# RRZE-HPC/Ultimate-SpMV

Hardware: AMD Instinct MI355X
Metric: SpMV GFLOP/s (SELL-32-512 dp; achieved HBM GB/s in roofline) (higher is better)
Workload: dtype f64; 1 GPU; nlpkkt200-class synthetic (27-pt stencil 253x253x253, n=16194277, nnz=433798093) scs -c 32 -s 512 -dp; C=32, sigma=512, n_rows=16194277, nnz=433798093, x=5.0 (DefaultValues), partition=none, halo_overlap=False, kernel=tile-local-column (LDS-staged x lines, 12-bit local indices)

## Files before the change

### include/uspmv.h

```cpp
#ifndef USPMV_H
#define USPMV_H

#include <stddef.h>
#include <stdint.h>

#ifdef __cplusplus
extern "C" {
#endif

typedef enum {
    USPMV_OK = 0,
    USPMV_ERR_INVALID = 1,
    USPMV_ERR_IO = 2,
    USPMV_ERR_UNSUPPORTED = 3,
    USPMV_ERR_OVERFLOW = 4,
    USPMV_ERR_NO_DEVICE = 5,
    USPMV_ERR_HIP = 6,
    USPMV_ERR_ALLOC = 7,
    USPMV_ERR_COMM = 8
} uspmv_status;

typedef enum { USPMV_F64 = 0, USPMV_F32 = 1, USPMV_F16 = 2 } uspmv_dtype;
typedef enum { USPMV_COLWISE = 0, USPMV_ROWWISE = 1 } uspmv_layout;
typedef enum { USPMV_SEG_ROWS = 0, USPMV_SEG_NNZ = 1 } uspmv_seg;
// ... 21 lines not shown

int uspmv_gen_stencil27(int64_t nx, int64_t ny, int64_t nz, int dof, uint64_t seed, double magnitude_decades,
                        int64_t row_begin, int64_t row_end, uspmv_coo_t **out);
int uspmv_gen_stencil27_row_counts(int64_t nx, int64_t ny, int64_t nz, int dof, int64_t row_begin, int64_t row_end, int32_t *out);
int uspmv_gen_banded_random(int64_t n, int nnz_per_row, int64_t band, uint64_t seed, double magnitude_decades,
                            int64_t row_begin, int64_t row_end, uspmv_coo_t **out);
int uspmv_gen_kkt(int64_t N, uint64_t seed, int64_t row_begin, int64_t row_end, uspmv_coo_t **out);
int uspmv_gen_kkt_row_counts(int64_t N, int64_t row_begin, int64_t row_end, int32_t *out);

int uspmv_convert_to_scs(const uspmv_coo_t *m, int64_t C, int64_t sigma, int dtype,
                         const int32_t *fixed_permutation, uspmv_scs_t **out);
int uspmv_scs_meta(const uspmv_scs_t *s, int64_t meta[8]);
int uspmv_scs_dtype(const uspmv_scs_t *s, int *dtype);
int uspmv_scs_arrays(const uspmv_scs_t *s, const int32_t **chunk_ptrs, const int32_t **chunk_lengths,
                     const int32_t **col_idxs, const void **values, const int32_t **old_to_new_idx,
                     const int32_t **new_to_old_idx);
int uspmv_scs_col_idxs_mut(uspmv_scs_t *s, int32_t **col_idxs);
int uspmv_permute_scs_cols(uspmv_scs_t *s, const int32_t *perm);
void uspmv_scs_free(uspmv_scs_t *s);
int uspmv_apply_permutation(void *out, const void *in, const int32_t *perm, int64_t n, int dtype);
int uspmv_partition_precisions(const uspmv_coo_t *m, double threshold_1, uspmv_coo_t **dp, uspmv_coo_t **sp);
enum { USPMV_AP_DP_HP = 0, USPMV_AP_SP_HP = 1, USPMV_AP_DP_SP_HP = 2 };
int uspmv_partition_precisions_hp(const uspmv_coo_t *m, int kind, double threshold_1, double threshold_2, uspmv_coo_t **hi,
                                  uspmv_coo_t **mid, uspmv_coo_t **hp);

int uspmv_device_count(int *count);
int uspmv_set_device(int device);
int uspmv_stream_synchronize(void *stream);

int uspmv_dmat_upload(const uspmv_scs_t *s, uspmv_dmat_t **out);
int uspmv_convert_to_scs_device(const uspmv_coo_t *m, int64_t C, int64_t sigma, int dtype, const int32_t *fixed_permutation,
                                int permute_cols, uspmv_scs_t **layout, uspmv_dmat_t **out);
int uspmv_dmat_plan_addresses(const uspmv_dmat_t *m, uint64_t addr[8]);
int uspmv_dmat_meta(const uspmv_dmat_t *m, int64_t meta[4]);
enum { USPMV_SORT_HOST = 0, USPMV_SORT_DEVICE_STABLE = 1 };
int uspmv_convert_to_scs_device_from_arrays(const int32_t *d_I, const int32_t *d_J, const double *d_V, int64_t n_rows, int64_t n_cols, int64_t nnz,
                                            int64_t C, int64_t sigma, int dtype, const int32_t *d_fixed_permutation, int permute_cols,
                                            int sort_mode, void *stream, uspmv_scs_t **layout, int32_t *d_old_to_new, int32_t *d_new_to_old,
                                            uspmv_dmat_t **out);
int uspmv_dmat_download(const uspmv_dmat_t *m, int32_t *chunk_ptrs, int32_t *chunk_lengths, int32_t *col_idxs, void *values);
int uspmv_dmat_wrap(int64_t C, int64_t n_chunks, int64_t n_elements, int dtype, const int32_t *d_chunk_ptrs,
                    const int32_t *d_chunk_lengths, const int32_t *d_col_idxs, const void *d_values,
                    uspmv_dmat_t **out);
void uspmv_dmat_free(uspmv_dmat_t *m);
int uspmv_dmat_optimize(uspmv_dmat_t *m, const uspmv_scs_t *s, int max_lines, int64_t *n_tiles, int64_t *n_staged);
int uspmv_dmat_optimize_ap(uspmv_dmat_t *dp, uspmv_dmat_t *sp, const uspmv_scs_t *s_dp, const uspmv_scs_t *s_sp,
                           int max_lines, int64_t *n_tiles, int64_t *n_staged);
int uspmv_dmat_optimize_ap_hp(uspmv_dmat_t *hi, uspmv_dmat_t *mid, uspmv_dmat_t *hp, const uspmv_scs_t *s_hi, const uspmv_scs_t *s_mid,
                              const uspmv_scs_t *s_hp, int max_lines, int64_t *n_tiles, int64_t *n_staged);
int uspmv_dmat_optimize_block(uspmv_dmat_t *m, const uspmv_scs_t *s, int block_vec_size, int64_t *n_tiles, int64_t *n_staged);

int uspmv_dmat_optimize_sweep(uspmv_dmat_t *m, const uspmv_scs_t *s, int wlog, int tile_rows, int64_t *n_tiles, int64_t *n_sweep);
int uspmv_dmat_optimize_sweep_ap(uspmv_dmat_t *dp, uspmv_dmat_t *sp, const uspmv_scs_t *s_dp, const uspmv_scs_t *s_sp, int wlog,
                                 int tile_rows, int64_t *n_tiles, int64_t *n_sweep);
int uspmv_dmat_optimize_sweep_ap_hp(uspmv_dmat_t *hi, uspmv_dmat_t *mid, uspmv_dmat_t *hp, const uspmv_scs_t *s_hi, const uspmv_scs_t *s_mid,
                                    const uspmv_scs_t *s_hp, int wlog, int tile_rows, int64_t *n_tiles, int64_t *n_sweep);
int uspmv_dmat_optimize_sweep_device_ap_hp(uspmv_dmat_t *hi, uspmv_dmat_t *mid, uspmv_dmat_t *hp, int wlog, int tile_rows, int64_t *n_tiles,
                                           int64_t *n_sweep);
int uspmv_dmat_optimize_sweep_device(uspmv_dmat_t *m, uspmv_dmat_t *sp, int wlog, int tile_rows, int64_t *n_tiles, int64_t *n_sweep);
int uspmv_dmat_sweep_plan_digest(const uspmv_dmat_t *m, uint64_t digest[16], int64_t meta[8]);
int uspmv_dmat_sweep_plan_digest_part(const uspmv_dmat_t *m, int part, uint64_t digest[5], int64_t *n_vals);
int uspmv_dmat_plan_info(const uspmv_dmat_t *m, int *kind, int64_t *n_tiles, int64_t *n_planned);
int uspmv_dmat_block_plan_info(const uspmv_dmat_t *m, int64_t meta[10]);
int uspmv_dmat_block_plan_staged(const uspmv_dmat_t *m, int64_t *rows_staged);
int uspmv_dmat_plan_granularity(const uspmv_dmat_t *m, int *elements_per_list_entry);
int uspmv_dmat_plan_rows_dealt(const uspmv_dmat_t *m, int *dealt);
int uspmv_dmat_stream_info(const uspmv_dmat_t *m, int64_t meta[2]);
int uspmv_dmat_block_plan_digest(const uspmv_dmat_t *m, uint64_t digest[8]);

int uspmv_dmat_optimize_block_sweep(uspmv_dmat_t *m, const uspmv_scs_t *s, int block_vec_size, int wlog, int tile_rows, int64_t *n_tiles, int64_t *n_sweep);

int uspmv_dmat_optimize_block_device(uspmv_dmat_t *m, int block_vec_size, int64_t *n_tiles, int64_t *n_staged);

int uspmv_dmat_optimize_device(uspmv_dmat_t *m, int max_lines, int64_t *n_tiles, int64_t *n_staged);
int uspmv_dmat_optimize_device_ap(uspmv_dmat_t *dp, uspmv_dmat_t *sp, int max_lines, int64_t *n_tiles, int64_t *n_staged);
int uspmv_dmat_optimize_device_ap_hp(uspmv_dmat_t *hi, uspmv_dmat_t *mid, uspmv_dmat_t *hp, int max_lines, int64_t *n_tiles, int64_t *n_staged);
int uspmv_dmat_plan_download(const uspmv_dmat_t *m, int64_t meta[4], int32_t *tile_line_ptr, int32_t *tile_lines,
                             uint32_t *c16_ptrs, uint16_t *col16);

int uspmv_dmat_tile_rows(const uspmv_dmat_t *m, int *tile_rows);
int uspmv_dmat_index_bits(const uspmv_dmat_t *m, int *bits);
int uspmv_dmat_additive_chunks(const uspmv_dmat_t *m, int64_t *n_additive, int64_t *n_chunks);
int uspmv_additive_plan_probe(const uspmv_scs_t *s, int64_t stats[8], int32_t *cols);
int uspmv_spmv_tiles(const uspmv_dmat_t *A, const int32_t *d_tile_ids, int64_t n_ids, const void *d_x, void *d_y,
                     void *stream);
int uspmv_dmat_set_crs(uspmv_dmat_t *m, int on);

int uspmv_spmv(const uspmv_dmat_t *A, const void *d_x, void *d_y, void *stream);
int uspmv_spmv_chunks(const uspmv_dmat_t *A, const int32_t *d_chunk_ids, int64_t n_ids, const void *d_x,
                      void *d_y, void *stream);
int uspmv_spmmv(const uspmv_dmat_t *A, const void *d_X, void *d_Y, int b, int64_t ld, int layout, void *stream);
int uspmv_spmmv_x_prepared(const uspmv_dmat_t *m, const void *d_X, int block_vec_size, int64_t ld, void *stream);
int uspmv_spmmv_x_release(const uspmv_dmat_t *m);
int uspmv_spmv_ap(const uspmv_dmat_t *dp, const uspmv_dmat_t *sp, const double *d_x, double *d_y, void *stream);
int uspmv_spmmv_ap(const uspmv_dmat_t *dp, const uspmv_dmat_t *sp, const void *d_X, void *d_Y, int b, int64_t ld, int layout,
                   void *stream);
int uspmv_spmmv_ap_plan_lines(int b, int *max_lines);
int uspmv_spmmv_ap_path(const uspmv_dmat_t *dp, const uspmv_dmat_t *sp, int b, int64_t ld, int layout, int *path, int *vectors_per_pass);
int uspmv_spmmv_ap_sweep_vectors(int b, int wlog, int *vectors);
int uspmv_spmv_ap_generic(const uspmv_dmat_t *dp, const uspmv_dmat_t *sp, const double *d_x, const float *d_x_sp,
                          double *d_y, void *stream);
int uspmv_spmv_ap_hp(const uspmv_dmat_t *hi, const uspmv_dmat_t *mid, const uspmv_dmat_t *hp, const void *d_x, void *d_y, void *stream);
int uspmv_spmmv_ap_hp(const uspmv_dmat_t *hi, const uspmv_dmat_t *mid, const uspmv_dmat_t *hp, const void *d_X, void *d_Y, int b, int64_t ld,
                      int layout, void *stream);
int uspmv_spmmv_ap_hp_path(const uspmv_dmat_t *hi, const uspmv_dmat_t *mid, const uspmv_dmat_t *hp, int b, int64_t ld, int layout, int *path,
                           int *vectors_per_pass);
int uspmv_spmmv_ap_hp_plan_lines(int b, int x_dtype, int *max_lines);
int uspmv_spmmv_ap_hp_sweep_vectors(int b, int wlog, int x_dtype, int *vectors);

int uspmv_scs_gpu_f64(int64_t C, int64_t n_chunks, const int32_t *d_chunk_ptrs, const int32_t *d_chunk_lengths,
                      const int32_t *d_col_idxs, const double *d_values, const double *d_x, double *d_y,
                      void *stream);
int uspmv_scs_gpu_f32(int64_t C, int64_t n_chunks, const int32_t *d_chunk_ptrs, const int32_t *d_chunk_lengths,
                      const int32_t *d_col_idxs, const float *d_values, const float *d_x, float *d_y,
                      void *stream);
int uspmv_csr_gpu_f64(int64_t n_rows, const int32_t *d_row_ptrs, const int32_t *d_col_idxs,
                      const double *d_values, const double *d_x, double *d_y, void *stream);
int uspmv_csr_gpu_f32(int64_t n_rows, const int32_t *d_row_ptrs, const int32_t *d_col_idxs,
                      const float *d_values, const float *d_x, float *d_y, void *stream);

int uspmv_peek_i64(const void *p, int64_t *out);
int uspmv_peek_i32(const void *p, int32_t *out);

int uspmv_apply_permutation_dev(void *d_out, const void *d_in, const int32_t *d_perm, int64_t n, int dtype,
                                void *stream);

void uspmv_raw_plan_cache_clear(void);
int uspmv_set_tuning(const char *key, int value);
int uspmv_get_tuning(const char *key, int *value);

int uspmv_seg_work_sharing_arr(const uspmv_coo_t *total, int seg_method, int P, int32_t *wsa);
int uspmv_graph_partition(const uspmv_coo_t *total, int P, int32_t *part );
int uspmv_read_partition(const char *path, int64_t n_rows, int P, int32_t *part);
int uspmv_coo_apply_partition(const uspmv_coo_t *total, int P, const int32_t *part, uspmv_coo_t **permuted, int32_t *wsa, int32_t *perm);
int uspmv_seg_from_row_counts(const int32_t *row_nnz, int64_t n_rows, int seg_method, int P, int32_t *wsa);
int uspmv_seg_local_coo(const uspmv_coo_t *total, const int32_t *wsa, int rank, uspmv_coo_t **out);
int uspmv_halo_discover(uspmv_scs_t *local_scs, const int32_t *wsa, int rank, int P, uspmv_halo_t **out);
int uspmv_halo_meta(const uspmv_halo_t *h, int64_t *n_halo, const int32_t **recv_counts_cumsum,
                    const int32_t **recv_idxs, const int32_t **recv_counts);
void uspmv_halo_free(uspmv_halo_t *h);
int uspmv_scs_split_chunks(const uspmv_scs_t *s, int64_t n_local, int32_t **interior, int64_t *n_interior,
                           int32_t **boundary, int64_t *n_boundary);
int uspmv_scs_chunk_classes(const uspmv_scs_t *s, int64_t n_local, uint8_t *classes, int32_t *pad_col);
void uspmv_free(void *p);
int uspmv_pack_send_buf(const void *d_x, const int32_t *d_perm, const int32_t *d_send_idxs, int64_t n,
                        int64_t block_offset, void *d_send, int dtype, void *stream);

typedef struct uspmv_transport {
    void *ctx;
    int rank, size;
    int (*alltoallv)(void *ctx, const void *send, const int64_t *send_off, void *recv, const int64_t *recv_off);
    int (*allgather)(void *ctx, const void *send, void *recv, int64_t bytes_per_rank);
    int (*barrier)(void *ctx);
} uspmv_transport_t;

typedef struct uspmv_hostcomm uspmv_hostcomm_t;
int uspmv_hostcomm_create(const char *job, int rank, int size, double timeout_s, uspmv_hostcomm_t **out);
int uspmv_hostcomm_info(const uspmv_hostcomm_t *h, int *rank, int *size, uint64_t *nonce );
int uspmv_hostcomm_barrier(uspmv_hostcomm_t *h);
int uspmv_hostcomm_abort(uspmv_hostcomm_t *h);
int uspmv_hostcomm_bcast(uspmv_hostcomm_t *h, void *buf, int64_t bytes, int root);
int uspmv_hostcomm_allgather(uspmv_hostcomm_t *h, const void *send, void *recv, int64_t bytes_per_rank);
int uspmv_hostcomm_alltoallv(uspmv_hostcomm_t *h, const void *send, const int64_t *send_off, void *recv, const int64_t *recv_off);
int uspmv_hostcomm_allreduce_max_f64(uspmv_hostcomm_t *h, double *value);
int uspmv_hostcomm_transport(uspmv_hostcomm_t *h, uspmv_transport_t *t);
void uspmv_hostcomm_free(uspmv_hostcomm_t *h);
// ... 65 lines not shown
```

### ultimate-spmv_amd/binding.py

```python
import ctypes as C
import os
import subprocess

import numpy as np

_HERE = os.path.dirname(os.path.abspath(__file__))
_LIB = None

F64, F32, F16 = 0, 1, 2
AP_DP_HP, AP_SP_HP, AP_DP_SP_HP = 0, 1, 2
COLWISE, ROWWISE = 0, 1
SEG_ROWS, SEG_NNZ = 0, 1

_vp = C.c_void_p
_i64 = C.c_int64
_i32p = C.POINTER(C.c_int32)
_f64p = C.POINTER(C.c_double)


class UspmvError(RuntimeError):
    def __init__(self, status, text):
        super().__init__(f"libuspmv status {status}: {text}")
        self.status = status


def library_path():
    return os.environ.get("USPMV_LIB") or os.path.join(_HERE, "libuspmv.so")


def build_library(force=False):
    if force:
        subprocess.check_call(["make", "-s", "-C", _HERE, "clean"])
    subprocess.check_call(["make", "-s", "-j4", "-C", _HERE, "all"])
    return library_path()


_SIGS = {
    "uspmv_status_string": (C.c_char_p, [C.c_int]),
    "uspmv_last_error": (C.c_char_p, []),
    "uspmv_version": (C.c_char_p, []),
    "uspmv_read_mtx": (C.c_int, [C.c_char_p, C.POINTER(_vp)]),
    "uspmv_coo_save": (C.c_int, [_vp, C.c_char_p]),
    "uspmv_coo_write_mtx": (C.c_int, [_vp, C.c_char_p, C.c_int]),
    "uspmv_coo_load": (C.c_int, [C.c_char_p, C.POINTER(_vp)]),
    "uspmv_coo_equilibrate": (C.c_int, [_vp]),
    "uspmv_coo_create": (C.c_int, [_i64, _i64, _i64, _vp, _vp, _vp, C.POINTER(_vp)]),
    "uspmv_coo_dims": (C.c_int, [_vp, C.POINTER(_i64), C.POINTER(_i64), C.POINTER(_i64)]),
    "uspmv_coo_arrays": (C.c_int, [_vp, C.POINTER(_i32p), C.POINTER(_i32p), C.POINTER(_f64p)]),
    "uspmv_coo_free": (None, [_vp]),
    "uspmv_gen_stencil27": (C.c_int, [_i64, _i64, _i64, C.c_int, C.c_uint64, C.c_double, _i64, _i64, C.POINTER(_vp)]),
    "uspmv_gen_banded_random": (C.c_int, [_i64, C.c_int, _i64, C.c_uint64, C.c_double, _i64, _i64, C.POINTER(_vp)]),
    "uspmv_gen_kkt": (C.c_int, [_i64, C.c_uint64, _i64, _i64, C.POINTER(_vp)]),
    "uspmv_gen_kkt_row_counts": (C.c_int, [_i64, _i64, _i64, _vp]),
    "uspmv_convert_to_scs": (C.c_int, [_vp, _i64, _i64, C.c_int, _vp, C.POINTER(_vp)]),
    "uspmv_scs_meta": (C.c_int, [_vp, C.POINTER(_i64)]),
    "uspmv_scs_dtype": (C.c_int, [_vp, C.POINTER(C.c_int)]),
    "uspmv_scs_arrays": (C.c_int, [_vp, C.POINTER(_i32p), C.POINTER(_i32p), C.POINTER(_i32p), C.POINTER(_vp),
                                   C.POINTER(_i32p), C.POINTER(_i32p)]),
    "uspmv_scs_col_idxs_mut": (C.c_int, [_vp, C.POINTER(_i32p)]),
    "uspmv_permute_scs_cols": (C.c_int, [_vp, _vp]),
    "uspmv_scs_free": (None, [_vp]),
    "uspmv_apply_permutation": (C.c_int, [_vp, _vp, _vp, _i64, C.c_int]),
    "uspmv_partition_precisions": (C.c_int, [_vp, C.c_double, C.POINTER(_vp), C.POINTER(_vp)]),
    "uspmv_partition_precisions_hp": (C.c_int, [_vp, C.c_int, C.c_double, C.c_double, C.POINTER(_vp), C.POINTER(_vp), C.POINTER(_vp)]),
    "uspmv_dmat_optimize_ap_hp": (C.c_int, [_vp, _vp, _vp, _vp, _vp, _vp, C.c_int, C.POINTER(_i64), C.POINTER(_i64)]),
    "uspmv_dmat_optimize_device_ap_hp": (C.c_int, [_vp, _vp, _vp, C.c_int, C.POINTER(_i64), C.POINTER(_i64)]),
    "uspmv_spmv_ap_hp": (C.c_int, [_vp, _vp, _vp, _vp, _vp, _vp]),
    "uspmv_spmmv_ap_hp": (C.c_int, [_vp, _vp, _vp, _vp, _vp, C.c_int, _i64, C.c_int, _vp]),
    "uspmv_spmmv_ap_hp_path": (C.c_int, [_vp, _vp, _vp, C.c_int, _i64, C.c_int, C.POINTER(C.c_int), C.POINTER(C.c_int)]),
    "uspmv_spmmv_ap_hp_plan_lines": (C.c_int, [C.c_int, C.c_int, C.POINTER(C.c_int)]),
    "uspmv_spmmv_ap_hp_sweep_vectors": (C.c_int, [C.c_int, C.c_int, C.c_int, C.POINTER(C.c_int)]),
    "uspmv_device_count": (C.c_int, [C.POINTER(C.c_int)]),
    "uspmv_set_device": (C.c_int, [C.c_int]),
    "uspmv_stream_synchronize": (C.c_int, [_vp]),
    "uspmv_dmat_upload": (C.c_int, [_vp, C.POINTER(_vp)]),
    "uspmv_convert_to_scs_device": (C.c_int, [_vp, _i64, _i64, C.c_int, _vp, C.c_int, C.POINTER(_vp), C.POINTER(_vp)]),
    "uspmv_dmat_download": (C.c_int, [_vp, _vp, _vp, _vp, _vp]),
    "uspmv_dmat_wrap": (C.c_int, [_i64, _i64, _i64, C.c_int, _vp, _vp, _vp, _vp, C.POINTER(_vp)]),
    "uspmv_dmat_free": (None, [_vp]),
    "uspmv_dmat_set_crs": (C.c_int, [_vp, C.c_int]),
    "uspmv_dmat_optimize": (C.c_int, [_vp, _vp, C.c_int, C.POINTER(_i64), C.POINTER(_i64)]),
    "uspmv_spmv": (C.c_int, [_vp, _vp, _vp, _vp]),
    "uspmv_spmv_chunks": (C.c_int, [_vp, _vp, _i64, _vp, _vp, _vp]),
    "uspmv_spmv_tiles": (C.c_int, [_vp, _vp, _i64, _vp, _vp, _vp]),
    "uspmv_dmat_tile_rows": (C.c_int, [_vp, C.POINTER(C.c_int)]),
    "uspmv_dmat_index_bits": (C.c_int, [_vp, C.POINTER(C.c_int)]),
    "uspmv_dmat_additive_chunks": (C.c_int, [_vp, C.POINTER(C.c_int64), C.POINTER(C.c_int64)]),
    "uspmv_additive_plan_probe": (C.c_int, [_vp, C.POINTER(C.c_int64), _vp]),
    "uspmv_dmat_optimize_device": (C.c_int, [_vp, C.c_int, C.POINTER(_i64), C.POINTER(_i64)]),
    "uspmv_dmat_optimize_device_ap": (C.c_int, [_vp, _vp, C.c_int, C.POINTER(_i64), C.POINTER(_i64)]),
    "uspmv_dmat_plan_download": (C.c_int, [_vp, C.POINTER(_i64), _vp, _vp, _vp, _vp]),
    "uspmv_dmat_optimize_block": (C.c_int, [_vp, _vp, C.c_int, C.POINTER(_i64), C.POINTER(_i64)]),
    "uspmv_dmat_optimize_block_device": (C.c_int, [_vp, C.c_int, C.POINTER(_i64), C.POINTER(_i64)]),
    "uspmv_dmat_optimize_ap": (C.c_int, [_vp, _vp, _vp, _vp, C.c_int, C.POINTER(_i64), C.POINTER(_i64)]),
    "uspmv_dmat_optimize_sweep": (C.c_int, [_vp, _vp, C.c_int, C.c_int, C.POINTER(_i64), C.POINTER(_i64)]),
    "uspmv_dmat_optimize_sweep_ap": (C.c_int, [_vp, _vp, _vp, _vp, C.c_int, C.c_int, C.POINTER(_i64), C.POINTER(_i64)]),
    "uspmv_dmat_plan_info": (C.c_int, [_vp, C.POINTER(C.c_int), C.POINTER(_i64), C.POINTER(_i64)]),
    "uspmv_dmat_block_plan_info": (C.c_int, [_vp, C.POINTER(_i64)]),
    "uspmv_dmat_block_plan_digest": (C.c_int, [_vp, C.POINTER(C.c_uint64)]),
    "uspmv_dmat_block_plan_staged": (C.c_int, [_vp, C.POINTER(_i64)]),
    "uspmv_dmat_stream_info": (C.c_int, [_vp, C.POINTER(_i64)]),
    "uspmv_dmat_plan_granularity": (C.c_int, [_vp, C.POINTER(C.c_int)]),
    "uspmv_dmat_plan_rows_dealt": (C.c_int, [_vp, C.POINTER(C.c_int)]),
    "uspmv_dmat_optimize_sweep_device": (C.c_int, [_vp, _vp, C.c_int, C.c_int, C.POINTER(_i64), C.POINTER(_i64)]),
    "uspmv_dmat_sweep_plan_digest": (C.c_int, [_vp, C.POINTER(C.c_uint64), C.POINTER(_i64)]),
    "uspmv_dmat_sweep_plan_digest_part": (C.c_int, [_vp, C.c_int, C.POINTER(C.c_uint64), C.POINTER(_i64)]),
    "uspmv_dmat_optimize_sweep_ap_hp": (C.c_int, [_vp, _vp, _vp, _vp, _vp, _vp, C.c_int, C.c_int, C.POINTER(_i64), C.POINTER(_i64)]),
    "uspmv_dmat_optimize_sweep_device_ap_hp": (C.c_int, [_vp, _vp, _vp, C.c_int, C.c_int, C.POINTER(_i64), C.POINTER(_i64)]),
    "uspmv_spmmv": (C.c_int, [_vp, _vp, _vp, C.c_int, _i64, C.c_int, _vp]),
    "uspmv_spmv_ap": (C.c_int, [_vp, _vp, _vp, _vp, _vp]),
    "uspmv_spmmv_ap": (C.c_int, [_vp, _vp, _vp, _vp, C.c_int, _i64, C.c_int, _vp]),
    "uspmv_spmmv_ap_plan_lines": (C.c_int, [C.c_int, C.POINTER(C.c_int)]),
    "uspmv_spmmv_ap_path": (C.c_int, [_vp, _vp, C.c_int, _i64, C.c_int, C.POINTER(C.c_int), C.POINTER(C.c_int)]),
    "uspmv_spmmv_ap_sweep_vectors": (C.c_int, [C.c_int, C.c_int, C.POINTER(C.c_int)]),
    "uspmv_spmv_ap_generic": (C.c_int, [_vp, _vp, _vp, _vp, _vp, _vp]),
    "uspmv_scs_gpu_f64": (C.c_int, [_i64, _i64, _vp, _vp, _vp, _vp, _vp, _vp, _vp]),
    "uspmv_scs_gpu_f32": (C.c_int, [_i64, _i64, _vp, _vp, _vp, _vp, _vp, _vp, _vp]),
    "uspmv_csr_gpu_f64": (C.c_int, [_i64, _vp, _vp, _vp, _vp, _vp, _vp]),
    "uspmv_csr_gpu_f32": (C.c_int, [_i64, _vp, _vp, _vp, _vp, _vp, _vp]),
    "uspmv_peek_i64": (C.c_int, [_vp, C.POINTER(_i64)]),
    "uspmv_peek_i32": (C.c_int, [_vp, C.POINTER(C.c_int32)]),
    "uspmv_apply_permutation_dev": (C.c_int, [_vp, _vp, _vp, _i64, C.c_int, _vp]),
    "uspmv_raw_plan_cache_clear": (None, []),
    "uspmv_set_tuning": (C.c_int, [C.c_char_p, C.c_int]),
    "uspmv_get_tuning": (C.c_int, [C.c_char_p, C.POINTER(C.c_int)]),
    "uspmv_seg_work_sharing_arr": (C.c_int, [_vp, C.c_int, C.c_int, _vp]),
    "uspmv_seg_local_coo": (C.c_int, [_vp, _vp, C.c_int, C.POINTER(_vp)]),
    "uspmv_graph_partition": (C.c_int, [_vp, C.c_int, _vp]),
    "uspmv_read_partition": (C.c_int, [C.c_char_p, _i64, C.c_int, _vp]),
    "uspmv_coo_apply_partition": (C.c_int, [_vp, C.c_int, _vp, C.POINTER(_vp), _vp, _vp]),
    "uspmv_halo_discover": (C.c_int, [_vp, _vp, C.c_int, C.c_int, C.POINTER(_vp)]),
    "uspmv_halo_meta": (C.c_int, [_vp, C.POINTER(_i64), C.POINTER(_i32p), C.POINTER(_i32p), C.POINTER(_i32p)]),
    "uspmv_halo_free": (None, [_vp]),
    "uspmv_scs_chunk_classes": (C.c_int, [_vp, _i64, C.POINTER(C.c_uint8), C.POINTER(C.c_int32)]),
    "uspmv_scs_split_chunks": (C.c_int, [_vp, _i64, C.POINTER(_i32p), C.POINTER(_i64), C.POINTER(_i32p),
                                         C.POINTER(_i64)]),
    "uspmv_free": (None, [_vp]),
    "uspmv_pack_send_buf": (C.c_int, [_vp, _vp, _vp, _i64, _i64, _vp, C.c_int, _vp]),
    "uspmv_seg_from_row_counts": (C.c_int, [_vp, _i64, C.c_int, C.c_int, _vp]),
    "uspmv_gen_stencil27_row_counts": (C.c_int, [_i64, _i64, _i64, C.c_int, _i64, _i64, _vp]),
    "uspmv_comm_unique_id": (C.c_int, [_vp]),
    "uspmv_dist_create": (C.c_int, [_vp, C.c_int, C.c_int, C.c_int, C.c_int, _vp, _vp, _vp, _vp, _i64, _vp, _i64, C.c_int, C.POINTER(_vp)]),
    "uspmv_dist_create_from_coo": (C.c_int, [_vp, C.c_int, C.c_int, C.c_int, C.c_int, _vp, _vp, _i64, _i64, C.c_int, C.c_int, C.POINTER(_vp)]),
    "uspmv_dist_info": (C.c_int, [_vp, C.POINTER(_i64)]),
    "uspmv_dist_spmmv_info": (C.c_int, [_vp, C.POINTER(_i64)]),
    "uspmv_dist_pad_info": (C.c_int, [_vp, C.POINTER(_i64)]),
    "uspmv_convert_to_scs_device_from_arrays": (C.c_int, [_vp, _vp, _vp, _i64, _i64, _i64, _i64, _i64, C.c_int, _vp, C.c_int, C.c_int, _vp,
                                                          C.POINTER(_vp), _vp, _vp, C.POINTER(_vp)]),
    "uspmv_dmat_plan_addresses": (C.c_int, [_vp, C.POINTER(C.c_uint64)]),
    "uspmv_dmat_optimize_block_sweep": (C.c_int, [_vp, _vp, C.c_int, C.c_int, C.c_int, C.POINTER(_i64), C.POINTER(_i64)]),
    "uspmv_spmmv_x_prepared": (C.c_int, [_vp, _vp, C.c_int, _i64, _vp]),
    "uspmv_spmmv_x_release": (C.c_int, [_vp]),
    "uspmv_dmat_meta": (C.c_int, [_vp, C.POINTER(_i64)]),
    "uspmv_dist_comm_count": (C.c_int, [_vp, C.POINTER(C.c_int)]),
    "uspmv_dist_exchange": (C.c_int, [_vp, C.POINTER(C.c_int)]),
    "uspmv_dist_autotune": (C.c_int, [_vp, _vp, _vp, C.c_int, _vp, _i32p, _vp, C.POINTER(C.c_int), C.POINTER(C.c_double)]),
    "uspmv_dist_check_reference": (C.c_int, [_vp, _i32p, C.c_int, C.c_int, C.c_int, _vp]),
    "uspmv_dist_parts": (C.c_int, [_vp, C.POINTER(_vp), C.POINTER(_vp), C.POINTER(_vp)]),
    "uspmv_dist_set_overlap": (C.c_int, [_vp, C.c_int]),
    "uspmv_dist_set_no_pack": (C.c_int, [_vp, C.c_int]),
    "uspmv_dist_spmv": (C.c_int, [_vp, _vp, _vp, C.c_int, _vp]),
    "uspmv_dist_run": (C.c_int, [_vp, _vp, _vp, C.c_int, C.c_int, _vp]),
    "uspmv_dist_spmmv": (C.c_int, [_vp, _vp, _vp, C.c_int, C.c_int, C.c_int, C.c_int, _vp]),
    "uspmv_dist_barrier": (C.c_int, [_vp, _vp]),
    "uspmv_dist_allreduce_max": (C.c_int, [_vp, C.POINTER(C.c_double), _vp]),
    "uspmv_dist_allgather_i64": (C.c_int, [_vp, _i64, C.POINTER(_i64), _vp]),
    "uspmv_dist_free": (None, [_vp]),
    "uspmv_dist_create_ex": (C.c_int, [_vp, C.c_int, C.c_int, C.c_int, C.c_int, _vp, _vp, _vp, _vp, _i64, _vp, _i64, C.c_int, _vp, C.POINTER(_vp)]),
    "uspmv_dist_create_from_coo_ex": (C.c_int, [_vp, C.c_int, C.c_int, C.c_int, C.c_int, _vp, _vp, _i64, _i64, C.c_int, C.c_int, _vp, C.POINTER(_vp)]),
    "uspmv_dist_comm_plan": (C.c_int, [_vp, C.POINTER(_i64), C.POINTER(C.POINTER(_i64)), C.POINTER(_i32p), C.POINTER(C.POINTER(_i64))]),
    "uspmv_dist_set_option": (C.c_int, [_vp, C.c_char_p, C.c_int]),
# ... 609 lines not shown
def _stream_ptr(stream):
    if stream is None:
        import torch
        return torch.cuda.current_stream().cuda_stream
    return getattr(stream, "cuda_stream", stream)


def _dp(t):
    return None if t is None else t.data_ptr()


def _torch_dtype(dtype):
    import torch
    return {F64: torch.float64, F32: torch.float32, F16: torch.float16}[dtype]


class DeviceMatrix:

    def __init__(self, scs, device="cuda", crs=False, tlc=False, tlc_max_lines=0, block_tlc=0, _handle=None):
        import torch
        if _handle is not None:
            self.C, self.n_chunks, self.n_elements, self.dtype = scs.C, scs.n_chunks, scs.n_elements, scs.dtype
            self.n_rows, self.n_rows_padded, self.nnz = scs.n_rows, scs.n_rows_padded, scs.nnz
            self.torch_dtype = _torch_dtype(scs.dtype)
            self.h = _handle
            self.tlc_tiles = self.tlc_staged = self.tile_rows = self.block_tiles = self.block_staged = 0
            return
        a = scs.arrays()
        self.C, self.n_chunks, self.n_elements, self.dtype = scs.C, scs.n_chunks, scs.n_elements, scs.dtype
        self.n_rows, self.n_rows_padded, self.nnz = scs.n_rows, scs.n_rows_padded, scs.nnz
        self.torch_dtype = _torch_dtype(scs.dtype)
        dev = torch.device(device)
        self.chunk_ptrs = torch.from_numpy(a["chunk_ptrs"].copy()).to(dev)
        self.chunk_lengths = torch.from_numpy(a["chunk_lengths"].copy()).to(dev)
        self.col_idxs = torch.from_numpy(a["col_idxs"]).to(dev)
        self.values = torch.from_numpy(a["values"]).to(dev)
        h = _vp()
        _ck(lib().uspmv_dmat_wrap(self.C, self.n_chunks, self.n_elements, self.dtype, _dp(self.chunk_ptrs),
                                  _dp(self.chunk_lengths), _dp(self.col_idxs), _dp(self.values), C.byref(h)))
        self.h = h
        self.tlc_tiles = self.tlc_staged = self.tile_rows = 0
        if crs:
            _ck(lib().uspmv_dmat_set_crs(h, 1))
        if tlc:
            self.optimize(scs, tlc_max_lines)
        self.block_tiles = self.block_staged = 0
        if block_tlc:
            self.optimize_block(scs, block_tlc)

    def optimize_block_sweep(self, scs, b, wlog=0, tile_rows=0):
        a, n = _i64(), _i64()
        _ck(lib().uspmv_dmat_optimize_block_sweep(self.h, scs.h, int(b), int(wlog), int(tile_rows), C.byref(a), C.byref(n)))
        return a.value, n.value

    def optimize_device(self, max_lines=0):
        a, b = _i64(), _i64()
        _ck(lib().uspmv_dmat_optimize_device(self.h, max_lines, C.byref(a), C.byref(b)))
        self.tlc_tiles, self.tlc_staged = a.value, b.value
        tr = C.c_int()
        _ck(lib().uspmv_dmat_tile_rows(self.h, C.byref(tr)))
        self.tile_rows = tr.value
        return a.value, b.value

    def plan_granularity(self):
        g = C.c_int()
        _ck(lib().uspmv_dmat_plan_granularity(self.h, C.byref(g)))
        return g.value

    def plan_rows_dealt(self):
        g = C.c_int()
        _ck(lib().uspmv_dmat_plan_rows_dealt(self.h, C.byref(g)))
        return bool(g.value)

    def index_bits(self):
        b = C.c_int()
        _ck(lib().uspmv_dmat_index_bits(self.h, C.byref(b)))
        return b.value

    def additive_chunks(self):
        a, b = C.c_int64(), C.c_int64()
        _ck(lib().uspmv_dmat_additive_chunks(self.h, C.byref(a), C.byref(b)))
        return a.value, b.value

    def plan_download(self):
        meta = (_i64 * 4)()
        _ck(lib().uspmv_dmat_plan_download(self.h, meta, None, None, None, None))
        nt, nl, n16, mx = [int(v) for v in meta]
        if nt == 0:
            return None
        lp = np.empty(nt + 1, np.int32); tl = np.empty(nl, np.int32)
        cp = np.empty(self.n_chunks + 1, np.uint32); c16 = np.empty(n16, np.uint16)
        _ck(lib().uspmv_dmat_plan_download(self.h, meta, _np_ptr(lp), _np_ptr(tl), _np_ptr(cp), _np_ptr(c16)))
        return dict(tile_line_ptr=lp, tile_lines=tl, c16_ptrs=cp, col16=c16, max_lines_used=mx)

    def optimize_block(self, scs, block_vec_size):
        a, b = _i64(), _i64()
        _ck(lib().uspmv_dmat_optimize_block(self.h, scs.h, int(block_vec_size), C.byref(a), C.byref(b)))
        self.block_tiles, self.block_staged = a.value, b.value
        return a.value, b.value

    def optimize_sweep(self, scs, wlog=0, tile_rows=0):
        a, b = _i64(), _i64()
        _ck(lib().uspmv_dmat_optimize_sweep(self.h, scs.h, int(wlog), int(tile_rows), C.byref(a), C.byref(b)))
        return a.value, b.value

    def plan_info(self):
        k, a, b = C.c_int(), _i64(), _i64()
        _ck(lib().uspmv_dmat_plan_info(self.h, C.byref(k), C.byref(a), C.byref(b)))
        return k.value, a.value, b.value

    def block_plan_digest(self):
        d = (C.c_uint64 * 8)()
        _ck(lib().uspmv_dmat_block_plan_digest(self.h, d))
        return [int(v) for v in d]

    def optimize_sweep_device(self, sp=None, wlog=0, tile_rows=0):
        a, b = _i64(), _i64()
        _ck(lib().uspmv_dmat_optimize_sweep_device(self.h, sp.h if sp is not None else None, wlog, tile_rows, C.byref(a), C.byref(b)))
        return a.value, b.value

    def sweep_plan_digest(self):
        d, m = (C.c_uint64 * 16)(), (_i64 * 8)()
        _ck(lib().uspmv_dmat_sweep_plan_digest(self.h, d, m))
        return [int(v) for v in d], [int(v) for v in m]

    def sweep_plan_digest_part(self, part):
        d, n = (C.c_uint64 * 5)(), _i64(0)
        _ck(lib().uspmv_dmat_sweep_plan_digest_part(self.h, int(part), d, C.byref(n)))
        return [int(v) for v in d], n.value

    def block_plan_info(self):
        m = (_i64 * 10)()
        _ck(lib().uspmv_dmat_block_plan_info(self.h, m))
        keys = ("list_plan", "phased_plan", "line_plan", "tiles", "phases", "line_phases", "line_rows_staged", "idx8", "device_built", "max_rows")
        d = dict(zip(keys, [int(v) for v in m]))
        n = _i64()
        _ck(lib().uspmv_dmat_block_plan_staged(self.h, C.byref(n)))
        d["rows_staged"] = n.value
        m2 = (_i64 * 2)()
        _ck(lib().uspmv_dmat_stream_info(self.h, m2))
        d["stream_grid"], d["stream_descriptors"] = int(m2[0]), int(m2[1])
        return d

    def optimize_block_device(self, block_vec_size):
        a, b = _i64(), _i64()
        _ck(lib().uspmv_dmat_optimize_block_device(self.h, int(block_vec_size), C.byref(a), C.byref(b)))
        self.block_tiles, self.block_staged = a.value, b.value
        return a.value, b.value

    def optimize(self, scs, max_lines=0):
        a, b = _i64(), _i64()
        _ck(lib().uspmv_dmat_optimize(self.h, scs.h, max_lines, C.byref(a), C.byref(b)))
        self.tlc_tiles, self.tlc_staged = a.value, b.value
        tr = C.c_int()
        _ck(lib().uspmv_dmat_tile_rows(self.h, C.byref(tr)))
        self.tile_rows = tr.value
        return a.value, b.value

    def __del__(self):
        if getattr(self, "h", None) and _LIB is not None:
            _LIB.uspmv_dmat_free(self.h)
            self.h = None


def additive_plan_probe(scs, decode=True):
    st = (C.c_int64 * 8)()
    cols = np.full(scs.n_elements, -3, dtype=np.int32) if decode else None
    _ck(lib().uspmv_additive_plan_probe(scs.h, st, _np_ptr(cols) if decode else None))
    keys = ("kept", "n_additive", "n_chunks", "tiles_with_records", "tiles", "new_bytes", "replaced_bytes", "max_elems")
    return dict(zip(keys, [int(v) for v in st])), cols


def convert_to_scs_device(coo, C_, sigma, dtype=F64, fixed_permutation=None, permute_cols=True, device="cuda"):
    import torch
    dev = torch.device(device)
    if dev.index is not None:
        torch.cuda.set_device(dev)
    fp = None if fixed_permutation is None else np.ascontiguousarray(fixed_permutation, np.int32)
    hs, hA = _vp(), _vp()
    _ck(lib().uspmv_convert_to_scs_device(coo.h, C_, sigma, dtype, _np_ptr(fp), int(bool(permute_cols)), C.byref(hs), C.byref(hA)))
    s = Scs(hs)
    return s, DeviceMatrix(s, device, _handle=hA)


SORT_HOST, SORT_DEVICE_STABLE = 0, 1


def convert_to_scs_device_from_arrays(d_I, d_J, d_V, n_rows, n_cols, C_, sigma, dtype=F64, fixed_permutation=None, permute_cols=True,
                                      sort=SORT_HOST, want_layout=True, stream=None):
    import torch
    assert d_I.dtype == torch.int32 and d_J.dtype == torch.int32 and d_V.dtype == torch.float64 and d_I.is_cuda
    nnz = int(d_I.numel())
    o2n = torch.empty(n_rows, dtype=torch.int32, device=d_I.device)
    n2o = torch.empty(n_rows, dtype=torch.int32, device=d_I.device)
    hs, hA = _vp(), _vp()
    _ck(lib().uspmv_convert_to_scs_device_from_arrays(_dp(d_I), _dp(d_J), _dp(d_V), n_rows, n_cols, nnz, C_, sigma, dtype,
                                                      None if fixed_permutation is None else _dp(fixed_permutation), int(bool(permute_cols)), int(sort),
                                                      _stream_ptr(stream), C.byref(hs) if want_layout else None, _dp(o2n), _dp(n2o), C.byref(hA)))
    if want_layout:
        s = Scs(hs)
        return s, DeviceMatrix(s, d_I.device, _handle=hA), o2n, n2o

    class _Meta:
        pass
    m = (_i64 * 4)()
    _ck(lib().uspmv_dmat_meta(hA, m))
    s = _Meta()
    s.C, s.n_chunks, s.n_elements, s.dtype = int(m[0]), int(m[1]), int(m[2]), int(m[3])
    s.n_rows, s.n_rows_padded, s.nnz = n_rows, s.n_chunks * s.C, nnz
    return None, DeviceMatrix(s, d_I.device, _handle=hA), o2n, n2o


def spmmv_x_prepared(A, X, b, ld, stream=None):
    _ck(lib().uspmv_spmmv_x_prepared(A.h, _dp(X), int(b), int(ld), _stream_ptr(stream)))


def spmmv_x_release(A):
    _ck(lib().uspmv_spmmv_x_release(A.h))


def dmat_download(A):
    cp = np.empty(A.n_chunks + 1, np.int32); cl = np.empty(A.n_chunks, np.int32)
    ci = np.empty(A.n_elements, np.int32); va = np.empty(A.n_elements, {F64: np.float64, F32: np.float32, F16: np.float16}[A.dtype])
    _ck(lib().uspmv_dmat_download(A.h, _np_ptr(cp), _np_ptr(cl), _np_ptr(ci), _np_ptr(va)))
    return dict(chunk_ptrs=cp, chunk_lengths=cl, col_idxs=ci, values=va)


def optimize_ap(A_dp, A_sp, scs_dp, scs_sp, max_lines=0):
    a, b = _i64(), _i64()
    _ck(lib().uspmv_dmat_optimize_ap(A_dp.h, A_sp.h, scs_dp.h, scs_sp.h, max_lines, C.byref(a), C.byref(b)))
    for A in (A_dp, A_sp):
        A.tlc_tiles, A.tlc_staged = a.value, b.value
    return a.value, b.value


def optimize_device_ap(A_dp, A_sp, max_lines=0):
    a, b = _i64(), _i64()
    _ck(lib().uspmv_dmat_optimize_device_ap(A_dp.h, A_sp.h, max_lines, C.byref(a), C.byref(b)))
    for A in (A_dp, A_sp):
        A.tlc_tiles, A.tlc_staged = a.value, b.value
    return a.value, b.value


def optimize_ap_hp(A_hi, A_mid, A_hp, scs_hi, scs_mid, scs_hp, max_lines=0):
    a, b = _i64(), _i64()
    _ck(lib().uspmv_dmat_optimize_ap_hp(A_hi.h, A_mid.h if A_mid is not None else None, A_hp.h, scs_hi.h,
                                        scs_mid.h if scs_mid is not None else None, scs_hp.h, max_lines, C.byref(a), C.byref(b)))
    return a.value, b.value


def optimize_device_ap_hp(A_hi, A_mid, A_hp, max_lines=0):
    a, b = _i64(), _i64()
# ... 147 lines not shown
```

### ultimate-spmv_amd/csrc/spmv_kernels.hip

```cpp
#include "uspmv_device.hpp"

using namespace uspmv_dev;

namespace {

template <typename VT, int CT, int U, bool NT, bool IDS, int ABL = 0, bool TAILB = false>
__global__ void scs_spmv_rows(const long n_work_chunks, const int C_rt, const int *__restrict__ chunk_ptrs,
                              const int *__restrict__ chunk_lengths, const int *__restrict__ col_idxs,
                              const VT *__restrict__ values, const VT *__restrict__ x, VT *__restrict__ y,
                              const int *__restrict__ chunk_ids, const int xcd_remap, const long n_store) {
    const int C = CT > 0 ? CT : C_rt;
    const unsigned lb = remap_block(blockIdx.x, gridDim.x, xcd_remap);
    const long vrow = (long)lb * blockDim.x + threadIdx.x;
    const long vc = vrow / C;
    const int i = (int)(vrow - vc * C);
    if (vc >= n_work_chunks) return;
    const long c = IDS ? (long)chunk_ids[vc] : vc;
    const long cs = chunk_ptrs[c];
    const int L = chunk_lengths[c];
    const VT *vp = values + cs + i;
    const int *cp = col_idxs + cs + i;
    VT acc = VT(0);
    int j = 0;
    for (; j + U <= L; j += U) {
// ... 103 lines not shown
#pragma unroll
        for (int u = 0; u < U; ++u) xv[u] = x[c0[u]];
#pragma unroll
        for (int u = 0; u < U; ++u) {
            const VT t = fma_t(v0[u], xv[u], acc);
            acc = (j + u < L) ? t : acc;
        }
    }
    if (valid && c * C + i < n_store) st_y<NT>(y + (c * C + i), acc);
}

template <typename T>
__device__ __forceinline__ T ld_now(const T *p) { return *(const volatile T *)p; }
__device__ __forceinline__ double ld_sys(const double *p) {
    return __longlong_as_double((long long)__hip_atomic_load((const unsigned long long *)p, __ATOMIC_RELAXED, __HIP_MEMORY_SCOPE_SYSTEM));
}
__device__ __forceinline__ float ld_sys(const float *p) {
    return __uint_as_float(__hip_atomic_load((const unsigned *)p, __ATOMIC_RELAXED, __HIP_MEMORY_SCOPE_SYSTEM));
}

typedef unsigned u32x4_t __attribute__((ext_vector_type(4)));
template <typename VT, int CT, bool NT, bool IDS, int SYNC = 0, bool I12 = false, bool ELEM = false, bool ADD = false>
__global__ void __launch_bounds__(1024) scs_spmv_tlc(const long n_chunks, const int C_rt, const int *__restrict__ chunk_ptrs,
        const int *__restrict__ chunk_lengths, const int *__restrict__ col_idxs, const VT *__restrict__ values,
        const VT *__restrict__ x_arg, VT *__restrict__ y, const int *__restrict__ tile_line_ptr,
        const int *__restrict__ tile_lines, const unsigned *__restrict__ c16_ptrs,
        const unsigned short *__restrict__ col16, const long x_len, const int *__restrict__ tile_ids,
        const int xcd_remap, const long n_store, const StepArgs sa, const int *__restrict__ row_map, const AddArgs aa) {
    static_assert(!ADD || (SYNC == 0 && !ELEM && !IDS), "additive chunk records: the plain single-struct launch only");
    extern __shared__ __attribute__((aligned(16))) unsigned char tlc_smem[];
    VT *xs = (VT *)tlc_smem;
    constexpr int EPL = 16 / (int)sizeof(VT);
    constexpr int LPL = 16 / EPL;
    typedef VT vec_t __attribute__((ext_vector_type(EPL)));
    const int C = CT > 0 ? CT : C_rt;
    const unsigned lbt = remap_block(blockIdx.x, gridDim.x, xcd_remap);
    const VT *x = x_arg;
    bool coh = false;
    unsigned tile;
    if constexpr (SYNC == 0) {
        tile = IDS ? (unsigned)tile_ids[lbt] : lbt;
        if (IDS && (int)tile < 0) return;
    } else {
        __shared__ int s_go;
        long pos = lbt;
        if constexpr (SYNC == 2) {
            const int e = ld_now(&sa.ss->flag);
            if (lbt == 0 && threadIdx.x == 0) { sa.ss->count[(e + 1) & 1] = 0; sa.ss->expect = e + 1; }
            if ((long)lbt >= (long)ld_now(&sa.ss->count[e & 1])) return;
            pos = sa.defer[(long)(e & 1) * sa.defer_cap + lbt];
        } else if (pos >= sa.late0 && pos < sa.late0 + sa.n_real + sa.n_cond) {
            if (threadIdx.x == 0) {
                const int e = ld_now(&sa.ss->expect);
                const int go = __hip_atomic_load(&sa.ss->flag, __ATOMIC_RELAXED, __HIP_MEMORY_SCOPE_SYSTEM) >= e;
                if (!go) sa.defer[(long)(e & 1) * sa.defer_cap + atomicAdd(&sa.ss->count[e & 1], 1)] = (int)pos;
                s_go = go;
            }
            __syncthreads();
            if (!s_go) return;
            coh = true;
        }
        if (pos >= sa.late0 + sa.n_real && pos < sa.late0 + sa.n_real + sa.n_cond) {
            const VT s = ld_now((const VT *)sa.stale), c = ld_now(x + sa.pad_col);
            if (isfinite(s) && isfinite(c) && (signbit(s) == signbit(c))) return;
            if (pos == sa.late0 + sa.n_real && threadIdx.x == 0) atomicAdd(&sa.ss->reruns, 1);
        }
        tile = (unsigned)tile_ids[pos];
    }
    const int lp0 = tile_line_ptr[tile];
    const int nl = tile_line_ptr[tile + 1] - lp0;
    const long row = (long)tile * blockDim.x + threadIdx.x;
    const long c = row / C;
    const int i = (int)(row - c * C);
    const bool valid = c < n_chunks;
    int cs = 0, L = 0;
    unsigned q0 = 0;
    if (valid) { cs = chunk_ptrs[c]; L = chunk_lengths[c]; q0 = c16_ptrs[c]; }
    VT acc = VT(0);
    bool add_tile = false;
    if constexpr (ADD) {
        const int iv0 = aa.iv_ptr[tile], niv = aa.iv_ptr[tile + 1] - iv0;
        add_tile = niv > 0;
        if (add_tile) {
            typedef int ivec_t __attribute__((ext_vector_type(EPL)));
            const int sub = threadIdx.x % LPL, lk = threadIdx.x / LPL;
            for (int k = lk; k < nl; k += blockDim.x / LPL) {
                const long idx = (long)tile_lines[lp0 + k] * 16 + sub * EPL;
                vec_t v;
                ivec_t pc;
                if (idx + EPL <= x_len) {
                    v = *(const vec_t *)(x + idx);
                    pc = *(const ivec_t *)(aa.cmap + idx);
                } else {
#pragma unroll
                    for (int e = 0; e < EPL; ++e) { const bool in = idx + e < x_len; v[e] = in ? x[idx + e] : VT(0); pc[e] = in ? aa.cmap[idx + e] : -1; }
                }
                int pos[EPL];
#pragma unroll
                for (int e = 0; e < EPL; ++e) pos[e] = -1;
                for (int q = 0; q < niv; ++q) {
                    const int base = aa.iv[4 * (iv0 + q)], len = aa.iv[4 * (iv0 + q) + 1], off = aa.iv[4 * (iv0 + q) + 2];
#pragma unroll
                    for (int e = 0; e < EPL; ++e)
                        if (pc[e] >= base && pc[e] - base < len) pos[e] = off + pc[e] - base;
                }
#pragma unroll
                for (int e = 0; e < EPL; ++e)
                    if (pos[e] >= 0) xs[pos[e]] = v[e];
            }
            __syncthreads();
            if (L > 0) {
                const unsigned ap = aa.ptrs[c];
                const unsigned short *rec = aa.rec + (long)(ap >> 1) * 8;
                const VT *vp = values + (long)cs + i;
                const bool addv = ap & 1u;
                const unsigned R = addv ? (unsigned)rec[i] : 0u;
                const u32x4_t *sp = addv ? (const u32x4_t *)(rec + C) : (const u32x4_t *)rec + i;
                const long ss = addv ? 1 : C;
                int p = 0;
                for (; 8 * p + 8 <= L; ++p) {
                    VT v[8];
#pragma unroll
                    for (int u = 0; u < 8; ++u) v[u] = ld_stream<NT>(vp + (long)(8 * p + u) * C);
                    const u32x4_t s4 = ld_stream<NT>(sp + p * ss);
#pragma unroll
                    for (int u = 0; u < 8; ++u) acc = fma_t(v[u], xs[R + ((s4[u >> 1] >> (16 * (u & 1))) & 0xFFFFu)], acc);
                }
                if (8 * p < L) {
                    const u32x4_t s4 = ld_stream<NT>(sp + p * ss);
#pragma unroll
                    for (int u = 0; u < 8; ++u)
                        if (8 * p + u < L) acc = fma_t(ld_stream<NT>(vp + (long)(8 * p + u) * C), xs[R + ((s4[u >> 1] >> (16 * (u & 1))) & 0xFFFFu)], acc);
                }
            }
        }
    }
    if (add_tile) {
    } else if (nl > 0) {
        const int sub = threadIdx.x % LPL, lk = threadIdx.x / LPL;
        if constexpr (ELEM) {
            for (int k = threadIdx.x; k < nl; k += blockDim.x) {
                const long idx = tile_lines[lp0 + k];
                xs[k] = idx < x_len ? x[idx] : VT(0);
            }
        } else
        for (int k = lk; k < nl; k += blockDim.x / LPL) {
            const long idx = (long)tile_lines[lp0 + k] * 16 + sub * EPL;
            vec_t v;
            if (SYNC == 1 && coh) {
#pragma unroll
                for (int e = 0; e < EPL; ++e) v[e] = idx + e < x_len ? ld_sys(x + idx + e) : VT(0);
            } else if (idx + EPL <= x_len) {
                v = *(const vec_t *)(x + idx);
            } else {
#pragma unroll
                for (int e = 0; e < EPL; ++e) v[e] = idx + e < x_len ? x[idx + e] : VT(0);
            }
            *(vec_t *)(xs + k * 16 + sub * EPL) = v;
        }
        __syncthreads();
        if constexpr (I12) {
            if (L > 0) {
                const VT *vp = values + (long)cs + i;
                const unsigned *cw = (const unsigned *)col16 + q0 + (long)i * 3;
                const int ngt = (L + 3) >> 2, np = ngt >> 1;
#define TLC12_UNPACK(D0, D1, D2)                                                                                      \
                const unsigned ix[8] = {(D0) & 0xFFFu, ((D0) >> 12) & 0xFFFu, ((D0) >> 24) | (((D1) & 0xFu) << 8), ((D1) >> 4) & 0xFFFu, \
                                        ((D1) >> 16) & 0xFFFu, ((D1) >> 28) | (((D2) & 0xFFu) << 4), ((D2) >> 8) & 0xFFFu, (D2) >> 20};
                int p = 0;
                for (; 8 * p + 8 <= L; ++p) {
                    VT v[8];
#pragma unroll
                    for (int u = 0; u < 8; ++u) v[u] = ld_stream<NT>(vp + (long)(8 * p + u) * C);
                    const unsigned *t3 = cw + (long)p * 3 * C;
                    const unsigned d0 = ld_stream<NT>(t3), d1 = ld_stream<NT>(t3 + 1), d2 = ld_stream<NT>(t3 + 2);
                    TLC12_UNPACK(d0, d1, d2)
#pragma unroll
                    for (int u = 0; u < 8; ++u) acc = fma_t(v[u], xs[ix[u]], acc);
                }
                if (p < np) {
                    const unsigned *t3 = cw + (long)p * 3 * C;
                    const unsigned d0 = ld_stream<NT>(t3), d1 = ld_stream<NT>(t3 + 1), d2 = ld_stream<NT>(t3 + 2);
                    TLC12_UNPACK(d0, d1, d2)
#pragma unroll
                    for (int u = 0; u < 8; ++u)
                        if (8 * p + u < L) acc = fma_t(ld_stream<NT>(vp + (long)(8 * p + u) * C), xs[ix[u]], acc);
                } else if (ngt & 1) {
                    const unsigned *t = (const unsigned *)col16 + q0 + (long)3 * np * C;
                    const unsigned e0 = ld_stream<NT>(t + i), e1 = ld_stream<NT>((const unsigned short *)(t + C) + i);
                    const unsigned jx[4] = {e0 & 0xFFFu, (e0 >> 12) & 0xFFFu, (e0 >> 24) | ((e1 & 0xFu) << 8), e1 >> 4};
#pragma unroll
                    for (int u = 0; u < 4; ++u)
                        if (8 * np + u < L) acc = fma_t(ld_stream<NT>(vp + (long)(8 * np + u) * C), xs[jx[u]], acc);
                }
#undef TLC12_UNPACK
            }
        } else
        if (L > 0) {
            const VT *vp = values + (long)cs + i;
            const unsigned long long *cq = (const unsigned long long *)(col16 + q0) + i;
            const int ng = L >> 2;
// ... 87 lines not shown
        acc = fma_t(v, x[ci], acc);
    }
    const VT other = __shfl_xor(acc, 32, 64);
    if (h == 0) st_y<NT>(y + (c * 32 + lane), acc + other);
}

template <typename VT, int G, bool NT>
__global__ void csr_spmv_vector(const long n_rows, const int *__restrict__ row_ptrs,
                                const int *__restrict__ col_idxs, const VT *__restrict__ values,
                                const VT *__restrict__ x, VT *__restrict__ y) {
    const long gt = (long)blockIdx.x * blockDim.x + threadIdx.x;
    const long row = gt / G;
    const int g = (int)(gt % G);
    VT acc = VT(0);
    if (row < n_rows) {
        const int b = row_ptrs[row], e = row_ptrs[row + 1];
        for (int k = b + g; k < e; k += G) acc = fma_t(ld_stream<NT>(values + k), x[ld_stream<NT>(col_idxs + k)], acc);
    }
#pragma unroll
    for (int o = G / 2; o > 0; o >>= 1) acc += __shfl_xor(acc, o, 64);
    if (row < n_rows && g == 0) y[row] = acc;
}


template <typename VT, int CT, int U, bool NT>
void launch_rows_ids(bool ids, unsigned grid, int block, hipStream_t st, long nwc, int C, const uspmv_dmat *A,
                     const VT *x, VT *y, const int *chunk_ids) {
    if (g_tune.spmv_variant == 2) {
        if (ids)
            hipLaunchKernelGGL((scs_spmv_rows_pipe<VT, CT, U, NT, true>), dim3(grid), dim3(block), 0, st, nwc, C, A->chunk_ptrs,
                               A->chunk_lengths, A->col_idxs, (const VT *)A->values, x, y, chunk_ids, g_tune.xcd_remap, A->n_store);
        else
            hipLaunchKernelGGL((scs_spmv_rows_pipe<VT, CT, U, NT, false>), dim3(grid), dim3(block), 0, st, nwc, C, A->chunk_ptrs,
                               A->chunk_lengths, A->col_idxs, (const VT *)A->values, x, y, chunk_ids, g_tune.xcd_remap, A->n_store);
        return;
    }
    if (g_tune.tail_batch && U > 1) {
        if (ids)
            hipLaunchKernelGGL((scs_spmv_rows<VT, CT, U, NT, true, 0, true>), dim3(grid), dim3(block), 0, st, nwc, C, A->chunk_ptrs,
                               A->chunk_lengths, A->col_idxs, (const VT *)A->values, x, y, chunk_ids, g_tune.xcd_remap, A->n_store);
        else
            hipLaunchKernelGGL((scs_spmv_rows<VT, CT, U, NT, false, 0, true>), dim3(grid), dim3(block), 0, st, nwc, C, A->chunk_ptrs,
                               A->chunk_lengths, A->col_idxs, (const VT *)A->values, x, y, chunk_ids, g_tune.xcd_remap, A->n_store);
        return;
    }
    if (ids)
        hipLaunchKernelGGL((scs_spmv_rows<VT, CT, U, NT, true>), dim3(grid), dim3(block), 0, st, nwc, C, A->chunk_ptrs,
                           A->chunk_lengths, A->col_idxs, (const VT *)A->values, x, y, chunk_ids, g_tune.xcd_remap, A->n_store);
    else
        hipLaunchKernelGGL((scs_spmv_rows<VT, CT, U, NT, false>), dim3(grid), dim3(block), 0, st, nwc, C, A->chunk_ptrs,
                           A->chunk_lengths, A->col_idxs, (const VT *)A->values, x, y, chunk_ids, g_tune.xcd_remap, A->n_store);
}

template <typename VT, int CT, int U>
void launch_rows_nt(bool ids, unsigned grid, int block, hipStream_t st, long nwc, int C, const uspmv_dmat *A,
                    const VT *x, VT *y, const int *chunk_ids) {
    if (g_tune.nontemporal) launch_rows_ids<VT, CT, U, true>(ids, grid, block, st, nwc, C, A, x, y, chunk_ids);
    else launch_rows_ids<VT, CT, U, false>(ids, grid, block, st, nwc, C, A, x, y, chunk_ids);
}

template <typename VT, int CT>
void launch_rows_unroll(bool ids, unsigned grid, int block, hipStream_t st, long nwc, int C, const uspmv_dmat *A,
                        const VT *x, VT *y, const int *chunk_ids) {
    switch (g_tune.unroll) {
        case 1: launch_rows_nt<VT, CT, 1>(ids, grid, block, st, nwc, C, A, x, y, chunk_ids); break;
        case 2: launch_rows_nt<VT, CT, 2>(ids, grid, block, st, nwc, C, A, x, y, chunk_ids); break;
        case 8: launch_rows_nt<VT, CT, 8>(ids, grid, block, st, nwc, C, A, x, y, chunk_ids); break;
        default: launch_rows_nt<VT, CT, 4>(ids, grid, block, st, nwc, C, A, x, y, chunk_ids); break;
    }
}

}

namespace uspmv_dev {

template <typename VT>
int launch_spmv_tlc(const uspmv_dmat *A, const int *tile_ids, long n_tiles, const VT *x, VT *y, hipStream_t st) {
    if (n_tiles == 0) return USPMV_OK;
    const int C = (int)A->C;
    unsigned grid = (unsigned)n_tiles;
    const bool elem = A->tlc.elem;
    const bool add = A->tlc.add_ptrs != nullptr && !elem && !tile_ids && !A->tlc.row_map;
    const size_t lds = std::max((size_t)A->tlc.max_lines * (elem ? 1 : 16), add ? (size_t)A->tlc.add_max_elems : (size_t)0) * sizeof(VT);
    const AddArgs aa = add ? AddArgs{A->tlc.add_iv_ptr, A->tlc.add_iv, A->tlc.add_cmap, A->tlc.add_ptrs, A->tlc.add_rec} : AddArgs{};
    const bool own_tiles = add && A->tlc.add_line_ptr != nullptr;
    const int block = own_tiles ? A->tlc.add_tile_rows : A->tlc.tile_rows;
    const int *lptr = own_tiles ? A->tlc.add_line_ptr : A->tlc.line_ptr, *llist = own_tiles ? A->tlc.add_lines : A->tlc.lines;
    if (own_tiles) grid = (unsigned)A->tlc.add_n_tiles;
    const bool i12 = A->tlc.col12 != nullptr;
    const unsigned *iptrs = i12 ? A->tlc.c12_ptrs : A->tlc.c16_ptrs;
    const unsigned short *idata = i12 ? (const unsigned short *)A->tlc.col12 : A->tlc.col16;
#define TLC_LAUNCH(CTV, NTV, IDSV)                                                                                    \
    do {                                                                                                              \
        auto kfn = i12 ? scs_spmv_tlc<VT, CTV, NTV, IDSV, 0, true> : scs_spmv_tlc<VT, CTV, NTV, IDSV>;                \
        if (elem) kfn = i12 ? scs_spmv_tlc<VT, CTV, NTV, IDSV, 0, true, true> : scs_spmv_tlc<VT, CTV, NTV, IDSV, 0, false, true>; \
        if constexpr (!IDSV) { if (add) kfn = i12 ? scs_spmv_tlc<VT, CTV, NTV, false, 0, true, false, true> : scs_spmv_tlc<VT, CTV, NTV, false, 0, false, false, true>; } \
        if (lds > 48 * 1024) (void)hipFuncSetAttribute((const void *)kfn, hipFuncAttributeMaxDynamicSharedMemorySize, (int)lds); \
        hipLaunchKernelGGL(kfn, dim3(grid), dim3(block), lds, st, (long)A->n_chunks, C, A->chunk_ptrs,        \
                           A->chunk_lengths, A->tlc.cols ? A->tlc.cols : A->col_idxs, (const VT *)(A->tlc.values ? A->tlc.values : A->values), x, y, lptr, llist,   \
                           iptrs, idata, (long)A->tlc.x_len, tile_ids, g_tune.xcd_remap, A->n_store, StepArgs{}, (const int *)A->tlc.row_map, aa);  \
    } while (0)
#define TLC_LAUNCH_C(NTV, IDSV) do { if (C == 32) TLC_LAUNCH(32, NTV, IDSV); else TLC_LAUNCH(0, NTV, IDSV); } while (0)
    if (tile_ids) { if (g_tune.nontemporal) TLC_LAUNCH_C(true, true); else TLC_LAUNCH_C(false, true); }
    else { if (g_tune.nontemporal) TLC_LAUNCH_C(true, false); else TLC_LAUNCH_C(false, false); }
#undef TLC_LAUNCH_C
#undef TLC_LAUNCH
    HIP_TRY(hipGetLastError());
    return USPMV_OK;
}

template <typename VT>
int launch_spmv_tlc_step(const uspmv_dmat *A, const int *step_ids, const StepArgs &sa, int sync, const VT *x, VT *y, hipStream_t st) {
    const long n = sync == 1 ? sa.n_early + sa.n_real + sa.n_cond : sa.n_real + sa.n_cond;
    if (n == 0) return USPMV_OK;
    if (A->tlc.elem) return uspmv::fail(USPMV_ERR_UNSUPPORTED, "one-launch distributed step: not on a plan over single x elements");
    const int C = (int)A->C;
    const size_t lds = (size_t)A->tlc.max_lines * 16 * sizeof(VT);
    const bool i12 = A->tlc.col12 != nullptr;
    const unsigned *iptrs = i12 ? A->tlc.c12_ptrs : A->tlc.c16_ptrs;
    const unsigned short *idata = i12 ? (const unsigned short *)A->tlc.col12 : A->tlc.col16;
#define TLC_STEP(CTV, SY)                                                                                             \
    do {                                                                                                              \
        auto kfn = i12 ? scs_spmv_tlc<VT, CTV, true, true, SY, true> : scs_spmv_tlc<VT, CTV, true, true, SY>;         \
        if (lds > 48 * 1024) (void)hipFuncSetAttribute((const void *)kfn, hipFuncAttributeMaxDynamicSharedMemorySize, (int)lds); \
        hipLaunchKernelGGL(kfn, dim3((unsigned)n), dim3(A->tlc.tile_rows), lds, st, (long)A->n_chunks, C, A->chunk_ptrs,  \
                           A->chunk_lengths, A->col_idxs, (const VT *)A->values, x, y, A->tlc.line_ptr, A->tlc.lines,   \
                           iptrs, idata, (long)A->tlc.x_len, step_ids, g_tune.xcd_remap, A->n_store, sa, (const int *)nullptr, AddArgs{}); \
    } while (0)
    if (sync == 1) { if (C == 32) TLC_STEP(32, 1); else TLC_STEP(0, 1); }
    else { if (C == 32) TLC_STEP(32, 2); else TLC_STEP(0, 2); }
#undef TLC_STEP
    HIP_TRY(hipGetLastError());
    return USPMV_OK;
}

template <typename VT>
int launch_spmv_scs(const uspmv_dmat *A, const int *chunk_ids, long n_ids, const VT *x, VT *y, hipStream_t st) {
    const bool ids = chunk_ids != nullptr;
    const long nwc = ids ? n_ids : A->n_chunks;
    if (nwc == 0) return USPMV_OK;
    const int C = (int)A->C;
    const int block = g_tune.block;
    if (!ids && A->sw.on && A->sw.tile_ids && !A->sw.idx_b && g_tune.sweep && !g_tune.ablate && g_tune.spmv_variant == 0 && ((uintptr_t)x % 16 == 0)) {
        if (int rc = launch_spmv_sweep<VT>(A, x, y, st)) return rc;
        return A->sw.n_rest ? launch_spmv_scs<VT>(A, A->sw.rest, (long)A->sw.n_rest, x, y, st) : USPMV_OK;
    }
    if (!ids && A->tlc.on && A->tlc.plan_id == 0 && g_tune.tlc && !g_tune.ablate && g_tune.spmv_variant == 0 && ((uintptr_t)x % 16 == 0))
        return launch_spmv_tlc<VT>(A, nullptr, A->tlc.n_tiles, x, y, st);
    if (!ids && C == 32 && g_tune.spmv_variant == 1) {
        const unsigned grid = grid_for(nwc * 64, block);
        if (g_tune.nontemporal)
            hipLaunchKernelGGL((scs_spmv_split2<VT, 4, true>), dim3(grid), dim3(block), 0, st, nwc, A->chunk_ptrs,
                               A->chunk_lengths, A->col_idxs, (const VT *)A->values, x, y, g_tune.xcd_remap);
        else
            hipLaunchKernelGGL((scs_spmv_split2<VT, 4, false>), dim3(grid), dim3(block), 0, st, nwc, A->chunk_ptrs,
                               A->chunk_lengths, A->col_idxs, (const VT *)A->values, x, y, g_tune.xcd_remap);
    } else {
        const unsigned grid = grid_for(nwc * C, block);
        if (g_tune.ablate && C == 32 && !ids) {
            if (g_tune.ablate == 1)
                hipLaunchKernelGGL((scs_spmv_rows<VT, 32, 8, true, false, 1>), dim3(grid), dim3(block), 0, st, nwc, C, A->chunk_ptrs,
                                   A->chunk_lengths, A->col_idxs, (const VT *)A->values, x, y, chunk_ids, g_tune.xcd_remap, A->n_store);
            else
                hipLaunchKernelGGL((scs_spmv_rows<VT, 32, 8, true, false, 2>), dim3(grid), dim3(block), 0, st, nwc, C, A->chunk_ptrs,
                                   A->chunk_lengths, A->col_idxs, (const VT *)A->values, x, y, chunk_ids, g_tune.xcd_remap, A->n_store);
            HIP_TRY(hipGetLastError());
            return USPMV_OK;
        }
        switch (C) {
            case 1: launch_rows_unroll<VT, 1>(ids, grid, block, st, nwc, C, A, x, y, chunk_ids); break;
// ... 57 lines not shown
```

### ultimate-spmv_amd/csrc/tlc_planner.hip

```cpp
#include "uspmv_device.hpp"

#include <mutex>

using namespace uspmv_dev;

namespace {

bool verbose() {
    static const bool on = getenv("USPMV_VERBOSE") != nullptr;
    return on;
}

int line_budget(int max_lines, int dtype_of_first_part, bool shared) {
    const int lds = (int)(160 * 1024 / (16 * (dtype_of_first_part == USPMV_F64 ? 8 : 4)));
    return std::min({max_lines <= 0 ? 512 : max_lines, lds, shared ? 1280 : 4096});
}

int plan_tile_rows(bool ap) { return g_tune.tlc_tile_rows ? g_tune.tlc_tile_rows : (ap ? 512 : 256); }

bool tile_rows_grow(int rows, int lines_used) { return g_tune.tlc_auto_tile && g_tune.tlc_tile_rows == 0 && rows == 256 && lines_used > 250; }
bool tile_rows_accept(int64_t n_tiles, int64_t n_staged) { return n_staged * 100 >= n_tiles * 99; }

bool stages_nine_tenths(int64_t n_tiles, int64_t n_staged) { return n_staged * 10 >= n_tiles * 9; }
bool stages_19_of_20(int64_t n_tiles, int64_t n_staged) { return n_staged * 20 >= n_tiles * 19; }
// ... 37 lines not shown

int install_host_plan(uspmv_dmat *const parts[3], const uspmv_tlc_plan &p, bool elem, const char *who) {
    auto &t = parts[0]->tlc;
    hipError_t e = t.line_ptr.upload(p.tile_line_ptr.data(), p.tile_line_ptr.size() * 4);
    if (e == hipSuccess) e = t.lines.upload(p.tile_lines.data(), p.tile_lines.size() * 4);
    const std::vector<uint32_t> *ptrs[3] = {&p.c16_ptrs, &p.c16_ptrs_b, &p.c16_ptrs_c};
    const std::vector<uint16_t> *cols[3] = {&p.col16, &p.col16_b, &p.col16_c};
    for (int k = 0; k < 3; ++k) {
        if (!parts[k]) continue;
        if (e == hipSuccess) e = parts[k]->tlc.c16_ptrs.upload(ptrs[k]->data(), ptrs[k]->size() * 4);
        if (e == hipSuccess) e = parts[k]->tlc.col16.upload(cols[k]->data(), cols[k]->size() * 2);
    }
    if (e != hipSuccess) {
        for (int k = 0; k < 3; ++k) if (parts[k]) parts[k]->tlc = {};
        return uspmv::fail(USPMV_ERR_ALLOC, "%s: device copy failed: %s", who, hipGetErrorString(e));
    }
    stamp_plan(parts, p.tile_rows, p.max_lines_used, p.x_len_min, p.n_tiles, p.n_staged_tiles, elem);
    return USPMV_OK;
}

int sweep_takes_over(uspmv_dmat *A, uspmv_dmat *B, const uspmv_scs *s, const uspmv_scs *sB, const PlanStats &st, const char *who, bool *took,
                     uspmv_dmat *B3 = nullptr, const uspmv_scs *sB3 = nullptr) {
    *took = false;
    uspmv_dmat *const ms[3] = {A, B, B3};
    for (uspmv_dmat *M : ms) if (M) M->sw = {};
    if (!g_tune.sweep || (st.valid && stages_half(st.n_tiles, st.n_staged))) return USPMV_OK;
    int64_t swt = 0, sws = 0;
    if (int rc = s ? sweep_plan_install(A, B, s, sB, 0, 0, &swt, &sws, who, B3, sB3) : sweep_plan_install_device(A, B, 0, 0, &swt, &sws, who, B3)) return rc;
    *took = A->sw.on && stages_half(swt, sws);
    if (!*took) for (uspmv_dmat *M : ms) if (M) M->sw = {};
    return USPMV_OK;
}

bool pack12_applies(bool elem, int max_lines, int64_t C, int64_t n_chunks) {
    return g_tune.tlc_idx12 && !(elem ? max_lines > 4096 : max_lines > 256) && C >= 2 && C % 2 == 0 && n_chunks >= 1;
}
bool pack12_kept(int64_t n_elements, int64_t padded_rows) { return g_tune.tlc_idx12 == 2 || !((double)n_elements < 8.0 * (double)padded_rows); }
int64_t c12_dwords(int64_t L, int64_t C) { const int64_t ngt = (L + 3) / 4; return (ngt / 2) * 3 * C + (ngt & 1) * (C + C / 2); }

int tlc_pack12(uspmv_dmat *A, const std::vector<int32_t> *cl, const char *who) {
    if (!A->tlc.on || !pack12_applies(A->tlc.elem, A->tlc.max_lines, A->C, A->n_chunks)) return USPMV_OK;
    std::vector<int32_t> own;
    if (!cl || (int64_t)cl->size() != A->n_chunks) {
        own.resize((size_t)A->n_chunks);
        HIP_TRY(hipMemcpy(own.data(), A->chunk_lengths, 4 * (size_t)A->n_chunks, hipMemcpyDeviceToHost));
        cl = &own;
    }
    const int64_t C = A->C, nc = A->n_chunks;
    std::vector<uint32_t> p12((size_t)nc + 1);
    int64_t tot = 0;
    for (int64_t c = 0; c < nc; ++c) {
        p12[(size_t)c] = (uint32_t)tot;
        tot += c12_dwords((*cl)[(size_t)c], C);
        if (tot > (int64_t)UINT32_MAX) return USPMV_OK;
    }
    p12[(size_t)nc] = (uint32_t)tot;
    hipError_t e = A->tlc.c12_ptrs.upload(p12.data(), 4 * ((size_t)nc + 1));
    if (e == hipSuccess) e = A->tlc.col12.alloc(4 * (size_t)std::max<int64_t>(tot, 1));
    if (e == hipSuccess && launch_plan_pack12(A, A->tlc.c16_ptrs, A->tlc.col16, A->tlc.c12_ptrs, A->tlc.col12, nullptr) != USPMV_OK) e = hipErrorUnknown;
    if (e == hipSuccess) e = hipStreamSynchronize(nullptr);
    if (e != hipSuccess) {
        A->tlc.c12_ptrs.reset(); A->tlc.col12.reset();
        return uspmv::fail(USPMV_ERR_HIP, "%s: packing the local indices to 12 bits failed: %s", who, hipGetErrorString(e));
    }
    if (!pack12_kept(A->n_elements, nc * C)) { A->tlc.c12_ptrs.reset(); A->tlc.col12.reset(); }
    return USPMV_OK;
}

bool additive_eligible(const uspmv_scs *s, const uspmv_tlc_plan &p, bool elem, const std::vector<int32_t> *n2o) {
    if (!g_tune.tlc_additive || elem || !p.valid || p.line_shift != 4) return false;
    if (s->dtype != USPMV_F64 && s->dtype != USPMV_F32) return false;
    return s->n_rows == s->n_cols && s->n_rows > 0 && (int64_t)(n2o ? n2o->size() : s->new_to_old_idx.size()) >= s->n_rows;
}
struct AdditiveBytes { int64_t fresh = 0, replaced = 0; };
AdditiveBytes additive_bytes(const uspmv_scs *s, const uspmv_additive_plan &a, bool idx12) {
    AdditiveBytes b;
    if (!a.valid) return b;
    const int64_t C = s->C, T = a.tile_rows / C;
    for (int64_t c = 0; c < s->n_chunks; ++c) {
        if (a.iv_ptr[(size_t)(c / T) + 1] == a.iv_ptr[(size_t)(c / T)]) continue;
        const int64_t L = s->chunk_lengths[(size_t)c];
        b.replaced += idx12 ? 4 * c12_dwords(L, C) : 2 * ((L + 3) / 4) * 4 * C;
    }
    b.fresh = a.rec_bytes + 4 * (int64_t)a.cmap.size();
    return b;
}
int additive_tile_rows(const uspmv_scs *s, int line_plan_rows) {
    return (s->sigma == 512 || s->sigma == 1024) && s->sigma > line_plan_rows && s->sigma % s->C == 0 ? (int)s->sigma : line_plan_rows;
}
bool additive_kept(const uspmv_additive_plan &a, const AdditiveBytes &b) {
    if (!a.valid || g_tune.tlc_additive == 2) return a.valid;
    return 2 * b.fresh <= b.replaced && (int64_t)(a.iv.size() / 4) <= 5 * a.n_add_tiles;
}

int tlc_additive_install(uspmv_dmat *A, const uspmv_scs *s, const uspmv_tlc_plan &p, int max_lines, const std::vector<int32_t> *n2o, const char *who) {
    if (!A->tlc.on || !additive_eligible(s, p, A->tlc.elem, n2o)) return USPMV_OK;
    uspmv_additive_plan a;
    if (int rc = uspmv_build_additive_plan(s, &p, max_lines * 16, &a, n2o, additive_tile_rows(s, p.tile_rows))) return rc;
    const AdditiveBytes b = additive_bytes(s, a, A->tlc.col12 != nullptr);
    if (verbose()) fprintf(stderr, "[uspmv] additive chunk records: valid=%d tiles=%lld of %lld chunks=%lld additive=%lld max_elems=%d tile_rows=%d records+map=%lld B against %lld B of local indices (columns %s) -> %s\n",
                           (int)a.valid, (long long)a.n_add_tiles, (long long)a.n_tiles, (long long)a.n_chunks, (long long)a.n_additive, a.max_elems, a.tile_rows, (long long)b.fresh,
                           (long long)b.replaced, a.cols_permuted ? "permuted" : "as they are", additive_kept(a, b) ? "kept" : "dropped");
    if (!additive_kept(a, b)) return USPMV_OK;
    auto &t = A->tlc;
    hipError_t e = t.add_iv_ptr.upload(a.iv_ptr.data(), a.iv_ptr.size() * 4);
    if (e == hipSuccess) e = t.add_iv.upload(a.iv.data(), a.iv.size() * 4);
    if (e == hipSuccess) e = t.add_cmap.upload(a.cmap.data(), a.cmap.size() * 4);
    if (e == hipSuccess) e = t.add_rec.upload(a.rec.data(), a.rec.size() * 2);
    if (e == hipSuccess) e = t.add_ptrs.upload(a.rec_ptrs.data(), a.rec_ptrs.size() * 4);
    if (e == hipSuccess && !a.line_ptr.empty()) e = t.add_line_ptr.upload(a.line_ptr.data(), a.line_ptr.size() * 4);
    if (e == hipSuccess && !a.line_ptr.empty()) e = t.add_lines.upload(a.lines.data(), a.lines.size() * 4);
    if (e != hipSuccess) {
        t.add_line_ptr.reset(); t.add_lines.reset();
        t.add_iv_ptr.reset(); t.add_iv.reset(); t.add_cmap.reset(); t.add_rec.reset(); t.add_ptrs.reset();
        return uspmv::fail(USPMV_ERR_ALLOC, "%s: device copy of the additive chunk records failed: %s", who, hipGetErrorString(e));
    }
    t.add_max_elems = a.max_elems; t.add_chunks = a.n_chunks; t.add_additive = a.n_additive;
    t.add_tile_rows = a.tile_rows; t.add_n_tiles = a.n_tiles;
    return USPMV_OK;
}

int device_plan_install_rows(uspmv_dmat *const parts[3], int max_lines, const int R, PlanStats *st, const char *who) {
    uspmv_dmat *const A = parts[0], *const B = parts[1], *const B3 = parts[2];
    for (int k = 0; k < 3; ++k) if (parts[k]) parts[k]->tlc = {};
    *st = {};
    const int64_t C = A->C, nc = A->n_chunks;
    if (C > 256 || 256 % C != 0 || nc < 1) return USPMV_OK;
    max_lines = line_budget(max_lines, A->dtype, B != nullptr);
    const int64_t T = R / C, nt = (nc + T - 1) / T;
    std::vector<int32_t> cl((size_t)nc);
    std::vector<uint32_t> c16p[3];
    int64_t tot16[3] = {0, 0, 0};
    for (int k = 0; k < 3; ++k) {
        if (!parts[k]) continue;
        HIP_TRY(hipMemcpy(cl.data(), parts[k]->chunk_lengths, 4 * (size_t)nc, hipMemcpyDeviceToHost));
        if (!c16_offsets(cl, C, &c16p[k], &tot16[k])) return USPMV_OK;
    }
    DeviceBuf<int> d_n, d_max;
    hipError_t e = d_n.alloc(4 * (size_t)nt);
    if (e == hipSuccess) e = d_max.zeros(4);
    if (e != hipSuccess) return uspmv::fail(USPMV_ERR_ALLOC, "%s: %s", who, hipGetErrorString(e));
    int rc = launch_plan_count(A, (long)nt, max_lines, d_n, d_max, nullptr, B, R, B3);
    std::vector<int32_t> lp((size_t)nt + 1, 0);
    int max_col = 0;
    if (!rc) {
        e = hipMemcpy(lp.data() + 1, d_n, 4 * (size_t)nt, hipMemcpyDeviceToHost);
        if (e == hipSuccess) e = hipMemcpy(&max_col, d_max, 4, hipMemcpyDeviceToHost);
        if (e != hipSuccess) rc = uspmv::fail(USPMV_ERR_HIP, "%s: %s", who, hipGetErrorString(e));
    }
    d_n.reset(); d_max.reset();
    if (rc) return rc;
    int64_t staged = 0, total = 0;
    int used = 0;
    for (int64_t t = 0; t < nt; ++t) {
        const int n = lp[(size_t)t + 1];
        staged += n > 0; used = std::max(used, n);
        total += n;
        if (total > INT32_MAX) return USPMV_OK;
        lp[(size_t)t + 1] = (int32_t)total;
    }
    st->n_tiles = nt; st->n_staged = staged;
    if (staged == 0) return USPMV_OK;
    e = A->tlc.line_ptr.upload(lp.data(), 4 * ((size_t)nt + 1));
    if (e == hipSuccess) e = A->tlc.lines.alloc(4 * (size_t)std::max<int64_t>(total, 1));
    for (int k = 0; k < 3; ++k) {
        if (!parts[k]) continue;
        if (e == hipSuccess) e = parts[k]->tlc.c16_ptrs.upload(c16p[k].data(), 4 * ((size_t)nc + 1));
        if (e == hipSuccess) e = parts[k]->tlc.col16.zeros(2 * (size_t)std::max<int64_t>(tot16[k], 1));
    }
    if (e == hipSuccess && launch_plan_write(A, (long)nt, A->tlc.line_ptr, A->tlc.c16_ptrs, A->tlc.lines, A->tlc.col16, nullptr, B,
                                             B ? B->tlc.c16_ptrs : nullptr, B ? B->tlc.col16 : nullptr, R, B3,
                                             B3 ? B3->tlc.c16_ptrs : nullptr, B3 ? B3->tlc.col16 : nullptr) != USPMV_OK)
        e = hipErrorUnknown;
    if (e == hipSuccess) e = hipStreamSynchronize(nullptr);
    if (e != hipSuccess) {
        for (int k = 0; k < 3; ++k) if (parts[k]) parts[k]->tlc = {};
        return uspmv::fail(USPMV_ERR_HIP, "%s: %s", who, hipGetErrorString(e));
    }
    stamp_plan(parts, R, used, (int64_t)max_col + 1, nt, staged, false);
    st->valid = true; st->lines = used;
    if (!B) return tlc_pack12(A, &cl, who);
    return USPMV_OK;
}

int measured_tile_rows(uspmv_dmat *A, uspmv_dmat *B, int max_lines, const char *who) {
    static std::mutex mtx;
    std::lock_guard<std::mutex> lock(mtx);
    if (!g_tune.tlc_measure_tile || g_tune.tlc_tile_rows != 0 || A->alt || A->C > 256 || 256 % A->C != 0) return 0;
    if (A->n_chunks * A->C < (int64_t)1 << 20) return 0;
    if (B && (B->alt || B->C != A->C || B->n_chunks != A->n_chunks || A->dtype != USPMV_F64 || B->dtype != USPMV_F32)) return 0;
    struct Key { int64_t nc, ne, ne2, C; int dtype, ml; };
    static std::vector<std::pair<Key, int>> seen;
    const int64_t ne2 = B ? B->n_elements : -1;
    for (auto &kv : seen)
        if (kv.first.nc == A->n_chunks && kv.first.ne == A->n_elements && kv.first.ne2 == ne2 && kv.first.C == A->C && kv.first.dtype == A->dtype && kv.first.ml == max_lines)
            return kv.second;
    const size_t vsz = A->dtype == USPMV_F64 ? 8 : 4;
    DeviceBuf<void> x, y;
    hipEvent_t e0 = nullptr, e1 = nullptr;
    int best = 0;
// ... 252 lines not shown
            return USPMV_OK;
        }
    }
    const bool own_budget = max_lines > 0;
    max_lines = line_budget(max_lines, s->dtype, false);
    uspmv_tlc_plan p, q;
    PlanStats st;
    auto build = [&](int R, PlanStats *o) {
        q = {};
        const int rc = uspmv_build_tlc_plan(s, nullptr, max_lines, R, &q);
        *o = stats_of(q);
        return rc;
    };
    if (int rc = plan_at_chosen_rows(opts.measure ? measured_tile_rows(A, nullptr, max_lines, who) : 0, false, build, [&]() { p = std::move(q); }, &st)) return rc;
    auto report = [&]() {
        if (n_tiles) *n_tiles = p.n_tiles;
        if (n_staged) *n_staged = p.valid ? p.n_staged_tiles : 0;
    };
    report();
    if (verbose()) fprintf(stderr, "[uspmv] tlc plan: tile_rows=%d tiles=%lld staged=%lld max_lines=%d lines_total=%zu col16=%zu\n",
                           p.tile_rows, (long long)p.n_tiles, (long long)p.n_staged_tiles, p.max_lines_used, p.tile_lines.size(), p.col16.size());
    A->sw = {};
    const PlanStats line = stats_of(p);
    const int ecap = element_cap(s->dtype);
    bool elem = false;
    if (int rc = elements_take_over(own_budget, line, opts.elements, s->dtype, s->n_elements,
                                    [&](int cap, double *over) { *over = elements_over_cap_frac(s, cap, 256); return USPMV_OK; },
                                    [&](int cap, ElemStats *o) {
                                        q = {};
                                        const int rc2 = uspmv_build_tlc_plan(s, nullptr, cap, 256, &q, 0);
                                        *o = {q.valid, q.n_tiles, q.n_staged_tiles, (int64_t)q.tile_lines.size(), q.max_lines_used};
                                        return rc2;
                                    }, &elem, n_tiles, n_staged))
        return rc;
    if (elem) p = std::move(q);
    uspmv_scs rr;
    std::vector<int32_t> rr_map;
    bool reordered = false;
    if (!elem && line_plan_short(own_budget, line) && g_tune.tlc_elem && g_tune.tlc_elem_rows && opts.deal_rows && s->n_rows == s->n_cols) {
        const int64_t seg_stage[2] = {(int64_t)g_tune.tlc_elem_seg_rows, (int64_t)1 << 20};
        for (int stage = 0; stage < 2 && !reordered; ++stage) {
            if (stage == 1 && seg_stage[1] <= seg_stage[0]) break;
            if (uspmv_scs_reorder_rows(s, g_tune.tlc_elem_rows == 4 ? 4 : 2, &rr, &rr_map, g_tune.tlc_elem_rows == 4 ? 64 : 256, seg_stage[stage]) != 1) break;
            const double over = elements_over_cap_frac(&rr, ecap, 256);
            q = {};
            if (over <= 0.1)
                if (int rc = uspmv_build_tlc_plan(&rr, nullptr, ecap, 256, &q, 0)) return rc;
            if (verbose()) fprintf(stderr, "[uspmv] element plan on the graph-dealt rows (segments of %lld rows): %.0f %% of the sampled tiles over the cap; valid=%d tiles=%lld staged=%lld max_elements=%d (cap %d) elements_total=%zu\n",
                                   (long long)seg_stage[stage], 100.0 * over, (int)q.valid, (long long)q.n_tiles, (long long)q.n_staged_tiles, q.max_lines_used, ecap, q.tile_lines.size());
            if (q.valid && stages_19_of_20(q.n_tiles, q.n_staged_tiles) && elements_pay((int64_t)q.tile_lines.size(), s->n_elements)) {
                p = std::move(q); elem = true; reordered = true;
                report();
                if (verbose()) fprintf(stderr, "[uspmv] tlc plan over single x elements, rows dealt to the tiles by the matrix graph: tiles=%lld max_elements=%d elements_total=%zu (%.1f entries per element)\n",
                                       (long long)p.n_tiles, p.max_lines_used, p.tile_lines.size(), (double)s->n_elements / (double)std::max<size_t>(p.tile_lines.size(), 1));
            } else if (over > 0.6) break;
        }
    }
    if (!elem) {
        bool swept = false;
        if (int rc = sweep_takes_over(A, nullptr, s, nullptr, stats_of(p), who, &swept)) return rc;
        if (swept) return USPMV_OK;
    }
    if (!p.valid) return USPMV_OK;
    uspmv_dmat *const parts[3] = {A, nullptr, nullptr};
    if (int rc = install_host_plan(parts, p, elem, who)) return rc;
    if (reordered) {
        hipError_t e = A->tlc.values.upload(rr.values_ptr(), (size_t)rr.n_elements * (rr.dtype == USPMV_F64 ? 8 : 4));
        if (e == hipSuccess) e = A->tlc.row_map.upload(rr_map.data(), rr_map.size() * 4);
        if (e == hipSuccess && p.n_staged_tiles < p.n_tiles) e = A->tlc.cols.upload(rr.col_idxs.data(), (size_t)rr.n_elements * 4);
        if (e != hipSuccess) {
            A->tlc = {};
            return uspmv::fail(USPMV_ERR_ALLOC, "%s: device copy failed: %s", who, hipGetErrorString(e));
        }
    }
    if (int rc = tlc_pack12(A, &s->chunk_lengths, who)) return rc;
    if (reordered || !opts.additive) return USPMV_OK;
    return tlc_additive_install(A, s, p, max_lines, opts.new_to_old, who);
}

}

extern "C" {

int uspmv_additive_plan_probe(const uspmv_scs_t *s, int64_t stats[8], int32_t *cols) {
    const char *who = "uspmv_additive_plan_probe";
    if (!s || !stats) return uspmv::fail(USPMV_ERR_INVALID, "%s: NULL argument", who);
    if (!uspmv::scs_has_entries(s)) return uspmv::fail(USPMV_ERR_INVALID, "%s: layout-only struct", who);
    for (int k = 0; k < 8; ++k) stats[k] = 0;
    if (cols) for (int64_t k = 0; k < s->n_elements; ++k) cols[k] = -1;
    const int max_lines = line_budget(0, s->dtype, false);
    uspmv_tlc_plan p;
    if (int rc = uspmv_build_tlc_plan(s, nullptr, max_lines, plan_tile_rows(false), &p)) return rc;
    stats[4] = p.n_tiles;
    if (!additive_eligible(s, p, false, nullptr)) return USPMV_OK;
    uspmv_additive_plan a;
    if (int rc = uspmv_build_additive_plan(s, &p, max_lines * 16, &a, nullptr, additive_tile_rows(s, p.tile_rows))) return rc;
    const bool idx12 = pack12_applies(false, p.max_lines_used, s->C, s->n_chunks) && pack12_kept(s->n_elements, s->n_chunks * s->C);
    if (verbose()) fprintf(stderr, "[uspmv] additive probe: line plan tile_rows=%d max_lines=%d; records tile_rows=%d tiles=%lld with records=%lld intervals=%zu max_elems=%d\n", p.tile_rows, p.max_lines_used,
                           a.tile_rows, (long long)a.n_tiles, (long long)a.n_add_tiles, a.iv.size() / 4, a.max_elems);
    const AdditiveBytes b = additive_bytes(s, a, idx12);
    stats[0] = additive_kept(a, b); stats[1] = a.n_additive; stats[2] = a.n_chunks; stats[3] = a.n_add_tiles;
    stats[5] = b.fresh; stats[6] = b.replaced; stats[7] = a.max_elems;
    if (a.valid) stats[4] = a.n_tiles;
    if (cols && stats[0]) uspmv_additive_plan_decode(s, &a, cols);
    return USPMV_OK;
}

int uspmv_dmat_optimize(uspmv_dmat_t *A, const uspmv_scs_t *s, int max_lines, int64_t *n_tiles, int64_t *n_staged) {
    return dmat_optimize(A, s, max_lines, TlcPlanOpts{}, n_tiles, n_staged);
}

int uspmv_dmat_optimize_device(uspmv_dmat_t *A, int max_lines, int64_t *n_tiles, int64_t *n_staged) {
    const char *who = "uspmv_dmat_optimize_device";
    if (int rc = check_dmat_one_prec(A, who)) return rc;
    if (int rc = require_device()) return rc;
    if (A->alt) { uspmv_dmat_free(A->alt); A->alt = nullptr; }
    if (A->C < 32 && 32 % A->C == 0 && g_tune.rechunk && A->n_chunks > 0) {
        const int64_t C = A->C, nc_old = A->n_chunks, per = 32 / C, nc = (nc_old + per - 1) / per;
        std::vector<int32_t> cl_old((size_t)nc_old), cl((size_t)nc, 0), cp((size_t)nc + 1, 0);
        int32_t last = 0;
        HIP_TRY(hipMemcpy(cl_old.data(), A->chunk_lengths, 4 * (size_t)nc_old, hipMemcpyDeviceToHost));
        HIP_TRY(hipMemcpy(&last, A->chunk_ptrs + nc_old, 4, hipMemcpyDeviceToHost));
        int64_t cur = 0;
        bool fits = true;
        for (int64_t k = 0; k < nc && fits; ++k) {
            int32_t L = 0;
            for (int64_t c = k * per; c < std::min((k + 1) * per, nc_old); ++c) L = std::max(L, cl_old[(size_t)c]);
            cl[(size_t)k] = L; cp[(size_t)k] = (int32_t)cur;
            cur += (int64_t)L * 32;
            fits = cur <= INT32_MAX;
        }
        if (fits && rechunk_worth(cur, last)) {
            cp[(size_t)nc] = (int32_t)cur;
            auto *alt = new uspmv_dmat;
            alt->C = 32; alt->n_chunks = nc; alt->n_elements = cur; alt->dtype = A->dtype;
            alt->n_store = (long)(nc_old * C);
            const size_t vsz = A->dtype == USPMV_F64 ? 8 : 4, ne = (size_t)std::max<int64_t>(cur, 1);
            hipError_t e = alt->own_arrays();
            if (e == hipSuccess) e = hipMemcpy(alt->own.chunk_ptrs, cp.data(), 4 * ((size_t)nc + 1), hipMemcpyHostToDevice);
            if (e == hipSuccess) e = hipMemcpy(alt->own.chunk_lengths, cl.data(), 4 * (size_t)nc, hipMemcpyHostToDevice);
            if (e == hipSuccess) e = hipMemsetAsync(alt->own.col_idxs, 0, 4 * ne, nullptr);
            if (e == hipSuccess) e = hipMemsetAsync(alt->own.values, 0, vsz * ne, nullptr);
            int rc = e == hipSuccess ? launch_rechunk32(A, alt->chunk_ptrs, alt->own.col_idxs, alt->own.values, nullptr) : uspmv::fail(USPMV_ERR_ALLOC, "%s: %s", who, hipGetErrorString(e));
            if (!rc) rc = device_plan_install(alt, nullptr, max_lines, n_tiles, n_staged, who);
            if (rc) { uspmv_dmat_free(alt); return rc; }
            A->tlc = {};
            A->alt = alt;
            return USPMV_OK;
        }
    }
    return device_plan_install(A, nullptr, max_lines, n_tiles, n_staged, who);
}

int uspmv_dmat_optimize_ap(uspmv_dmat_t *dp, uspmv_dmat_t *sp, const uspmv_scs_t *s_dp, const uspmv_scs_t *s_sp,
                           int max_lines, int64_t *n_tiles, int64_t *n_staged) {
    const char *who = "uspmv_dmat_optimize_ap";
    if (!dp || !sp || !s_dp || !s_sp) return uspmv::fail(USPMV_ERR_INVALID, "%s: NULL argument", who);
    if (!uspmv::scs_has_entries(s_dp) || !uspmv::scs_has_entries(s_sp))
        return uspmv::fail(USPMV_ERR_INVALID, "%s: layout-only struct; the plan builder needs the host column indices", who);
    if (dp->C != s_dp->C || dp->n_chunks != s_dp->n_chunks || dp->dtype != USPMV_F64 || s_dp->dtype != USPMV_F64 ||
        sp->C != s_sp->C || sp->n_chunks != s_sp->n_chunks || sp->dtype != USPMV_F32 || s_sp->dtype != USPMV_F32 ||
        dp->C != sp->C || dp->n_chunks != sp->n_chunks)
        return uspmv::fail(USPMV_ERR_INVALID, "%s: handles / host structs do not form a dp+sp pair", who);
    if (int rc = require_device()) return rc;
    dp->tlc = {};
    sp->tlc = {};
    max_lines = line_budget(max_lines, USPMV_F64, true);
    uspmv_tlc_plan p;
    PlanStats st;
    auto build = [&](int R, PlanStats *o) {
        const int rc = uspmv_build_tlc_plan(s_dp, s_sp, max_lines, R, &p);
        *o = stats_of(p);
        return rc;
    };
    if (int rc = plan_at_chosen_rows(measured_tile_rows(dp, sp, max_lines, who), true, build, []() {}, &st)) return rc;
    if (n_tiles) *n_tiles = p.n_tiles;
    if (n_staged) *n_staged = p.valid ? p.n_staged_tiles : 0;
    bool swept = false;
    if (int rc = sweep_takes_over(dp, sp, s_dp, s_sp, st, who, &swept)) return rc;
    if (swept || !p.valid) return USPMV_OK;
    uspmv_dmat *const parts[3] = {dp, sp, nullptr};
    return install_host_plan(parts, p, false, who);
}

int uspmv_dmat_optimize_device_ap(uspmv_dmat_t *dp, uspmv_dmat_t *sp, int max_lines, int64_t *n_tiles, int64_t *n_staged) {
    const char *who = "uspmv_dmat_optimize_device_ap";
    if (int rc = check_dmat(dp, who)) return rc;
    if (int rc = check_dmat(sp, who)) return rc;
// ... 71 lines not shown
```

### ultimate-spmv_amd/csrc/uspmv_api.hip

```cpp
#include "uspmv_device.hpp"

#include <mutex>

using namespace uspmv_dev;

namespace uspmv_dev {

Tuning g_tune;

int require_device() {
    int n = 0;
    hipError_t e = hipGetDeviceCount(&n);
    if (e != hipSuccess || n < 1) {
        (void)hipGetLastError();
        return uspmv::fail(USPMV_ERR_NO_DEVICE, "no HIP device is visible (hipGetDeviceCount: %s); "
                           "libuspmv has no CPU fallback", e == hipSuccess ? "0 devices" : hipGetErrorString(e));
    }
    return USPMV_OK;
}

int check_dmat(const uspmv_dmat *A, const char *who) {
    if (!A) return uspmv::fail(USPMV_ERR_INVALID, "%s: NULL matrix", who);
    if (A->C < 1 || A->n_chunks < 0) return uspmv::fail(USPMV_ERR_INVALID, "%s: corrupt matrix handle", who);
    if (A->n_chunks * A->C > INT32_MAX) return uspmv::fail(USPMV_ERR_OVERFLOW, "%s: padded rows exceed int32", who);
// ... 1173 lines not shown
        uint64_t h = 1469598103934665603ull;
        if (d && bytes) {
            buf.resize(bytes);
            HIP_TRY(hipMemcpy(buf.data(), d, bytes, hipMemcpyDeviceToHost));
            for (size_t k = 0; k < bytes; ++k) { h ^= buf[k]; h *= 1099511628211ull; }
        }
        *out = h;
        return USPMV_OK;
    };
    const size_t nt = (size_t)A->pb.n_tiles, nph = (size_t)A->pb.n_phases, nc = (size_t)A->n_chunks, vsz = A->dtype == USPMV_F64 ? 8 : 4;
    int32_t n_list = 0;
    uint32_t tot16 = 0;
    HIP_TRY(hipMemcpy(&n_list, A->pb.list_ptr + nph, 4, hipMemcpyDeviceToHost));
    HIP_TRY(hipMemcpy(&tot16, A->pb.c16_ptrs + nc, 4, hipMemcpyDeviceToHost));
    int rc = fnv(A->pb.ph_ptr, (nt + 1) * 4, &digest[0]);
    if (!rc) rc = fnv(A->pb.g0, nph * 4, &digest[1]);
    if (!rc) rc = fnv(A->pb.list_ptr, (nph + 1) * 4, &digest[2]);
    if (!rc) rc = fnv(A->pb.xrows, (size_t)n_list * 4, &digest[3]);
    if (!rc) rc = fnv(A->pb.c16_ptrs, (nc + 1) * 4, &digest[4]);
    if (!rc) rc = fnv(A->pb.col16, (size_t)tot16 * (A->pb.idx8 ? 1 : 2), &digest[5]);
    if (!rc) rc = fnv(A->pb.values, (size_t)tot16 * vsz, &digest[6]);
    if (!rc) rc = fnv(A->bt.row_map, A->bt.row_map ? nc * (size_t)A->C * 4 : 0, &digest[7]);
    return rc;
}

int uspmv_dmat_block_plan_staged(const uspmv_dmat_t *A, int64_t *rows_staged) {
    if (!A || !rows_staged) return uspmv::fail(USPMV_ERR_INVALID, "uspmv_dmat_block_plan_staged: NULL argument");
    const uspmv_dmat_t *M = (A->alt && g_tune.rechunk) ? A->alt : A;
    *rows_staged = M->pb.on ? M->pb.rows_staged : 0;
    return USPMV_OK;
}

int uspmv_dmat_block_plan_info(const uspmv_dmat_t *A, int64_t meta[10]) {
    if (!A || !meta) return uspmv::fail(USPMV_ERR_INVALID, "uspmv_dmat_block_plan_info: NULL argument");
    const uspmv_dmat_t *M = (A->alt && g_tune.rechunk) ? A->alt : A;
    meta[0] = M->bt.on; meta[1] = M->pb.on; meta[2] = M->pl.on; meta[3] = M->pb.n_tiles; meta[4] = M->pb.n_phases; meta[5] = M->pl.n_phases;
    meta[6] = M->pl.rows_staged; meta[7] = M->pb.idx8; meta[8] = M->pb.device_built; meta[9] = M->pb.max_rows;
    return USPMV_OK;
}

int uspmv_dmat_plan_granularity(const uspmv_dmat_t *A, int *elements_per_list_entry) {
    if (!A || !elements_per_list_entry) return uspmv::fail(USPMV_ERR_INVALID, "uspmv_dmat_plan_granularity: NULL argument");
    const uspmv_dmat_t *M = (A->alt && g_tune.rechunk) ? A->alt : A;
    *elements_per_list_entry = !M->tlc.on ? 0 : M->tlc.elem ? 1 : 16;
    return USPMV_OK;
}

int uspmv_dmat_plan_rows_dealt(const uspmv_dmat_t *A, int *dealt) {
    if (!A || !dealt) return uspmv::fail(USPMV_ERR_INVALID, "uspmv_dmat_plan_rows_dealt: NULL argument");
    const uspmv_dmat_t *M = (A->alt && g_tune.rechunk) ? A->alt : A;
    *dealt = M->tlc.on && M->tlc.row_map != nullptr;
    return USPMV_OK;
}

int uspmv_dmat_stream_info(const uspmv_dmat_t *A, int64_t meta[2]) {
    if (!A || !meta) return uspmv::fail(USPMV_ERR_INVALID, "uspmv_dmat_stream_info: NULL argument");
    const uspmv_dmat_t *M = (A->alt && g_tune.rechunk) ? A->alt : A;
    meta[0] = M->ps.desc ? M->ps.grid : 0; meta[1] = M->ps.desc ? M->ps.n_desc : 0;
    return USPMV_OK;
}

int uspmv_dmat_tile_rows(const uspmv_dmat_t *A, int *tile_rows) {
    if (!A || !tile_rows) return uspmv::fail(USPMV_ERR_INVALID, "uspmv_dmat_tile_rows: NULL argument");
    *tile_rows = A->tlc.on ? A->tlc.tile_rows : 0;
    return USPMV_OK;
}

int uspmv_dmat_index_bits(const uspmv_dmat_t *A, int *bits) {
    if (!A || !bits) return uspmv::fail(USPMV_ERR_INVALID, "uspmv_dmat_index_bits: NULL argument");
    const uspmv_dmat_t *M = (A->alt && g_tune.rechunk) ? A->alt : A;
    *bits = !M->tlc.on ? 0 : M->tlc.col12 ? 12 : 16;
    return USPMV_OK;
}

int uspmv_dmat_additive_chunks(const uspmv_dmat_t *A, int64_t *n_additive, int64_t *n_chunks) {
    if (!A || !n_additive || !n_chunks) return uspmv::fail(USPMV_ERR_INVALID, "uspmv_dmat_additive_chunks: NULL argument");
    const uspmv_dmat_t *M = (A->alt && g_tune.rechunk) ? A->alt : A;
    const bool on = M->tlc.on && M->tlc.add_ptrs;
    *n_additive = on ? M->tlc.add_additive : 0;
    *n_chunks = on ? M->tlc.add_chunks : 0;
    return USPMV_OK;
}

int uspmv_spmmv(const uspmv_dmat_t *A, const void *d_X, void *d_Y, int b, int64_t ld, int layout, void *stream) {
    if (int rc = check_dmat_one_prec(A, "uspmv_spmmv")) return rc;
    if (!d_X || !d_Y || b < 1) return uspmv::fail(USPMV_ERR_INVALID, "uspmv_spmmv: bad argument");
    if (layout != USPMV_COLWISE && layout != USPMV_ROWWISE) return uspmv::fail(USPMV_ERR_INVALID, "uspmv_spmmv: unknown layout %d", layout);
    if (layout == USPMV_COLWISE && ld < A->n_chunks * A->C)
        return uspmv::fail(USPMV_ERR_INVALID, "uspmv_spmmv: ld=%lld smaller than n_rows_padded=%lld", (long long)ld,
                           (long long)(A->n_chunks * A->C));
    if (int rc = require_device()) return rc;
    if (A->alt && g_tune.rechunk) A = A->alt;
    if (A->dtype == USPMV_F64) return launch_spmmv<double>(A, (const double *)d_X, (double *)d_Y, b, (long)ld, layout, (hipStream_t)stream);
    return launch_spmmv<float>(A, (const float *)d_X, (float *)d_Y, b, (long)ld, layout, (hipStream_t)stream);
}

int uspmv_spmmv_x_prepared(const uspmv_dmat_t *A, const void *d_X, int b, int64_t ld, void *stream) {
    if (int rc = check_dmat_one_prec(A, "uspmv_spmmv_x_prepared")) return rc;
    if (!d_X || b < 1 || ld < A->n_chunks * A->C) return uspmv::fail(USPMV_ERR_INVALID, "uspmv_spmmv_x_prepared: bad argument");
    if (int rc = require_device()) return rc;
    if (A->alt && g_tune.rechunk) A = A->alt;
    A->xprep_ptr = nullptr;
    const int rc = A->dtype == USPMV_F64 ? prepare_x<double>(A, (const double *)d_X, b, (long)ld, (hipStream_t)stream)
                                         : prepare_x<float>(A, (const float *)d_X, b, (long)ld, (hipStream_t)stream);
    if (rc > 0) return USPMV_OK;
    if (rc) return rc;
    HIP_TRY(hipGetLastError());
    return USPMV_OK;
}

int uspmv_spmmv_x_release(const uspmv_dmat_t *A) {
    if (int rc = check_dmat(A, "uspmv_spmmv_x_release")) return rc;
    A->xprep_ptr = nullptr;
    if (A->alt) A->alt->xprep_ptr = nullptr;
    return USPMV_OK;
}

static int spmv_ap_impl(const uspmv_dmat_t *dp, const uspmv_dmat_t *sp, const double *d_x, const float *d_x_sp,
                        double *d_y, void *stream, const char *who) {
    if (int rc = check_dmat(dp, who)) return rc;
    if (int rc = check_dmat(sp, who)) return rc;
    if (dp->dtype != USPMV_F64 || sp->dtype != USPMV_F32)
        return uspmv::fail(USPMV_ERR_INVALID, "%s: expects a double and a float struct", who);
    if (dp->C != sp->C || dp->n_chunks != sp->n_chunks)
        return uspmv::fail(USPMV_ERR_INVALID, "%s: dp and sp structs must share C and n_chunks", who);
    if (!d_x || !d_y) return uspmv::fail(USPMV_ERR_INVALID, "%s: NULL vector", who);
    if (int rc = require_device()) return rc;
    if (dp->n_chunks == 0) return USPMV_OK;
    return launch_spmv_ap(dp, sp, d_x, d_x_sp, d_y, (hipStream_t)stream);
}

int uspmv_spmv_ap(const uspmv_dmat_t *dp, const uspmv_dmat_t *sp, const double *d_x, double *d_y, void *stream) {
    return spmv_ap_impl(dp, sp, d_x, nullptr, d_y, stream, "uspmv_spmv_ap");
}

int uspmv_spmv_ap_generic(const uspmv_dmat_t *dp, const uspmv_dmat_t *sp, const double *d_x, const float *d_x_sp,
                          double *d_y, void *stream) {
    if (!d_x_sp) return uspmv::fail(USPMV_ERR_INVALID, "uspmv_spmv_ap_generic: NULL float x");
    return spmv_ap_impl(dp, sp, d_x, d_x_sp, d_y, stream, "uspmv_spmv_ap_generic");
}

int uspmv_spmmv_ap(const uspmv_dmat_t *dp, const uspmv_dmat_t *sp, const void *d_X, void *d_Y, int b, int64_t ld, int layout, void *stream) {
    const char *who = "uspmv_spmmv_ap";
    if (int rc = check_dmat(dp, who)) return rc;
    if (int rc = check_dmat(sp, who)) return rc;
    if (dp->dtype != USPMV_F64 || sp->dtype != USPMV_F32)
        return uspmv::fail(USPMV_ERR_INVALID, "%s: expects a double and a float struct", who);
    if (dp->C != sp->C || dp->n_chunks != sp->n_chunks)
        return uspmv::fail(USPMV_ERR_INVALID, "%s: dp and sp structs must share C and n_chunks", who);
    if (!d_X || !d_Y) return uspmv::fail(USPMV_ERR_INVALID, "%s: NULL vector", who);
    if (b < 1) return uspmv::fail(USPMV_ERR_INVALID, "%s: b=%d", who, b);
    if (layout != USPMV_COLWISE && layout != USPMV_ROWWISE) return uspmv::fail(USPMV_ERR_INVALID, "%s: unknown layout %d", who, layout);
    if (layout == USPMV_COLWISE && ld < dp->n_chunks * dp->C)
        return uspmv::fail(USPMV_ERR_INVALID, "%s: ld=%lld smaller than n_rows_padded=%lld", who, (long long)ld,
                           (long long)(dp->n_chunks * dp->C));
    if (int rc = require_device()) return rc;
    if (dp->n_chunks == 0) return USPMV_OK;
    return launch_spmmv_ap(dp, sp, (const double *)d_X, (double *)d_Y, b, (long)ld, layout, (hipStream_t)stream);
}

int uspmv_spmmv_ap_path(const uspmv_dmat_t *dp, const uspmv_dmat_t *sp, int b, int64_t ld, int layout, int *path, int *vectors_per_pass) {
    const char *who = "uspmv_spmmv_ap_path";
    if (int rc = check_dmat(dp, who)) return rc;
    if (int rc = check_dmat(sp, who)) return rc;
    if (dp->dtype != USPMV_F64 || sp->dtype != USPMV_F32)
        return uspmv::fail(USPMV_ERR_INVALID, "%s: expects a double and a float struct", who);
// ... 208 lines not shown
```

### ultimate-spmv_amd/csrc/uspmv_device.hpp

```cpp
#pragma once
#include <hip/hip_runtime.h>

#include <algorithm>
#include <cstdint>
#include <cstdio>
#include <cstdlib>
#include <cstring>

#include "../host/uspmv_internal.hpp"

template <typename T>
class DeviceBuf {
  public:
    static constexpr size_t MIN_BYTES = 16;
    DeviceBuf() = default;
    DeviceBuf(const DeviceBuf &) = delete;
    DeviceBuf &operator=(const DeviceBuf &) = delete;
    DeviceBuf(DeviceBuf &&o) noexcept : p_(o.p_) { o.p_ = nullptr; }
    DeviceBuf &operator=(DeviceBuf &&o) noexcept {
        if (this != &o) { reset(); p_ = o.p_; o.p_ = nullptr; }
        return *this;
    }
    ~DeviceBuf() { reset(); }
    void reset() {
// ... 19 lines not shown
    hipError_t upload(const void *host, size_t bytes) {
        hipError_t e = alloc(bytes);
        if (e == hipSuccess && bytes) e = hipMemcpy((void *)p_, host, bytes, hipMemcpyHostToDevice);
        return e;
    }

  private:
    T *p_ = nullptr;
};

class PinnedBuf {
  public:
    PinnedBuf() = default;
    PinnedBuf(const PinnedBuf &) = delete;
    PinnedBuf &operator=(const PinnedBuf &) = delete;
    PinnedBuf(PinnedBuf &&o) noexcept : p_(o.p_) { o.p_ = nullptr; }
    PinnedBuf &operator=(PinnedBuf &&o) noexcept {
        if (this != &o) { reset(); p_ = o.p_; o.p_ = nullptr; }
        return *this;
    }
    ~PinnedBuf() { reset(); }
    void reset() {
        if (p_) (void)hipHostFree(p_);
        p_ = nullptr;
    }
    void *get() const { return p_; }
    hipError_t alloc(size_t bytes) {
        reset();
        void *q = nullptr;
        const hipError_t e = hipHostMalloc(&q, bytes, hipHostMallocDefault);
        p_ = q;
        return e;
    }

  private:
    void *p_ = nullptr;
};

struct uspmv_dmat {
    uspmv_dmat() = default;
    uspmv_dmat(const uspmv_dmat &) = delete;
    uspmv_dmat &operator=(const uspmv_dmat &) = delete;

    int64_t C = 0, n_chunks = 0, n_elements = 0;
    int dtype = USPMV_F64;
    const int32_t *chunk_ptrs = nullptr, *chunk_lengths = nullptr, *col_idxs = nullptr;
    const void *values = nullptr;
    struct {
        DeviceBuf<int32_t> chunk_ptrs, chunk_lengths, col_idxs;
        DeviceBuf<void> values;
    } own;
    hipError_t own_arrays() {
        const size_t ne = (size_t)std::max<int64_t>(n_elements, 1);
        hipError_t e = own.chunk_ptrs.alloc(4 * ((size_t)n_chunks + 1));
        if (e == hipSuccess) e = own.chunk_lengths.alloc(4 * (size_t)std::max<int64_t>(n_chunks, 1));
        if (e == hipSuccess) e = own.col_idxs.alloc(4 * ne);
        if (e == hipSuccess) e = own.values.alloc(uspmv_dtype_bytes(dtype) * ne);
        chunk_ptrs = own.chunk_ptrs; chunk_lengths = own.chunk_lengths; col_idxs = own.col_idxs; values = own.values;
        return e;
    }
    bool crs = false;
    long n_store = 0;
    uspmv_dmat *alt = nullptr;
    mutable DeviceBuf<void> ws;
    mutable size_t ws_bytes = 0;
    mutable const void *xprep_ptr = nullptr;
    mutable int xprep_b = 0, xprep_form = 0;
    mutable long xprep_ld = 0;
    DeviceBuf<int32_t> part_len[2][2];
    int part = 0;
    long part_split = 0;
    struct TlcPlan {
        bool on = false;
        bool elem = false;
        int max_lines = 0, tile_rows = 256;
        int64_t x_len = 0, n_tiles = 0, staged = 0;
        uint64_t plan_id = 0;
        DeviceBuf<int32_t> line_ptr, lines;
        DeviceBuf<uint32_t> c16_ptrs;
        DeviceBuf<uint16_t> col16;
        DeviceBuf<uint32_t> c12_ptrs, col12;
        DeviceBuf<void> values;
        DeviceBuf<int32_t> row_map, cols;
        DeviceBuf<int32_t> add_iv_ptr, add_iv, add_cmap;
        DeviceBuf<uint32_t> add_ptrs;
        DeviceBuf<uint16_t> add_rec;
        DeviceBuf<int32_t> add_line_ptr, add_lines;
        int add_max_elems = 0, add_tile_rows = 0;
        int64_t add_n_tiles = 0;
        int64_t add_chunks = 0, add_additive = 0;
    } tlc;
    struct BlockPlan {
        bool on = false;
        int max_rows = 0, tile_rows = 64;
        int64_t n_tiles = 0, staged = 0;
        DeviceBuf<int32_t> line_ptr, xrows;
        DeviceBuf<uint32_t> c16_ptrs;
        DeviceBuf<uint16_t> col16;
        DeviceBuf<void> values;
        DeviceBuf<int32_t> cols, row_map;
    } bt;
    struct PhasedPlan {
        bool on = false;
        int cap_rows = 0, ngp = 0, max_rows = 0;
        int64_t n_tiles = 0, n_phases = 0, rows_staged = 0;
        DeviceBuf<int32_t> ph_ptr, g0, list_ptr, xrows;
        DeviceBuf<void> values;
        DeviceBuf<uint32_t> c16_ptrs;
        DeviceBuf<uint16_t> col16;
        bool idx8 = false;
        bool device_built = false;
    } pb;
    struct StreamSchedule {
        int grid = 0;
        bool per_tile = false;
        int64_t n_desc = 0;
        DeviceBuf<int32_t> wg_ptr;
        DeviceBuf<void> desc;
    } ps;
    struct LinePlan {
        bool on = false;
        int shift = 0, max_rows = 0;
        int64_t n_phases = 0, rows_staged = 0;
        DeviceBuf<int32_t> ph_ptr, g0, list_ptr, lines;
        DeviceBuf<uint8_t> col8;
    } pl;
    struct UnscrambledPlan {
        bool on = false;
        int max_rows = 0;
        int64_t n_phases = 0, n_perm = 0;
        DeviceBuf<int32_t> ph_ptr, g0, list_ptr, xrows, perm;
        DeviceBuf<uint8_t> col8;
    } pu;
    struct BlockSweepPlan {
        bool on = false;
        int tile_rows = 2048, wlog = 9, b = 0;
        int64_t n_tiles = 0, all_tiles = 0, x_rows = 0, windows = 0;
        DeviceBuf<int32_t> tile_ids, win_ptr, wins, pad;
        DeviceBuf<uint64_t> cnt_off;
        DeviceBuf<uint32_t> wave_off;
        DeviceBuf<uint8_t> cnt;
        DeviceBuf<void> vals;
        DeviceBuf<uint16_t> idx;
    } bw;
    struct SweepPlan {
        bool on = false;
        int tile_rows = 1024, wlog = 13;
        int64_t n_tiles = 0, all_tiles = 0, x_len = 0, n_rest = 0;
        int64_t n_vals = 0, n_vals_b = 0, n_vals_c = 0, cnt_bytes = 0;
        int n_parts = 1, dtype_b = USPMV_F32, dtype_c = USPMV_F16;
        uint64_t plan_id = 0;
        DeviceBuf<int32_t> tile_ids, smin, S, pad, pad_b, pad_c, rest;
        DeviceBuf<uint64_t> cnt_off;
        DeviceBuf<uint32_t> wave_off, wave_off_b, wave_off_c;
        DeviceBuf<uint8_t> cnt, cnt_b, cnt_c;
        DeviceBuf<void> vals, vals_b, vals_c;
        DeviceBuf<uint16_t> idx, idx_b, idx_c;
    } sw;
};

namespace uspmv_dev {

struct TlcPlanOpts { bool measure = true, elements = true, deal_rows = true, additive = true; const std::vector<int32_t> *new_to_old = nullptr; };
int dmat_optimize(uspmv_dmat *A, const uspmv_scs *s, int max_lines, const TlcPlanOpts &opts, int64_t *n_tiles, int64_t *n_staged);

struct StepSync {
    int flag;
    int expect;
    int count[2];
    int reruns;
    int spare[3];
};
struct StepArgs {
    long n_early = 0, n_real = 0, n_cond = 0, defer_cap = 0;
    long late0 = 0;
    StepSync *ss = nullptr;
    int *defer = nullptr;
    const void *stale = nullptr;
    int pad_col = -1;
};

struct AddArgs {
    const int *iv_ptr = nullptr, *iv = nullptr, *cmap = nullptr;
    const unsigned *ptrs = nullptr;
    const unsigned short *rec = nullptr;
};

constexpr int USPMV_SKIP_LEN = -4;

inline const int32_t *part_lengths(const uspmv_dmat *A, int order) {
    return A->part && A->part_len[order][A->part - 1] ? A->part_len[order][A->part - 1] : A->chunk_lengths;
}
inline bool part_ok(const uspmv_dmat *A, int order) { return !A->part || A->part_len[order][A->part - 1]; }

struct Tuning {
    int unroll = 8;
    int nontemporal = 1;
    int xcd_remap = 256;
    int block = 256;
    int spmv_variant = 0;
    int csr_lanes = 0;
    int ablate = 0;
    int tlc = 1;
    int rechunk = 1;
    int tlc_tile_rows = 0;
    int tlc_auto_tile = 1;
    int tlc_measure_tile = 1;
    int tail_batch = 0;
    int spmmv_unroll = 0;
    int spmmv_lds_kb = 0;
    int spmmv_tile_rows = 0;
    int raw_plan_cache = 0;
    int spmmv_swizzle = 0;
    int spmmv_prefetch = 1;
    int sweep = 1;
    int sweep_threads = 0;
    int sweep_nbuf = 1;
    int sweep_pair = 2;
    int sweep_unroll = 8;
    int sweep_remap = 8;
    int sweep_wlog = 0;
    int sweep_tile_rows = 0;
    int sweep_max_stage = 0;
    int spmmv_unscramble = 0;
    int block_plan_device = 1;
    int spmmv_xline = 0;
    int spmmv_ycol_nt = 0;
    int spmmv_xcol = 0;
    int spmmv_phased = 1;
    int spmmv_phase_rows = 256;
    int spmmv_list_plan = 0;
    int spmmv_idx8 = 1;
    int tlc_elem = 1;
    int tlc_elem_rows = 1;
    int tlc_elem_seg_rows = 65536;
    int tlc_elem_cap = 4096;
    int tlc_idx12 = 1;
    int tlc_additive = 1;
    int spmmv_reorder = 4;
    int spmmv_brick_stride = 0;
    int spmmv_brick_lines = 4;
    int spmmv_phase_dp = 24;
    int spmmv_stream = 0;
    int spmmv_stream_waves = 4;
    int spmmv_stream_depth = 1;
    int spmmv_stream_xcd = 1;
    int spmmv_variant = 0;
};
extern Tuning g_tune;

int require_device();
int check_dmat(const uspmv_dmat *A, const char *who);
int check_dmat_one_prec(const uspmv_dmat *A, const char *who);
int check_ap_hp(const uspmv_dmat *hi, const uspmv_dmat *mid, const uspmv_dmat *hp, const char *who);
bool c16_offsets(const std::vector<int32_t> &cl, int64_t C, std::vector<uint32_t> *c16p, int64_t *tot16);
int sweep_plan_install(uspmv_dmat *A, uspmv_dmat *B, const uspmv_scs *s, const uspmv_scs *sB, int wlog, int tile_rows, int64_t *n_tiles,
                       int64_t *n_sweep, const char *who, uspmv_dmat *B3 = nullptr, const uspmv_scs *sB3 = nullptr);
int sweep_plan_install_device(uspmv_dmat *A, uspmv_dmat *B, int wlog, int tile_rows, int64_t *n_tiles, int64_t *n_sweep, const char *who,
                              uspmv_dmat *B3 = nullptr);
inline unsigned grid_for(long work_items, int block) { return (unsigned)((work_items + block - 1) / block); }

constexpr size_t BT_LDS_CAP = 80 * 1024;

template <typename VT>
int launch_spmv_scs(const uspmv_dmat *A, const int *chunk_ids, long n_ids, const VT *x, VT *y, hipStream_t st);
template <typename VT>
// ... 167 lines not shown
```

### ultimate-spmv_amd/host/tlc_plan.cpp

```cpp
#include <algorithm>
#include <cstring>
#include <cstdio>
#include <cstdlib>
#include <omp.h>

#include "uspmv_internal.hpp"

int uspmv_build_tlc_plan(const uspmv_scs *s, const uspmv_scs *s2, int max_lines, int tile_rows, uspmv_tlc_plan *p, int line_shift,
                         const uspmv_scs *s3) {
    p->valid = false;
    const int64_t C = s->C;
    if (line_shift < 0 || line_shift > 4) line_shift = 4;
    const int LS = line_shift;
    const int32_t LM = (1 << LS) - 1;
    if (tile_rows != 32 && tile_rows != 64 && tile_rows != 128 && tile_rows != 256 && tile_rows != 512 && tile_rows != 1024) tile_rows = 256;
    if (C < 1 || C > tile_rows || tile_rows % C != 0 || s->n_chunks < 1) return USPMV_OK;
    if (s2 && (s2->C != C || s2->n_chunks != s->n_chunks)) return USPMV_OK;
    if (s3 && (!s2 || s3->C != C || s3->n_chunks != s->n_chunks)) return USPMV_OK;
    if (max_lines < 1) return USPMV_OK;
    if (max_lines > (65536 >> LS)) max_lines = 65536 >> LS;
    p->line_shift = LS;
    const int64_t T = tile_rows / C;
    p->tile_rows = tile_rows;
    const int64_t n_tiles = (s->n_chunks + T - 1) / T;
// ... 30 lines not shown
                const int32_t *ci = ss[w]->col_idxs.data();
                const int64_t e0 = ss[w]->chunk_ptrs[(size_t)c0], e1 = ss[w]->chunk_ptrs[(size_t)c1];
                n_el += e1 - e0;
                for (int64_t k = e0; k < e1; ++k) {
                    const int32_t l = ci[k] >> LS;
                    lo = std::min(lo, l); hi = std::max(hi, l);
                    my_max = std::max(my_max, ci[k]);
                }
            }
            if (hi < 0) continue;
            const int64_t range = (int64_t)hi - lo + 1;
            const bool dense = range <= 65536;
            int32_t n = 0;
            if (dense) {
                pos.assign((size_t)range, -1);
                for (int w = 0; w < ns; ++w) {
                    const int32_t *ci = ss[w]->col_idxs.data();
                    for (int64_t k = ss[w]->chunk_ptrs[(size_t)c0]; k < ss[w]->chunk_ptrs[(size_t)c1]; ++k) pos[(size_t)((ci[k] >> LS) - lo)] = 0;
                }
                for (int64_t r = 0; r < range && n <= max_lines; ++r)
                    if (pos[(size_t)r] == 0) { pos[(size_t)r] = n++; lines.push_back((int32_t)(lo + r)); }
            } else {
                lines.reserve((size_t)n_el);
                for (int w = 0; w < ns; ++w) {
                    const int32_t *ci = ss[w]->col_idxs.data();
                    for (int64_t k = ss[w]->chunk_ptrs[(size_t)c0]; k < ss[w]->chunk_ptrs[(size_t)c1]; ++k) lines.push_back(ci[k] >> LS);
                }
                std::sort(lines.begin(), lines.end());
                lines.erase(std::unique(lines.begin(), lines.end()), lines.end());
                n = (int32_t)lines.size();
            }
            if (n > max_lines) continue;
            auto local_of = [&](int32_t col) -> uint16_t {
                const int32_t l = col >> LS;
                const int32_t pl = dense ? pos[(size_t)(l - lo)]
                                         : (int32_t)(std::lower_bound(lines.begin(), lines.end(), l) - lines.begin());
                return (uint16_t)((pl << LS) | (col & LM));
            };
            for (int w = 0; w < ns; ++w) {
                const int32_t *ci = ss[w]->col_idxs.data();
                for (int64_t c = c0; c < c1; ++c) {
                    const int64_t cs = ss[w]->chunk_ptrs[(size_t)c], L = ss[w]->chunk_lengths[(size_t)c];
                    uint16_t *q = c16[w]->data() + (*ptrs[w])[(size_t)c];
                    for (int64_t j = 0; j < L; ++j)
                        for (int64_t i = 0; i < C; ++i)
                            q[(j / 4) * 4 * C + i * 4 + (j % 4)] = local_of(ci[cs + j * C + i]);
                }
            }
            tile_lines[(size_t)t] = lines;
        }
#pragma omp critical
        max_col = std::max(max_col, my_max);
    }
    p->tile_line_ptr.assign((size_t)n_tiles + 1, 0);
    int64_t tot = 0;
    int mx = 0;
    int64_t n_staged = 0;
    for (int64_t t = 0; t < n_tiles; ++t) {
        p->tile_line_ptr[(size_t)t] = (int32_t)tot;
        tot += (int64_t)tile_lines[(size_t)t].size();
        mx = std::max<int>(mx, (int)tile_lines[(size_t)t].size());
        n_staged += !tile_lines[(size_t)t].empty();
        if (tot > INT32_MAX) return USPMV_OK;
    }
    p->tile_line_ptr[(size_t)n_tiles] = (int32_t)tot;
    p->tile_lines.resize((size_t)tot);
    for (int64_t t = 0; t < n_tiles; ++t)
        std::copy(tile_lines[(size_t)t].begin(), tile_lines[(size_t)t].end(), p->tile_lines.begin() + p->tile_line_ptr[(size_t)t]);
    p->max_lines_used = mx;
    p->n_staged_tiles = n_staged;
    p->x_len_min = (int64_t)max_col + 1;
    p->valid = n_staged > 0;
    return USPMV_OK;
}

namespace {
struct AddMaps {
    const int32_t *n2o;
    const int32_t *cm;
    int64_t n_rows;
    int64_t row(int64_t r) const { return r < n_rows ? n2o[r] : r; }
    int64_t col(int32_t c) const { return cm ? cm[c] : c; }
};
bool chunk_offsets(const uspmv_scs *s, const AddMaps &m, int64_t c, const int64_t *rr, int64_t *d) {
    const int64_t C = s->C, cs = s->chunk_ptrs[(size_t)c], L = s->chunk_lengths[(size_t)c];
    const int32_t *ci = s->col_idxs.data() + cs;
    for (int64_t j = 0; j < L; ++j) {
        const int64_t dj = m.col(ci[j * C]) - rr[0];
        for (int64_t i = 1; i < C; ++i)
            if (m.col(ci[j * C + i]) - rr[i] != dj) return false;
        d[j] = dj;
    }
    return true;
}
int64_t add_pos(const int32_t *iv, int n_iv, int64_t p, int *which = nullptr) {
    for (int k = 0; k < n_iv; ++k)
        if (p >= iv[4 * k] && p < (int64_t)iv[4 * k] + iv[4 * k + 1]) { if (which) *which = k; return iv[4 * k + 2] + p - iv[4 * k]; }
    return -1;
}
constexpr int ADD_MAX_IV = 16;
constexpr int64_t ADD_HOLE = 32;
}

int uspmv_build_additive_plan(const uspmv_scs *s, const uspmv_tlc_plan *lp, int budget, uspmv_additive_plan *p, const std::vector<int32_t> *new_to_old, int tile_rows) {
    *p = {};
    const std::vector<int32_t> &n2o = new_to_old ? *new_to_old : s->new_to_old_idx;
    const int64_t C = s->C, nc = s->n_chunks, n = s->n_rows;
    if (!lp || !lp->valid || lp->line_shift != 4 || C < 8 || C % 8 != 0 || C > lp->tile_rows || nc < 1 || n < 1 || n != s->n_cols) return USPMV_OK;
    if ((int64_t)n2o.size() < n || n > (int64_t)INT32_MAX || lp->x_len_min > n) return USPMV_OK;
    budget = std::min(budget, 65536);
    std::vector<int32_t> inv((size_t)n, -1);
    for (int64_t r = 0; r < n; ++r) {
        const int64_t o = n2o[(size_t)r];
        if (o < 0 || o >= n || inv[(size_t)o] >= 0) return USPMV_OK;
        inv[(size_t)o] = (int32_t)r;
    }
    const bool own_tiles = tile_rows > 0 && tile_rows != lp->tile_rows && tile_rows % C == 0 && tile_rows <= 1024 && lp->n_staged_tiles == lp->n_tiles;
    if (!own_tiles) tile_rows = lp->tile_rows;
    const int64_t T = tile_rows / C, nt = (nc + T - 1) / T;
    p->tile_rows = tile_rows;
    p->n_tiles = nt;
    std::vector<std::vector<int32_t>> t_lines(own_tiles ? (size_t)nt : 0);
    AddMaps m{n2o.data(), n2o.data(), n};
    {
        const int64_t step = std::max<int64_t>(1, nc / 4096);
        int64_t hits[2] = {0, 0};
        for (int w = 0; w < 2; ++w) {
            const AddMaps mw{m.n2o, w == 0 ? m.n2o : nullptr, n};
            int64_t h = 0;
#pragma omp parallel reduction(+ : h)
            {
                std::vector<int64_t> rr((size_t)C), d;
#pragma omp for schedule(dynamic, 16)
                for (int64_t c = 0; c < nc; c += step) {
                    bool in_range = true;
                    for (int64_t k = s->chunk_ptrs[(size_t)c]; k < s->chunk_ptrs[(size_t)c + 1]; ++k) in_range = in_range && s->col_idxs[(size_t)k] >= 0 && s->col_idxs[(size_t)k] < n;
                    if (!in_range) continue;
                    for (int64_t i = 0; i < C; ++i) rr[(size_t)i] = mw.row(c * C + i);
                    d.resize((size_t)s->chunk_lengths[(size_t)c] + 1);
                    h += chunk_offsets(s, mw, c, rr.data(), d.data());
                }
            }
            hits[w] = h;
        }
        p->cols_permuted = hits[0] >= hits[1];
        if (!p->cols_permuted) m.cm = nullptr;
    }
    std::vector<std::vector<int32_t>> t_iv((size_t)nt);
    std::vector<uint32_t> units((size_t)nc, 0);
    std::vector<uint8_t> additive((size_t)nc, 0);
    auto chunk_additive = [&](int64_t c, const int32_t *iv, int n_iv, int64_t *rr, int64_t *d, int64_t *rmin) -> bool {
        const int64_t L = s->chunk_lengths[(size_t)c];
        if (L < 1) return false;
        int64_t lo = INT64_MAX, hi = INT64_MIN;
        for (int64_t i = 0; i < C; ++i) { rr[i] = m.row(c * C + i); lo = std::min(lo, rr[i]); hi = std::max(hi, rr[i]); }
        *rmin = lo;
        if (hi - lo > 65535 || !chunk_offsets(s, m, c, rr, d)) return false;
        for (int64_t j = 0; j < L; ++j) {
            int ka = -1, kb = -2;
            if (add_pos(iv, n_iv, lo + d[j], &ka) < 0 || add_pos(iv, n_iv, hi + d[j], &kb) < 0 || ka != kb) return false;
        }
        return true;
    };
#pragma omp parallel
    {
        std::vector<int64_t> cols, rr((size_t)C), d;
        std::vector<std::pair<int64_t, int64_t>> gaps;
        std::vector<size_t> cb;
        std::vector<char> joined;
#pragma omp for schedule(dynamic, 16)
        for (int64_t t = 0; t < nt; ++t) {
            if (!own_tiles && lp->tile_line_ptr[(size_t)t + 1] == lp->tile_line_ptr[(size_t)t]) continue;
            const int64_t c0 = t * T, c1 = std::min<int64_t>(c0 + T, nc);
            const int64_t e0 = s->chunk_ptrs[(size_t)c0], e1 = s->chunk_ptrs[(size_t)c1];
            if (e1 <= e0) continue;
            cols.clear();
            bool in_range = true;
            for (int64_t k = e0; k < e1; ++k) {
                const int32_t col = s->col_idxs[(size_t)k];
                if (col < 0 || col >= n) { in_range = false; break; }
                cols.push_back(m.col(col));
            }
            if (!in_range) continue;
            std::sort(cols.begin(), cols.end());
            cols.erase(std::unique(cols.begin(), cols.end()), cols.end());
            cb.clear();
            cb.push_back(0);
            for (size_t k = 1; k < cols.size(); ++k)
                if (cols[k] - cols[k - 1] - 1 > ADD_HOLE) cb.push_back(k);
            const size_t n_run = cb.size();
            cb.push_back(cols.size());
            joined.assign(n_run, 0);
            auto run_of = [&](int64_t pc) { return (size_t)(std::upper_bound(cb.begin(), cb.begin() + (long)n_run, (size_t)(std::lower_bound(cols.begin(), cols.end(), pc) - cols.begin())) - cb.begin()) - 1; };
            for (int64_t c = c0; c < c1 && n_run > 1; ++c) {
                const int64_t L = s->chunk_lengths[(size_t)c];
                if (L < 1) continue;
                int64_t lo = INT64_MAX, hi = INT64_MIN;
                for (int64_t i = 0; i < C; ++i) { rr[(size_t)i] = m.row(c * C + i); lo = std::min(lo, rr[(size_t)i]); hi = std::max(hi, rr[(size_t)i]); }
                d.resize((size_t)L + 1);
                if (hi - lo > 65535 || !chunk_offsets(s, m, c, rr.data(), d.data())) continue;
                for (int64_t j = 0; j < L; ++j)
                    for (size_t k = run_of(lo + d[(size_t)j]), ke = run_of(hi + d[(size_t)j]); k < ke; ++k) joined[k] = 1;
            }
            std::vector<int32_t> iv;
            int64_t total = 0;
            for (int attempt = 0; attempt < 2; ++attempt) {
                if (attempt == 1) joined.assign(n_run, 0);
                size_t n_iv_now = 1;
                gaps.clear();
                for (size_t k = 0; k + 1 < n_run; ++k)
                    if (!joined[k]) { ++n_iv_now; gaps.emplace_back(cols[cb[k + 1]] - cols[cb[k + 1] - 1] - 1, (int64_t)k); }
                if (n_iv_now > (size_t)ADD_MAX_IV) {
                    std::sort(gaps.begin(), gaps.end());
                    for (size_t g = 0; g < n_iv_now - ADD_MAX_IV; ++g) joined[(size_t)gaps[g].second] = 1;
                }
                iv.clear();
                total = 0;
                for (size_t k = 0, first = 0; k < n_run; ++k) {
                    if (k + 1 < n_run && joined[k]) continue;
                    const int64_t len = cols[cb[k + 1] - 1] - cols[cb[first]] + 1;
                    iv.push_back((int32_t)cols[cb[first]]); iv.push_back((int32_t)len); iv.push_back((int32_t)total); iv.push_back(0);
                    total += len;
                    first = k + 1;
                }
                if (total <= budget) break;
            }
            if (total > budget) continue;
            const int n_iv = (int)iv.size() / 4;
            for (int64_t c = c0; c < c1; ++c) {
                const int64_t L = s->chunk_lengths[(size_t)c];
                d.resize((size_t)L + 1);
                int64_t rmin = 0;
                additive[(size_t)c] = chunk_additive(c, iv.data(), n_iv, rr.data(), d.data(), &rmin);
                units[(size_t)c] = (uint32_t)(additive[(size_t)c] ? C / 8 + (L + 7) / 8 : ((L + 7) / 8) * C);
            }
            t_iv[(size_t)t] = std::move(iv);
            if (own_tiles) {
                auto &ln = t_lines[(size_t)t];
                for (int64_t k = e0; k < e1; ++k) ln.push_back(s->col_idxs[(size_t)k] >> 4);
                std::sort(ln.begin(), ln.end());
                ln.erase(std::unique(ln.begin(), ln.end()), ln.end());
            }
        }
    }
    if (own_tiles) {
        int64_t with = 0, n_lines = 0;
        for (int64_t t = 0; t < nt; ++t) { with += !t_iv[(size_t)t].empty() || s->chunk_ptrs[(size_t)std::min<int64_t>(t * T + T, nc)] == s->chunk_ptrs[(size_t)(t * T)]; n_lines += (int64_t)t_lines[(size_t)t].size(); }
        if (with != nt || n_lines > (int64_t)INT32_MAX) return uspmv_build_additive_plan(s, lp, budget, p, new_to_old, 0);
        p->line_ptr.assign((size_t)nt + 1, 0);
        p->lines.reserve((size_t)n_lines);
        for (int64_t t = 0; t < nt; ++t) {
            p->lines.insert(p->lines.end(), t_lines[(size_t)t].begin(), t_lines[(size_t)t].end());
            p->line_ptr[(size_t)t + 1] = (int32_t)p->lines.size();
        }
    }
    p->iv_ptr.assign((size_t)nt + 1, 0);
    int64_t n_iv_all = 0;
    for (int64_t t = 0; t < nt; ++t) {
        p->iv_ptr[(size_t)t] = (int32_t)n_iv_all;
        const int64_t k = (int64_t)t_iv[(size_t)t].size() / 4;
        n_iv_all += k;
        if (k == 0) continue;
        ++p->n_add_tiles;
        int64_t total = 0;
        for (int64_t q = 0; q < k; ++q) total += t_iv[(size_t)t][(size_t)(4 * q + 1)];
        p->max_elems = std::max<int>(p->max_elems, (int)total);
        const int64_t c0 = t * T, c1 = std::min<int64_t>(c0 + T, nc);
        p->n_chunks += c1 - c0;
        for (int64_t c = c0; c < c1; ++c) p->n_additive += additive[(size_t)c];
    }
    p->iv_ptr[(size_t)nt] = (int32_t)n_iv_all;
    if (p->n_add_tiles == 0 || n_iv_all > (int64_t)INT32_MAX / 4) return USPMV_OK;
    p->iv.resize((size_t)(4 * n_iv_all));
    for (int64_t t = 0; t < nt; ++t) std::copy(t_iv[(size_t)t].begin(), t_iv[(size_t)t].end(), p->iv.begin() + 4 * (int64_t)p->iv_ptr[(size_t)t]);
    p->rec_ptrs.assign((size_t)nc, 0);
    int64_t tot_units = 0;
    for (int64_t c = 0; c < nc; ++c) {
        p->rec_ptrs[(size_t)c] = (uint32_t)(tot_units << 1) | additive[(size_t)c];
        tot_units += units[(size_t)c];
        if (tot_units >= ((int64_t)1 << 31)) return USPMV_OK;
    }
    p->rec_bytes = tot_units * 16;
    p->rec.assign((size_t)(tot_units * 8), 0);
#pragma omp parallel
    {
        std::vector<int64_t> rr((size_t)C), d;
#pragma omp for schedule(dynamic, 16)
        for (int64_t t = 0; t < nt; ++t) {
            const int n_iv = p->iv_ptr[(size_t)t + 1] - p->iv_ptr[(size_t)t];
            if (n_iv == 0) continue;
            const int32_t *iv = p->iv.data() + 4 * (int64_t)p->iv_ptr[(size_t)t];
            for (int64_t c = t * T; c < std::min<int64_t>(t * T + T, nc); ++c) {
                const int64_t cs = s->chunk_ptrs[(size_t)c], L = s->chunk_lengths[(size_t)c];
                uint16_t *q = p->rec.data() + (size_t)(p->rec_ptrs[(size_t)c] >> 1) * 8;
                if (additive[(size_t)c]) {
                    d.resize((size_t)L + 1);
                    int64_t rmin = 0;
                    chunk_additive(c, iv, n_iv, rr.data(), d.data(), &rmin);
                    for (int64_t i = 0; i < C; ++i) q[i] = (uint16_t)(rr[(size_t)i] - rmin);
                    for (int64_t j = 0; j < L; ++j) q[C + j] = (uint16_t)add_pos(iv, n_iv, rmin + d[(size_t)j]);
                } else {
                    for (int64_t j = 0; j < L; ++j)
                        for (int64_t i = 0; i < C; ++i)
                            q[((j / 8) * C + i) * 8 + (j % 8)] = (uint16_t)add_pos(iv, n_iv, m.col(s->col_idxs[(size_t)(cs + j * C + i)]));
                }
            }
        }
    }
    if (p->cols_permuted) { p->o2n.swap(inv); p->cmap.assign(n2o.begin(), n2o.begin() + n); }
    else { p->o2n.resize((size_t)n); for (int64_t k = 0; k < n; ++k) p->o2n[(size_t)k] = (int32_t)k; p->cmap = p->o2n; }
    p->valid = true;
    return USPMV_OK;
}

void uspmv_additive_plan_decode(const uspmv_scs *s, const uspmv_additive_plan *p, int32_t *out) {
    const int64_t C = s->C, nc = s->n_chunks, T = p->tile_rows / C;
    for (int64_t k = 0; k < s->n_elements; ++k) out[k] = -1;
    if (!p->valid) return;
    std::vector<int32_t> lds;
    for (int64_t c = 0; c < nc; ++c) {
        const int64_t t = c / T;
        const int n_iv = p->iv_ptr[(size_t)t + 1] - p->iv_ptr[(size_t)t];
        if (n_iv == 0) continue;
        if (c % T == 0) {
            const int32_t *iv = p->iv.data() + 4 * (int64_t)p->iv_ptr[(size_t)t];
            lds.clear();
            for (int k = 0; k < n_iv; ++k) {
                lds.resize((size_t)iv[4 * k + 2], -2);
                for (int32_t e = 0; e < iv[4 * k + 1]; ++e) lds.push_back(p->o2n[(size_t)(iv[4 * k] + e)]);
            }
        }
        const int64_t cs = s->chunk_ptrs[(size_t)c], L = s->chunk_lengths[(size_t)c];
        const uint16_t *q = p->rec.data() + (size_t)(p->rec_ptrs[(size_t)c] >> 1) * 8;
        for (int64_t j = 0; j < L; ++j)
            for (int64_t i = 0; i < C; ++i) {
                const size_t l = (p->rec_ptrs[(size_t)c] & 1) ? (size_t)q[i] + q[C + j] : (size_t)q[((j / 8) * C + i) * 8 + (j % 8)];
                out[cs + j * C + i] = l < lds.size() ? lds[l] : -2;
            }
    }
}


int uspmv_scs_rechunk32(const uspmv_scs *s, uspmv_scs *o) {
    const int64_t C = s->C;
    if (C < 1 || C >= 32 || 32 % C != 0) return USPMV_ERR_UNSUPPORTED;
    const int64_t per = 32 / C, n_pad_old = s->n_chunks * C;
    const int64_t nc = (s->n_chunks + per - 1) / per;
    o->C = 32; o->sigma = s->sigma; o->n_rows = s->n_rows; o->n_cols = s->n_cols; o->nnz = s->nnz; o->dtype = s->dtype;
    o->n_chunks = nc; o->n_rows_padded = nc * 32;
    o->chunk_lengths.assign((size_t)nc, 0);
    o->chunk_ptrs.assign((size_t)nc + 1, 0);
    int64_t cur = 0;
    for (int64_t k = 0; k < nc; ++k) {
        int32_t L = 0;
        for (int64_t c = k * per; c < std::min((k + 1) * per, s->n_chunks); ++c) L = std::max(L, s->chunk_lengths[(size_t)c]);
        o->chunk_lengths[(size_t)k] = L;
        o->chunk_ptrs[(size_t)k] = (int32_t)cur;
        cur += (int64_t)L * 32;
        if (cur > INT32_MAX) return USPMV_ERR_OVERFLOW;
    }
    o->chunk_ptrs[(size_t)nc] = (int32_t)cur;
    o->n_elements = cur;
    o->col_idxs.assign((size_t)cur, 0);
    if (s->dtype == USPMV_F64) o->values_f64.assign((size_t)cur, 0.0); else o->values_f32.assign((size_t)cur, 0.0f);
#pragma omp parallel for schedule(static)
    for (int64_t k = 0; k < nc; ++k) {
        const int64_t base = o->chunk_ptrs[(size_t)k];
        for (int64_t i = 0; i < 32; ++i) {
            const int64_t row = k * 32 + i;
            if (row >= n_pad_old) break;
            const int64_t co = row / C, io = row % C;
            const int64_t cs = s->chunk_ptrs[(size_t)co], L = s->chunk_lengths[(size_t)co];
            for (int64_t j = 0; j < L; ++j) {
                const int64_t src = cs + j * C + io, dst = base + j * 32 + i;
                o->col_idxs[(size_t)dst] = s->col_idxs[(size_t)src];
                if (s->dtype == USPMV_F64) o->values_f64[(size_t)dst] = s->values_f64[(size_t)src];
                else o->values_f32[(size_t)dst] = s->values_f32[(size_t)src];
            }
        }
    }
    return USPMV_OK;
}

static int64_t cluster_row_map(const uspmv_scs *s, const std::vector<int32_t> &base, int64_t window_chunks, std::vector<int32_t> *row_map, bool flat, int64_t seg_stride = 1,
                               int64_t tile_rows = 64, int64_t seg_rows = 65536) {
    const int64_t C = s->C, nc = s->n_chunks, n_pad = nc * C;
    const int64_t T = std::max<int64_t>(1, tile_rows / C);
    int64_t seg_chunks = std::max<int64_t>(window_chunks, T);
    while (seg_chunks * C < seg_rows) seg_chunks *= 2;
    const int64_t n_seg = (nc + seg_chunks - 1) / seg_chunks;
    if (seg_stride > 1) *row_map = base;
    std::vector<char> assigned((size_t)n_pad, 0);
    std::vector<int32_t> stamp((size_t)n_pad, -1), cnt((size_t)n_pad, 0);
#pragma omp parallel
    {
        std::vector<int32_t> cls_rows;
        std::vector<std::pair<int32_t, int32_t>> heap;
        std::vector<int64_t> cls_begin, cursor;
#pragma omp for schedule(dynamic, 1)
        for (int64_t sg = seg_stride / 2; sg < n_seg; sg += seg_stride) {
            const int64_t cA = sg * seg_chunks, cB = std::min(nc, cA + seg_chunks), lo = cA * C, hi = cB * C;
            int32_t max_len = 0;
            for (int64_t c = cA; c < cB; ++c) max_len = std::max(max_len, s->chunk_lengths[(size_t)c]);
            cls_begin.assign((size_t)max_len + 2, 0);
            for (int64_t c = cA; c < cB; ++c) cls_begin[(size_t)s->chunk_lengths[(size_t)c] + 1] += C;
            for (size_t l = 0; l + 1 < cls_begin.size(); ++l) cls_begin[l + 1] += cls_begin[l];
            cls_rows.resize((size_t)(hi - lo));
            cursor.assign(cls_begin.begin(), cls_begin.end() - 1);
            for (int64_t c = cA; c < cB; ++c) {
                const int32_t l = s->chunk_lengths[(size_t)c];
                for (int64_t i = 0; i < C; ++i) cls_rows[(size_t)cursor[(size_t)l]++] = base[(size_t)(c * C + i)];
            }
            cursor.assign(cls_begin.begin(), cls_begin.end() - 1);
            int32_t blob = 0;
            for (int64_t c0 = cA; c0 < cB;) {
                const int64_t tile_end = std::min(cB, (c0 / T + 1) * T);
                int64_t c1 = c0 + 1;
                const int32_t l = s->chunk_lengths[(size_t)c0];
                while (c1 < tile_end && s->chunk_lengths[(size_t)c1] == l) ++c1;
// ... 394 lines not shown
```

### ultimate-spmv_amd/host/uspmv_internal.hpp

```cpp
#pragma once
#include <sys/mman.h>
#include <cstdint>
#include <cstdarg>
#include <cstdint>
#include <cstdio>
#include <string>
#include <memory>
#include <utility>
#include <vector>

#include "uspmv.h"

template <class T> struct uspmv_noinit_alloc : std::allocator<T> {
    template <class U> struct rebind { using other = uspmv_noinit_alloc<U>; };
    uspmv_noinit_alloc() = default;
    template <class U> uspmv_noinit_alloc(const uspmv_noinit_alloc<U> &) {}
    template <class U, class... A> void construct(U *p, A &&...a) {
        if constexpr (sizeof...(A) == 0) ::new ((void *)p) U;
        else ::new ((void *)p) U(std::forward<A>(a)...);
    }
};
using uspmv_ivec = std::vector<int32_t, uspmv_noinit_alloc<int32_t>>;
using uspmv_dvec = std::vector<double, uspmv_noinit_alloc<double>>;

struct uspmv_coo {
    int64_t n_rows = 0, n_cols = 0, nnz = 0;
    uspmv_ivec I, J;
    uspmv_dvec values;
};

struct uspmv_scs {
    int64_t C = 0, sigma = 0, n_rows = 0, n_cols = 0, n_rows_padded = 0, n_chunks = 0, n_elements = 0, nnz = 0;
    int dtype = USPMV_F64;
    std::vector<int32_t> chunk_ptrs, chunk_lengths, col_idxs, old_to_new_idx, new_to_old_idx;
    std::vector<double> values_f64;
    std::vector<float> values_f32;
    std::vector<uint16_t> values_f16;
    const void *values_ptr() const {
        return dtype == USPMV_F64 ? (const void *)values_f64.data()
             : dtype == USPMV_F32 ? (const void *)values_f32.data() : (const void *)values_f16.data();
    }
};
inline size_t uspmv_dtype_bytes(int dtype) { return dtype == USPMV_F64 ? 8 : dtype == USPMV_F32 ? 4 : 2; }
uint16_t uspmv_f64_to_f16(double v);
double uspmv_f16_to_f64(uint16_t h);

struct uspmv_halo {
    int P = 0, rank = 0;
    int64_t n_local = 0, n_halo = 0;
    std::vector<int32_t> recv_counts_cumsum;
    std::vector<int32_t> recv_counts;
    std::vector<int32_t> recv_idxs;
};

struct uspmv_comm_plan {
    int P = 0, rank = 0;
    int64_t n_local = 0, n_send = 0;
    std::vector<int64_t> send_off, recv_off;
    std::vector<int32_t> send_idxs;
};

template <typename V>
inline void uspmv_resize_huge(V &v, size_t n) {
    v.reserve(n);
    const uintptr_t a = ((uintptr_t)v.data() + (2u << 20) - 1) & ~(uintptr_t)((2u << 20) - 1), e = ((uintptr_t)(v.data() + v.capacity())) & ~(uintptr_t)((2u << 20) - 1);
    if (n * sizeof(typename V::value_type) >= (64u << 20) && e > a) {
        (void)madvise((void *)a, e - a, MADV_HUGEPAGE);
        volatile char *b = (volatile char *)a;
        const int64_t pages = (int64_t)((e - a) >> 12);
#pragma omp parallel for schedule(static)
        for (int64_t k = 0; k < pages; ++k) b[(size_t)k << 12] = 0;
    }
    v.resize(n);
}

struct uspmv_tlc_plan {
    bool valid = false;
    int chunks_per_tile = 0, max_lines_used = 0, tile_rows = 256, line_shift = 4;
    int64_t n_tiles = 0, n_staged_tiles = 0, x_len_min = 0;
    std::vector<int32_t> tile_line_ptr;
    std::vector<int32_t> tile_lines;
    std::vector<uint32_t> c16_ptrs;
    std::vector<uint16_t> col16;
    std::vector<uint32_t> c16_ptrs_b;
    std::vector<uint16_t> col16_b;
    std::vector<uint32_t> c16_ptrs_c;
    std::vector<uint16_t> col16_c;
};
int uspmv_build_tlc_plan(const uspmv_scs *s, const uspmv_scs *s2, int max_lines, int tile_rows, uspmv_tlc_plan *plan, int line_shift = 4,
                         const uspmv_scs *s3 = nullptr);

struct uspmv_additive_plan {
    bool valid = false;
    bool cols_permuted = false;
    int tile_rows = 256, max_elems = 0;
    int64_t n_tiles = 0, n_add_tiles = 0;
    int64_t n_chunks = 0, n_additive = 0;
    int64_t rec_bytes = 0;
    std::vector<int32_t> line_ptr, lines;
    std::vector<int32_t> iv_ptr;
    std::vector<int32_t> iv;
    std::vector<uint32_t> rec_ptrs;
    std::vector<uint16_t> rec;
    std::vector<int32_t> o2n;
    std::vector<int32_t> cmap;
};
int uspmv_build_additive_plan(const uspmv_scs *s, const uspmv_tlc_plan *lp, int budget, uspmv_additive_plan *plan,
                              const std::vector<int32_t> *new_to_old = nullptr, int tile_rows = 0);
void uspmv_additive_plan_decode(const uspmv_scs *s, const uspmv_additive_plan *plan, int32_t *cols);

struct uspmv_sweep_plan {
    bool valid = false;
    int tile_rows = 1024, wlog = 13;
    int64_t n_tiles = 0, n_sweep_tiles = 0, x_len_min = 0;
    std::vector<int32_t> tile_ids, t_smin, t_S;
    std::vector<uint64_t> t_cnt_off;
    std::vector<uint32_t> wave_off, wave_off_b, wave_off_c;
    std::vector<uint8_t> cnt, cnt_b, cnt_c;
    std::vector<uint16_t> idx, idx_b, idx_c;
    std::vector<double> vals_f64, vals_b_f64;
    std::vector<float> vals_f32, vals_b_f32;
    std::vector<uint16_t> vals_b_f16, vals_c_f16;
    std::vector<int32_t> pad_col, pad_col_b, pad_col_c;
    std::vector<int32_t> rest_chunks;
};
int uspmv_build_sweep_plan(const uspmv_scs *s, const uspmv_scs *s2, int wlog, int tile_rows, double max_stage_bytes_per_nnz,
                           uspmv_sweep_plan *plan, const uspmv_scs *s3 = nullptr);

struct uspmv_block_sweep_plan {
    bool valid = false;
    int tile_rows = 2048, wlog = 9;
    int64_t n_tiles = 0, n_sweep_tiles = 0, x_rows_min = 0, windows_staged = 0;
    std::vector<int32_t> tile_ids;
    std::vector<int32_t> t_win_ptr;
    std::vector<int32_t> wins;
    std::vector<uint64_t> t_cnt_off;
    std::vector<uint32_t> wave_off;
    std::vector<uint8_t> cnt;
    std::vector<uint16_t> idx;
    std::vector<double> vals_f64;
    std::vector<float> vals_f32;
    std::vector<int32_t> pad_col;
    std::vector<int32_t> rest_chunks;
};
int uspmv_build_block_sweep_plan(const uspmv_scs *s, int wlog, int tile_rows, int row_bytes, double max_stage_bytes_per_nnz,
                                 uspmv_block_sweep_plan *plan);

struct uspmv_phased_plan {
    bool valid = false;
    int cap_rows = 256, ngp = 8, max_rows_used = 0, line_shift = 0;
    int64_t n_tiles = 0, n_phases = 0;
    std::vector<int32_t> ph_ptr;
    std::vector<int32_t> ph_g0;
    std::vector<int32_t> ph_list_ptr;
    std::vector<int32_t> xrows;
    std::vector<uint32_t> c16_ptrs;
    std::vector<uint16_t> col16;
};
int uspmv_build_phased_plan(const uspmv_scs *s, int cap_rows, int ngp, uspmv_phased_plan *plan, int line_shift = 0, int phase_cost = 0);

int uspmv_scs_rechunk32(const uspmv_scs *s, uspmv_scs *out);
int uspmv_scs_classify_chunks(const uspmv_scs *s, int64_t n_local, std::vector<uint8_t> *cls, int32_t *pad_col);
int uspmv_scs_reorder_ties(const uspmv_scs *s, uspmv_scs *r, std::vector<int32_t> *row_map);
int uspmv_scs_reorder_rows(const uspmv_scs *s, int mode, uspmv_scs *r, std::vector<int32_t> *row_map, int tile_rows = 64, int64_t seg_rows = 65536);
int uspmv_scs_reorder_bricks(const uspmv_scs *s, int64_t stride, int64_t lines, uspmv_scs *r, std::vector<int32_t> *row_map);

int uspmv_scs_layout(const uspmv_coo *m, int64_t C, int64_t sigma, int dtype, const int32_t *fixed_permutation,
                     uspmv_scs *s, std::vector<int64_t> *row_start, const char *who);

namespace uspmv {
int fail(int status, const char *fmt, ...);
inline bool scs_has_entries(const uspmv_scs *s) { return (int64_t)s->col_idxs.size() == s->n_elements; }
double check_x(int64_t global_col);
int64_t check_col(int64_t j, const int32_t *wsa, int P, int rank, bool loopback);
int dist_reference_rows(const uspmv_coo *local, const int32_t *wsa, int P, int rank, bool loopback, int dtype, void *y_ref);
}
```

Measured before the change: 1296 GFLOP/s.

## Add classed additive chunk records and per-line interval tags with 16-bit column delta map

```diff
diff --git a/include/uspmv.h b/include/uspmv.h
--- a/include/uspmv.h
+++ b/include/uspmv.h
@@ -127,6 +127,8 @@
 int uspmv_dmat_index_bits(const uspmv_dmat_t *m, int *bits);
 int uspmv_dmat_additive_chunks(const uspmv_dmat_t *m, int64_t *n_additive, int64_t *n_chunks);
 int uspmv_additive_plan_probe(const uspmv_scs_t *s, int64_t stats[8], int32_t *cols);
+int uspmv_additive_plan_probe2(const uspmv_scs_t *s, int64_t stats[16], int32_t *cols);
+int uspmv_dmat_additive_classed(const uspmv_dmat_t *m, int64_t *n_classed);
 int uspmv_spmv_tiles(const uspmv_dmat_t *A, const int32_t *d_tile_ids, int64_t n_ids, const void *d_x, void *d_y,
                      void *stream);
 int uspmv_dmat_set_crs(uspmv_dmat_t *m, int on);
diff --git a/ultimate-spmv_amd/binding.py b/ultimate-spmv_amd/binding.py
--- a/ultimate-spmv_amd/binding.py
+++ b/ultimate-spmv_amd/binding.py
@@ -87,6 +87,8 @@
     "uspmv_dmat_index_bits": (C.c_int, [_vp, C.POINTER(C.c_int)]),
     "uspmv_dmat_additive_chunks": (C.c_int, [_vp, C.POINTER(C.c_int64), C.POINTER(C.c_int64)]),
     "uspmv_additive_plan_probe": (C.c_int, [_vp, C.POINTER(C.c_int64), _vp]),
+    "uspmv_additive_plan_probe2": (C.c_int, [_vp, C.POINTER(C.c_int64), _vp]),
+    "uspmv_dmat_additive_classed": (C.c_int, [_vp, C.POINTER(C.c_int64)]),
     "uspmv_dmat_optimize_device": (C.c_int, [_vp, C.c_int, C.POINTER(_i64), C.POINTER(_i64)]),
     "uspmv_dmat_optimize_device_ap": (C.c_int, [_vp, _vp, C.c_int, C.POINTER(_i64), C.POINTER(_i64)]),
     "uspmv_dmat_plan_download": (C.c_int, [_vp, C.POINTER(_i64), _vp, _vp, _vp, _vp]),
@@ -862,6 +864,11 @@
         _ck(lib().uspmv_dmat_additive_chunks(self.h, C.byref(a), C.byref(b)))
         return a.value, b.value
 
+    def additive_classed(self):
+        a = C.c_int64()
+        _ck(lib().uspmv_dmat_additive_classed(self.h, C.byref(a)))
+        return a.value
+
     def plan_download(self):
         meta = (_i64 * 4)()
         _ck(lib().uspmv_dmat_plan_download(self.h, meta, None, None, None, None))
@@ -944,10 +951,11 @@
 
 
 def additive_plan_probe(scs, decode=True):
-    st = (C.c_int64 * 8)()
+    st = (C.c_int64 * 16)()
     cols = np.full(scs.n_elements, -3, dtype=np.int32) if decode else None
-    _ck(lib().uspmv_additive_plan_probe(scs.h, st, _np_ptr(cols) if decode else None))
-    keys = ("kept", "n_additive", "n_chunks", "tiles_with_records", "tiles", "new_bytes", "replaced_bytes", "max_elems")
+    _ck(lib().uspmv_additive_plan_probe2(scs.h, st, _np_ptr(cols) if decode else None))
+    keys = ("kept", "n_additive", "n_chunks", "tiles_with_records", "tiles", "new_bytes", "replaced_bytes", "max_elems",
+            "n_classed", "n_intervals", "cols_permuted", "line_entries", "lines", "map_bytes", "record_bytes")
     return dict(zip(keys, [int(v) for v in st])), cols
 
 
diff --git a/ultimate-spmv_amd/csrc/spmv_kernels.hip b/ultimate-spmv_amd/csrc/spmv_kernels.hip
--- a/ultimate-spmv_amd/csrc/spmv_kernels.hip
+++ b/ultimate-spmv_amd/csrc/spmv_kernels.hip
@@ -209,41 +209,45 @@
         const int iv0 = aa.iv_ptr[tile], niv = aa.iv_ptr[tile + 1] - iv0;
         add_tile = niv > 0;
         if (add_tile) {
-            typedef int ivec_t __attribute__((ext_vector_type(EPL)));
+            typedef short svec_t __attribute__((ext_vector_type(EPL)));
+            typedef int i32x4_t __attribute__((ext_vector_type(4)));
             const int sub = threadIdx.x % LPL, lk = threadIdx.x / LPL;
-            for (int k = lk; k < nl; k += blockDim.x / LPL) {
-                const long idx = (long)tile_lines[lp0 + k] * 16 + sub * EPL;
+            const int al0 = aa.line_ptr[tile], anl = aa.line_ptr[tile + 1] - al0;
+            const i32x4_t *ivt = (const i32x4_t *)aa.iv + iv0;
+            const bool mapped = aa.dmap != nullptr;
+            for (int k = lk; k < anl; k += blockDim.x / LPL) {
+                const unsigned le = aa.lines[al0 + k];
+                const long idx = (long)(le & 0x0FFFFFFFu) * 16 + sub * EPL;
+                const i32x4_t q = ivt[le >> 28];
                 vec_t v;
-                ivec_t pc;
                 if (idx + EPL <= x_len) {
                     v = *(const vec_t *)(x + idx);
-                    pc = *(const ivec_t *)(aa.cmap + idx);
                 } else {
 #pragma unroll
-                    for (int e = 0; e < EPL; ++e) { const bool in = idx + e < x_len; v[e] = in ? x[idx + e] : VT(0); pc[e] = in ? aa.cmap[idx + e] : -1; }
+                    for (int e = 0; e < EPL; ++e) v[e] = idx + e < x_len ? x[idx + e] : VT(0);
                 }
-                int pos[EPL];
-#pragma unroll
-                for (int e = 0; e < EPL; ++e) pos[e] = -1;
-                for (int q = 0; q < niv; ++q) {
-                    const int base = aa.iv[4 * (iv0 + q)], len = aa.iv[4 * (iv0 + q) + 1], off = aa.iv[4 * (iv0 + q) + 2];
-#pragma unroll
-                    for (int e = 0; e < EPL; ++e)
-                        if (pc[e] >= base && pc[e] - base < len) pos[e] = off + pc[e] - base;
+                int t[EPL];
+#pragma unroll
+                for (int e = 0; e < EPL; ++e) t[e] = (int)(idx - q[0]) + e;
+                if (mapped) {
+                    const svec_t dv = *(const svec_t *)(aa.dmap + idx);
+#pragma unroll
+                    for (int e = 0; e < EPL; ++e) t[e] += dv[e];
                 }
 #pragma unroll
                 for (int e = 0; e < EPL; ++e)
-                    if (pos[e] >= 0) xs[pos[e]] = v[e];
+                    if ((unsigned)t[e] < (unsigned)q[1]) xs[q[2] + t[e]] = v[e];
             }
             __syncthreads();
             if (L > 0) {
                 const unsigned ap = aa.ptrs[c];
-                const unsigned short *rec = aa.rec + (long)(ap >> 1) * 8;
+                const unsigned short *rec = aa.rec + (long)(ap >> 2) * 8;
                 const VT *vp = values + (long)cs + i;
-                const bool addv = ap & 1u;
-                const unsigned R = addv ? (unsigned)rec[i] : 0u;
-                const u32x4_t *sp = addv ? (const u32x4_t *)(rec + C) : (const u32x4_t *)rec + i;
-                const long ss = addv ? 1 : C;
+                const unsigned kind = ap & 3u;
+                const unsigned R = kind ? (unsigned)rec[i] : 0u;
+                const u32x4_t *sp = kind ? (const u32x4_t *)(rec + C) : (const u32x4_t *)rec + i;
+                if (kind == 2) sp += (C + 15) / 16 + (unsigned)((const unsigned char *)(rec + C))[i] * (unsigned)((L + 7) >> 3);
+                const long ss = kind ? 1 : C;
                 int p = 0;
                 for (; 8 * p + 8 <= L; ++p) {
                     VT v[8];
@@ -497,10 +501,10 @@
     const bool elem = A->tlc.elem;
     const bool add = A->tlc.add_ptrs != nullptr && !elem && !tile_ids && !A->tlc.row_map;
     const size_t lds = std::max((size_t)A->tlc.max_lines * (elem ? 1 : 16), add ? (size_t)A->tlc.add_max_elems : (size_t)0) * sizeof(VT);
-    const AddArgs aa = add ? AddArgs{A->tlc.add_iv_ptr, A->tlc.add_iv, A->tlc.add_cmap, A->tlc.add_ptrs, A->tlc.add_rec} : AddArgs{};
-    const bool own_tiles = add && A->tlc.add_line_ptr != nullptr;
+    const AddArgs aa = add ? AddArgs{A->tlc.add_iv_ptr, A->tlc.add_iv, A->tlc.add_dmap, A->tlc.add_line_ptr, A->tlc.add_lines, A->tlc.add_ptrs, A->tlc.add_rec} : AddArgs{};
+    const bool own_tiles = add && A->tlc.add_tile_rows != A->tlc.tile_rows;
     const int block = own_tiles ? A->tlc.add_tile_rows : A->tlc.tile_rows;
-    const int *lptr = own_tiles ? A->tlc.add_line_ptr : A->tlc.line_ptr, *llist = own_tiles ? A->tlc.add_lines : A->tlc.lines;
+    const int *lptr = own_tiles ? A->tlc.add_line_ptr : A->tlc.line_ptr, *llist = own_tiles ? (const int *)(const uint32_t *)A->tlc.add_lines : A->tlc.lines;
     if (own_tiles) grid = (unsigned)A->tlc.add_n_tiles;
     const bool i12 = A->tlc.col12 != nullptr;
     const unsigned *iptrs = i12 ? A->tlc.c12_ptrs : A->tlc.c16_ptrs;
diff --git a/ultimate-spmv_amd/csrc/tlc_planner.hip b/ultimate-spmv_amd/csrc/tlc_planner.hip
--- a/ultimate-spmv_amd/csrc/tlc_planner.hip
+++ b/ultimate-spmv_amd/csrc/tlc_planner.hip
@@ -143,7 +143,7 @@
         const int64_t L = s->chunk_lengths[(size_t)c];
         b.replaced += idx12 ? 4 * c12_dwords(L, C) : 2 * ((L + 3) / 4) * 4 * C;
     }
-    b.fresh = a.rec_bytes + 4 * (int64_t)a.cmap.size();
+    b.fresh = a.rec_bytes + 2 * (int64_t)a.dmap.size();
     return b;
 }
 int additive_tile_rows(const uspmv_scs *s, int line_plan_rows) {
@@ -159,24 +159,24 @@
     uspmv_additive_plan a;
     if (int rc = uspmv_build_additive_plan(s, &p, max_lines * 16, &a, n2o, additive_tile_rows(s, p.tile_rows))) return rc;
     const AdditiveBytes b = additive_bytes(s, a, A->tlc.col12 != nullptr);
-    if (verbose()) fprintf(stderr, "[uspmv] additive chunk records: valid=%d tiles=%lld of %lld chunks=%lld additive=%lld max_elems=%d tile_rows=%d records+map=%lld B against %lld B of local indices (columns %s) -> %s\n",
-                           (int)a.valid, (long long)a.n_add_tiles, (long long)a.n_tiles, (long long)a.n_chunks, (long long)a.n_additive, a.max_elems, a.tile_rows, (long long)b.fresh,
+    if (verbose()) fprintf(stderr, "[uspmv] additive chunk records: valid=%d tiles=%lld of %lld chunks=%lld additive=%lld classed=%lld max_elems=%d tile_rows=%d records+map=%lld B against %lld B of local indices (columns %s) -> %s\n",
+                           (int)a.valid, (long long)a.n_add_tiles, (long long)a.n_tiles, (long long)a.n_chunks, (long long)a.n_additive, (long long)a.n_classed, a.max_elems, a.tile_rows, (long long)b.fresh,
                            (long long)b.replaced, a.cols_permuted ? "permuted" : "as they are", additive_kept(a, b) ? "kept" : "dropped");
     if (!additive_kept(a, b)) return USPMV_OK;
     auto &t = A->tlc;
     hipError_t e = t.add_iv_ptr.upload(a.iv_ptr.data(), a.iv_ptr.size() * 4);
     if (e == hipSuccess) e = t.add_iv.upload(a.iv.data(), a.iv.size() * 4);
-    if (e == hipSuccess) e = t.add_cmap.upload(a.cmap.data(), a.cmap.size() * 4);
+    if (e == hipSuccess && !a.dmap.empty()) e = t.add_dmap.upload(a.dmap.data(), a.dmap.size() * 2);
     if (e == hipSuccess) e = t.add_rec.upload(a.rec.data(), a.rec.size() * 2);
     if (e == hipSuccess) e = t.add_ptrs.upload(a.rec_ptrs.data(), a.rec_ptrs.size() * 4);
-    if (e == hipSuccess && !a.line_ptr.empty()) e = t.add_line_ptr.upload(a.line_ptr.data(), a.line_ptr.size() * 4);
-    if (e == hipSuccess && !a.line_ptr.empty()) e = t.add_lines.upload(a.lines.data(), a.lines.size() * 4);
+    if (e == hipSuccess) e = t.add_line_ptr.upload(a.line_ptr.data(), a.line_ptr.size() * 4);
+    if (e == hipSuccess) e = t.add_lines.upload(a.lines.data(), std::max<size_t>(a.lines.size(), 1) * 4);
     if (e != hipSuccess) {
         t.add_line_ptr.reset(); t.add_lines.reset();
-        t.add_iv_ptr.reset(); t.add_iv.reset(); t.add_cmap.reset(); t.add_rec.reset(); t.add_ptrs.reset();
+        t.add_iv_ptr.reset(); t.add_iv.reset(); t.add_dmap.reset(); t.add_rec.reset(); t.add_ptrs.reset();
         return uspmv::fail(USPMV_ERR_ALLOC, "%s: device copy of the additive chunk records failed: %s", who, hipGetErrorString(e));
     }
-    t.add_max_elems = a.max_elems; t.add_chunks = a.n_chunks; t.add_additive = a.n_additive;
+    t.add_max_elems = a.max_elems; t.add_chunks = a.n_chunks; t.add_additive = a.n_additive; t.add_classed = a.n_classed;
     t.add_tile_rows = a.tile_rows; t.add_n_tiles = a.n_tiles;
     return USPMV_OK;
 }
@@ -595,11 +595,11 @@
 
 extern "C" {
 
-int uspmv_additive_plan_probe(const uspmv_scs_t *s, int64_t stats[8], int32_t *cols) {
+int uspmv_additive_plan_probe2(const uspmv_scs_t *s, int64_t stats[16], int32_t *cols) {
     const char *who = "uspmv_additive_plan_probe";
     if (!s || !stats) return uspmv::fail(USPMV_ERR_INVALID, "%s: NULL argument", who);
     if (!uspmv::scs_has_entries(s)) return uspmv::fail(USPMV_ERR_INVALID, "%s: layout-only struct", who);
-    for (int k = 0; k < 8; ++k) stats[k] = 0;
+    for (int k = 0; k < 16; ++k) stats[k] = 0;
     if (cols) for (int64_t k = 0; k < s->n_elements; ++k) cols[k] = -1;
     const int max_lines = line_budget(0, s->dtype, false);
     uspmv_tlc_plan p;
@@ -615,8 +615,17 @@
     stats[0] = additive_kept(a, b); stats[1] = a.n_additive; stats[2] = a.n_chunks; stats[3] = a.n_add_tiles;
     stats[5] = b.fresh; stats[6] = b.replaced; stats[7] = a.max_elems;
     if (a.valid) stats[4] = a.n_tiles;
+    stats[8] = a.n_classed; stats[9] = (int64_t)(a.iv.size() / 4); stats[10] = a.valid && a.cols_permuted;
+    stats[11] = (int64_t)a.lines.size(); stats[12] = a.n_lines; stats[13] = 2 * (int64_t)a.dmap.size(); stats[14] = a.rec_bytes;
     if (cols && stats[0]) uspmv_additive_plan_decode(s, &a, cols);
     return USPMV_OK;
+}
+
+int uspmv_additive_plan_probe(const uspmv_scs_t *s, int64_t stats[8], int32_t *cols) {
+    int64_t st[16];
+    const int rc = uspmv_additive_plan_probe2(s, st, cols);
+    if (stats) for (int k = 0; k < 8; ++k) stats[k] = st[k];
+    return rc;
 }
 
 int uspmv_dmat_optimize(uspmv_dmat_t *A, const uspmv_scs_t *s, int max_lines, int64_t *n_tiles, int64_t *n_staged) {
diff --git a/ultimate-spmv_amd/csrc/uspmv_api.hip b/ultimate-spmv_amd/csrc/uspmv_api.hip
--- a/ultimate-spmv_amd/csrc/uspmv_api.hip
+++ b/ultimate-spmv_amd/csrc/uspmv_api.hip
@@ -1279,6 +1279,13 @@
     return USPMV_OK;
 }
 
+int uspmv_dmat_additive_classed(const uspmv_dmat_t *A, int64_t *n_classed) {
+    if (!A || !n_classed) return uspmv::fail(USPMV_ERR_INVALID, "uspmv_dmat_additive_classed: NULL argument");
+    const uspmv_dmat_t *M = (A->alt && g_tune.rechunk) ? A->alt : A;
+    *n_classed = M->tlc.on && M->tlc.add_ptrs ? M->tlc.add_classed : 0;
+    return USPMV_OK;
+}
+
 int uspmv_spmmv(const uspmv_dmat_t *A, const void *d_X, void *d_Y, int b, int64_t ld, int layout, void *stream) {
     if (int rc = check_dmat_one_prec(A, "uspmv_spmmv")) return rc;
     if (!d_X || !d_Y || b < 1) return uspmv::fail(USPMV_ERR_INVALID, "uspmv_spmmv: bad argument");
diff --git a/ultimate-spmv_amd/csrc/uspmv_device.hpp b/ultimate-spmv_amd/csrc/uspmv_device.hpp
--- a/ultimate-spmv_amd/csrc/uspmv_device.hpp
+++ b/ultimate-spmv_amd/csrc/uspmv_device.hpp
@@ -125,13 +125,15 @@
         DeviceBuf<uint32_t> c12_ptrs, col12;
         DeviceBuf<void> values;
         DeviceBuf<int32_t> row_map, cols;
-        DeviceBuf<int32_t> add_iv_ptr, add_iv, add_cmap;
+        DeviceBuf<int32_t> add_iv_ptr, add_iv;
+        DeviceBuf<int16_t> add_dmap;
         DeviceBuf<uint32_t> add_ptrs;
         DeviceBuf<uint16_t> add_rec;
-        DeviceBuf<int32_t> add_line_ptr, add_lines;
+        DeviceBuf<int32_t> add_line_ptr;
+        DeviceBuf<uint32_t> add_lines;
         int add_max_elems = 0, add_tile_rows = 0;
         int64_t add_n_tiles = 0;
-        int64_t add_chunks = 0, add_additive = 0;
+        int64_t add_chunks = 0, add_additive = 0, add_classed = 0;
     } tlc;
     struct BlockPlan {
         bool on = false;
@@ -224,7 +226,10 @@
 };
 
 struct AddArgs {
-    const int *iv_ptr = nullptr, *iv = nullptr, *cmap = nullptr;
+    const int *iv_ptr = nullptr, *iv = nullptr;
+    const short *dmap = nullptr;
+    const int *line_ptr = nullptr;
+    const unsigned *lines = nullptr;
     const unsigned *ptrs = nullptr;
     const unsigned short *rec = nullptr;
 };
diff --git a/ultimate-spmv_amd/host/tlc_plan.cpp b/ultimate-spmv_amd/host/tlc_plan.cpp
--- a/ultimate-spmv_amd/host/tlc_plan.cpp
+++ b/ultimate-spmv_amd/host/tlc_plan.cpp
@@ -136,6 +136,10 @@
     int64_t row(int64_t r) const { return r < n_rows ? n2o[r] : r; }
     int64_t col(int32_t c) const { return cm ? cm[c] : c; }
 };
+constexpr int ADD_MAX_IV = 16;
+constexpr int64_t ADD_HOLE = 32;
+constexpr int ADD_MAX_CLASSES = 8;
+constexpr uint32_t ADD_LINE_MASK = 0x0FFFFFFFu;
 bool chunk_offsets(const uspmv_scs *s, const AddMaps &m, int64_t c, const int64_t *rr, int64_t *d) {
     const int64_t C = s->C, cs = s->chunk_ptrs[(size_t)c], L = s->chunk_lengths[(size_t)c];
     const int32_t *ci = s->col_idxs.data() + cs;
@@ -147,13 +151,66 @@
     }
     return true;
 }
+int chunk_classes(const uspmv_scs *s, const AddMaps &m, int64_t c, const int64_t *rr, uint8_t *cls, int64_t *d, int64_t *lo, int64_t *hi) {
+    const int64_t C = s->C, cs = s->chunk_ptrs[(size_t)c], L = s->chunk_lengths[(size_t)c];
+    const int32_t *ci = s->col_idxs.data() + cs;
+    int n = 0;
+    for (int64_t i = 0; i < C; ++i) {
+        int k = 0;
+        for (; k < n; ++k) {
+            const int64_t *dk = d + (int64_t)k * L;
+            int64_t j = 0;
+            while (j < L && m.col(ci[j * C + i]) - rr[i] == dk[j]) ++j;
+            if (j == L) break;
+        }
+        if (k == n) {
+            if (n == ADD_MAX_CLASSES) return 0;
+            for (int64_t j = 0; j < L; ++j) d[(int64_t)n * L + j] = m.col(ci[j * C + i]) - rr[i];
+            lo[n] = hi[n] = rr[i];
+            ++n;
+        } else { lo[k] = std::min(lo[k], rr[i]); hi[k] = std::max(hi[k], rr[i]); }
+        cls[i] = (uint8_t)k;
+    }
+    return n;
+}
 int64_t add_pos(const int32_t *iv, int n_iv, int64_t p, int *which = nullptr) {
     for (int k = 0; k < n_iv; ++k)
         if (p >= iv[4 * k] && p < (int64_t)iv[4 * k] + iv[4 * k + 1]) { if (which) *which = k; return iv[4 * k + 2] + p - iv[4 * k]; }
     return -1;
 }
-constexpr int ADD_MAX_IV = 16;
-constexpr int64_t ADD_HOLE = 32;
+struct ChunkEnc {
+    int kind = 0, n_cls = 0;
+    uint32_t units = 0;
+    int64_t lo[ADD_MAX_CLASSES], hi[ADD_MAX_CLASSES];
+    std::vector<int64_t> rr, d;
+    std::vector<uint8_t> cls;
+};
+void chunk_encode(const uspmv_scs *s, const AddMaps &m, int64_t c, const int32_t *iv, int n_iv, ChunkEnc &E) {
+    const int64_t C = s->C, L = s->chunk_lengths[(size_t)c], B = (L + 7) / 8;
+    E.kind = 0; E.n_cls = 0;
+    E.units = (uint32_t)(B * C);
+    if (L < 1) return;
+    E.rr.resize((size_t)C); E.cls.assign((size_t)C, 0); E.d.resize((size_t)(ADD_MAX_CLASSES * L));
+    int64_t lo = INT64_MAX, hi = INT64_MIN;
+    for (int64_t i = 0; i < C; ++i) { E.rr[(size_t)i] = m.row(c * C + i); lo = std::min(lo, E.rr[(size_t)i]); hi = std::max(hi, E.rr[(size_t)i]); }
+    int n = 0;
+    if (chunk_offsets(s, m, c, E.rr.data(), E.d.data())) { n = 1; E.lo[0] = lo; E.hi[0] = hi; }
+    else n = chunk_classes(s, m, c, E.rr.data(), E.cls.data(), E.d.data(), E.lo, E.hi);
+    for (int k = 0; k < n; ++k)
+        if (E.hi[k] - E.lo[k] > 65535) return;
+    const uint32_t units = (uint32_t)(n == 1 ? C / 8 + B : C / 8 + (C + 15) / 16 + n * B);
+    if (n < 1 || units >= E.units) return;
+    E.n_cls = n;
+    if (!iv) return;
+    for (int k = 0; k < n; ++k)
+        for (int64_t j = 0; j < L; ++j) {
+            int ka = -1, kb = -2;
+            const int64_t dj = E.d[(size_t)(k * L + j)];
+            if (add_pos(iv, n_iv, E.lo[k] + dj, &ka) < 0 || add_pos(iv, n_iv, E.hi[k] + dj, &kb) < 0 || ka != kb) return;
+        }
+    E.kind = n == 1 ? 1 : 2;
+    E.units = units;
+}
 }
 
 int uspmv_build_additive_plan(const uspmv_scs *s, const uspmv_tlc_plan *lp, int budget, uspmv_additive_plan *p, const std::vector<int32_t> *new_to_old, int tile_rows) {
@@ -163,18 +220,19 @@
     if (!lp || !lp->valid || lp->line_shift != 4 || C < 8 || C % 8 != 0 || C > lp->tile_rows || nc < 1 || n < 1 || n != s->n_cols) return USPMV_OK;
     if ((int64_t)n2o.size() < n || n > (int64_t)INT32_MAX || lp->x_len_min > n) return USPMV_OK;
     budget = std::min(budget, 65536);
-    std::vector<int32_t> inv((size_t)n, -1);
-    for (int64_t r = 0; r < n; ++r) {
-        const int64_t o = n2o[(size_t)r];
-        if (o < 0 || o >= n || inv[(size_t)o] >= 0) return USPMV_OK;
-        inv[(size_t)o] = (int32_t)r;
+    {
+        std::vector<char> seen((size_t)n, 0);
+        for (int64_t r = 0; r < n; ++r) {
+            const int64_t o = n2o[(size_t)r];
+            if (o < 0 || o >= n || seen[(size_t)o]) return USPMV_OK;
+            seen[(size_t)o] = 1;
+        }
     }
     const bool own_tiles = tile_rows > 0 && tile_rows != lp->tile_rows && tile_rows % C == 0 && tile_rows <= 1024 && lp->n_staged_tiles == lp->n_tiles;
     if (!own_tiles) tile_rows = lp->tile_rows;
     const int64_t T = tile_rows / C, nt = (nc + T - 1) / T;
     p->tile_rows = tile_rows;
     p->n_tiles = nt;
-    std::vector<std::vector<int32_t>> t_lines(own_tiles ? (size_t)nt : 0);
     AddMaps m{n2o.data(), n2o.data(), n};
     {
         const int64_t step = std::max<int64_t>(1, nc / 4096);
@@ -200,25 +258,27 @@
         p->cols_permuted = hits[0] >= hits[1];
         if (!p->cols_permuted) m.cm = nullptr;
     }
+    std::vector<int16_t> dmap;
+    if (p->cols_permuted) {
+        dmap.assign((size_t)((n + 15) / 16 * 16), 0);
+        bool fits = true;
+#pragma omp parallel for schedule(static) reduction(&& : fits)
+        for (int64_t k = 0; k < n; ++k) {
+            const int64_t dk = (int64_t)n2o[(size_t)k] - k;
+            fits = fits && dk >= -32767 && dk <= 32767;
+            dmap[(size_t)k] = (int16_t)dk;
+        }
+        if (!fits) return USPMV_OK;
+    }
     std::vector<std::vector<int32_t>> t_iv((size_t)nt);
+    std::vector<std::vector<uint32_t>> t_lines((size_t)nt);
+    std::vector<int32_t> t_nl((size_t)nt, 0);
     std::vector<uint32_t> units((size_t)nc, 0);
-    std::vector<uint8_t> additive((size_t)nc, 0);
-    auto chunk_additive = [&](int64_t c, const int32_t *iv, int n_iv, int64_t *rr, int64_t *d, int64_t *rmin) -> bool {
-        const int64_t L = s->chunk_lengths[(size_t)c];
-        if (L < 1) return false;
-        int64_t lo = INT64_MAX, hi = INT64_MIN;
-        for (int64_t i = 0; i < C; ++i) { rr[i] = m.row(c * C + i); lo = std::min(lo, rr[i]); hi = std::max(hi, rr[i]); }
-        *rmin = lo;
-        if (hi - lo > 65535 || !chunk_offsets(s, m, c, rr, d)) return false;
-        for (int64_t j = 0; j < L; ++j) {
-            int ka = -1, kb = -2;
-            if (add_pos(iv, n_iv, lo + d[j], &ka) < 0 || add_pos(iv, n_iv, hi + d[j], &kb) < 0 || ka != kb) return false;
-        }
-        return true;
-    };
+    std::vector<uint8_t> kind((size_t)nc, 0);
 #pragma omp parallel
     {
-        std::vector<int64_t> cols, rr((size_t)C), d;
+        std::vector<int64_t> cols;
+        ChunkEnc E;
         std::vector<std::pair<int64_t, int64_t>> gaps;
         std::vector<size_t> cb;
         std::vector<char> joined;
@@ -248,13 +308,10 @@
             auto run_of = [&](int64_t pc) { return (size_t)(std::upper_bound(cb.begin(), cb.begin() + (long)n_run, (size_t)(std::lower_bound(cols.begin(), cols.end(), pc) - cols.begin())) - cb.begin()) - 1; };
             for (int64_t c = c0; c < c1 && n_run > 1; ++c) {
                 const int64_t L = s->chunk_lengths[(size_t)c];
-                if (L < 1) continue;
-                int64_t lo = INT64_MAX, hi = INT64_MIN;
-                for (int64_t i = 0; i < C; ++i) { rr[(size_t)i] = m.row(c * C + i); lo = std::min(lo, rr[(size_t)i]); hi = std::max(hi, rr[(size_t)i]); }
-                d.resize((size_t)L + 1);
-                if (hi - lo > 65535 || !chunk_offsets(s, m, c, rr.data(), d.data())) continue;
-                for (int64_t j = 0; j < L; ++j)
-                    for (size_t k = run_of(lo + d[(size_t)j]), ke = run_of(hi + d[(size_t)j]); k < ke; ++k) joined[k] = 1;
+                chunk_encode(s, m, c, nullptr, 0, E);
+                for (int q = 0; q < E.n_cls; ++q)
+                    for (int64_t j = 0; j < L; ++j)
+                        for (size_t k = run_of(E.lo[q] + E.d[(size_t)(q * L + j)]), ke = run_of(E.hi[q] + E.d[(size_t)(q * L + j)]); k < ke; ++k) joined[k] = 1;
             }
             std::vector<int32_t> iv;
             int64_t total = 0;
@@ -282,31 +339,34 @@
             if (total > budget) continue;
             const int n_iv = (int)iv.size() / 4;
             for (int64_t c = c0; c < c1; ++c) {
-                const int64_t L = s->chunk_lengths[(size_t)c];
-                d.resize((size_t)L + 1);
-                int64_t rmin = 0;
-                additive[(size_t)c] = chunk_additive(c, iv.data(), n_iv, rr.data(), d.data(), &rmin);
-                units[(size_t)c] = (uint32_t)(additive[(size_t)c] ? C / 8 + (L + 7) / 8 : ((L + 7) / 8) * C);
-            }
+                chunk_encode(s, m, c, iv.data(), n_iv, E);
+                kind[(size_t)c] = (uint8_t)E.kind;
+                units[(size_t)c] = E.units;
+            }
+            auto &ln = t_lines[(size_t)t];
+            for (int64_t k = e0; k < e1; ++k) {
+                const int32_t col = s->col_idxs[(size_t)k];
+                int q = 0;
+                add_pos(iv.data(), n_iv, m.col(col), &q);
+                ln.push_back(((uint32_t)(col >> 4) << 4) | (uint32_t)q);
+            }
+            std::sort(ln.begin(), ln.end());
+            ln.erase(std::unique(ln.begin(), ln.end()), ln.end());
+            int32_t nl = 0;
+            for (size_t k = 0; k < ln.size(); ++k) {
+                nl += k == 0 || (ln[k] >> 4) != (ln[k - 1] >> 4);
+                ln[k] = (ln[k] >> 4) | ((ln[k] & 15u) << 28);
+            }
+            t_nl[(size_t)t] = nl;
             t_iv[(size_t)t] = std::move(iv);
-            if (own_tiles) {
-                auto &ln = t_lines[(size_t)t];
-                for (int64_t k = e0; k < e1; ++k) ln.push_back(s->col_idxs[(size_t)k] >> 4);
-                std::sort(ln.begin(), ln.end());
-                ln.erase(std::unique(ln.begin(), ln.end()), ln.end());
-            }
-        }
-    }
-    if (own_tiles) {
-        int64_t with = 0, n_lines = 0;
-        for (int64_t t = 0; t < nt; ++t) { with += !t_iv[(size_t)t].empty() || s->chunk_ptrs[(size_t)std::min<int64_t>(t * T + T, nc)] == s->chunk_ptrs[(size_t)(t * T)]; n_lines += (int64_t)t_lines[(size_t)t].size(); }
-        if (with != nt || n_lines > (int64_t)INT32_MAX) return uspmv_build_additive_plan(s, lp, budget, p, new_to_old, 0);
-        p->line_ptr.assign((size_t)nt + 1, 0);
-        p->lines.reserve((size_t)n_lines);
-        for (int64_t t = 0; t < nt; ++t) {
-            p->lines.insert(p->lines.end(), t_lines[(size_t)t].begin(), t_lines[(size_t)t].end());
-            p->line_ptr[(size_t)t + 1] = (int32_t)p->lines.size();
-        }
+        }
+    }
+    int64_t n_entries = 0;
+    {
+        int64_t with = 0;
+        for (int64_t t = 0; t < nt; ++t) { with += !t_iv[(size_t)t].empty() || s->chunk_ptrs[(size_t)std::min<int64_t>(t * T + T, nc)] == s->chunk_ptrs[(size_t)(t * T)]; n_entries += (int64_t)t_lines[(size_t)t].size(); }
+        if (own_tiles && with != nt) return uspmv_build_additive_plan(s, lp, budget, p, new_to_old, 0);
+        if (n_entries > (int64_t)INT32_MAX) { *p = {}; return USPMV_OK; }
     }
     p->iv_ptr.assign((size_t)nt + 1, 0);
     int64_t n_iv_all = 0;
@@ -319,40 +379,52 @@
         int64_t total = 0;
         for (int64_t q = 0; q < k; ++q) total += t_iv[(size_t)t][(size_t)(4 * q + 1)];
         p->max_elems = std::max<int>(p->max_elems, (int)total);
+        p->n_lines += t_nl[(size_t)t];
         const int64_t c0 = t * T, c1 = std::min<int64_t>(c0 + T, nc);
         p->n_chunks += c1 - c0;
-        for (int64_t c = c0; c < c1; ++c) p->n_additive += additive[(size_t)c];
+        for (int64_t c = c0; c < c1; ++c) { p->n_additive += kind[(size_t)c] == 1; p->n_classed += kind[(size_t)c] == 2; }
     }
     p->iv_ptr[(size_t)nt] = (int32_t)n_iv_all;
     if (p->n_add_tiles == 0 || n_iv_all > (int64_t)INT32_MAX / 4) return USPMV_OK;
+    p->line_ptr.assign((size_t)nt + 1, 0);
+    p->lines.reserve((size_t)n_entries);
+    for (int64_t t = 0; t < nt; ++t) {
+        p->lines.insert(p->lines.end(), t_lines[(size_t)t].begin(), t_lines[(size_t)t].end());
+        p->line_ptr[(size_t)t + 1] = (int32_t)p->lines.size();
+    }
     p->iv.resize((size_t)(4 * n_iv_all));
     for (int64_t t = 0; t < nt; ++t) std::copy(t_iv[(size_t)t].begin(), t_iv[(size_t)t].end(), p->iv.begin() + 4 * (int64_t)p->iv_ptr[(size_t)t]);
     p->rec_ptrs.assign((size_t)nc, 0);
     int64_t tot_units = 0;
     for (int64_t c = 0; c < nc; ++c) {
-        p->rec_ptrs[(size_t)c] = (uint32_t)(tot_units << 1) | additive[(size_t)c];
+        p->rec_ptrs[(size_t)c] = (uint32_t)(tot_units << 2) | kind[(size_t)c];
         tot_units += units[(size_t)c];
-        if (tot_units >= ((int64_t)1 << 31)) return USPMV_OK;
+        if (tot_units >= ((int64_t)1 << 30)) return USPMV_OK;
     }
     p->rec_bytes = tot_units * 16;
     p->rec.assign((size_t)(tot_units * 8), 0);
 #pragma omp parallel
     {
-        std::vector<int64_t> rr((size_t)C), d;
+        ChunkEnc E;
 #pragma omp for schedule(dynamic, 16)
         for (int64_t t = 0; t < nt; ++t) {
             const int n_iv = p->iv_ptr[(size_t)t + 1] - p->iv_ptr[(size_t)t];
             if (n_iv == 0) continue;
             const int32_t *iv = p->iv.data() + 4 * (int64_t)p->iv_ptr[(size_t)t];
             for (int64_t c = t * T; c < std::min<int64_t>(t * T + T, nc); ++c) {
-                const int64_t cs = s->chunk_ptrs[(size_t)c], L = s->chunk_lengths[(size_t)c];
-                uint16_t *q = p->rec.data() + (size_t)(p->rec_ptrs[(size_t)c] >> 1) * 8;
-                if (additive[(size_t)c]) {
-                    d.resize((size_t)L + 1);
-                    int64_t rmin = 0;
-                    chunk_additive(c, iv, n_iv, rr.data(), d.data(), &rmin);
-                    for (int64_t i = 0; i < C; ++i) q[i] = (uint16_t)(rr[(size_t)i] - rmin);
-                    for (int64_t j = 0; j < L; ++j) q[C + j] = (uint16_t)add_pos(iv, n_iv, rmin + d[(size_t)j]);
+                const int64_t cs = s->chunk_ptrs[(size_t)c], L = s->chunk_lengths[(size_t)c], B = (L + 7) / 8;
+                uint16_t *q = p->rec.data() + (size_t)(p->rec_ptrs[(size_t)c] >> 2) * 8;
+                if (kind[(size_t)c]) {
+                    chunk_encode(s, m, c, iv, n_iv, E);
+                    for (int64_t i = 0; i < C; ++i) q[i] = (uint16_t)(E.rr[(size_t)i] - E.lo[E.cls[(size_t)i]]);
+                    uint16_t *S = q + C;
+                    if (kind[(size_t)c] == 2) {
+                        uint8_t *cl = (uint8_t *)(q + C);
+                        for (int64_t i = 0; i < C; ++i) cl[i] = E.cls[(size_t)i];
+                        S += 8 * ((C + 15) / 16);
+                    }
+                    for (int k = 0; k < E.n_cls; ++k)
+                        for (int64_t j = 0; j < L; ++j) S[k * B * 8 + j] = (uint16_t)add_pos(iv, n_iv, E.lo[k] + E.d[(size_t)(k * L + j)]);
                 } else {
                     for (int64_t j = 0; j < L; ++j)
                         for (int64_t i = 0; i < C; ++i)
@@ -361,8 +433,7 @@
             }
         }
     }
-    if (p->cols_permuted) { p->o2n.swap(inv); p->cmap.assign(n2o.begin(), n2o.begin() + n); }
-    else { p->o2n.resize((size_t)n); for (int64_t k = 0; k < n; ++k) p->o2n[(size_t)k] = (int32_t)k; p->cmap = p->o2n; }
+    p->dmap.swap(dmap);
     p->valid = true;
     return USPMV_OK;
 }
@@ -378,17 +449,25 @@
         if (n_iv == 0) continue;
         if (c % T == 0) {
             const int32_t *iv = p->iv.data() + 4 * (int64_t)p->iv_ptr[(size_t)t];
-            lds.clear();
-            for (int k = 0; k < n_iv; ++k) {
-                lds.resize((size_t)iv[4 * k + 2], -2);
-                for (int32_t e = 0; e < iv[4 * k + 1]; ++e) lds.push_back(p->o2n[(size_t)(iv[4 * k] + e)]);
-            }
-        }
-        const int64_t cs = s->chunk_ptrs[(size_t)c], L = s->chunk_lengths[(size_t)c];
-        const uint16_t *q = p->rec.data() + (size_t)(p->rec_ptrs[(size_t)c] >> 1) * 8;
+            lds.assign((size_t)p->max_elems, -2);
+            for (int32_t k = p->line_ptr[(size_t)t]; k < p->line_ptr[(size_t)t + 1]; ++k) {
+                const uint32_t e = p->lines[(size_t)k];
+                const int32_t *q = iv + 4 * (e >> 28);
+                for (int64_t col = (int64_t)(e & ADD_LINE_MASK) * 16, ce = col + 16; col < ce; ++col) {
+                    const int64_t pos = col + (p->dmap.empty() ? 0 : p->dmap[(size_t)col]) - q[0];
+                    if (pos >= 0 && pos < q[1]) lds[(size_t)(q[2] + pos)] = (int32_t)col;
+                }
+            }
+        }
+        const int64_t cs = s->chunk_ptrs[(size_t)c], L = s->chunk_lengths[(size_t)c], B = (L + 7) / 8;
+        const uint32_t kind = p->rec_ptrs[(size_t)c] & 3u;
+        const uint16_t *q = p->rec.data() + (size_t)(p->rec_ptrs[(size_t)c] >> 2) * 8;
         for (int64_t j = 0; j < L; ++j)
             for (int64_t i = 0; i < C; ++i) {
-                const size_t l = (p->rec_ptrs[(size_t)c] & 1) ? (size_t)q[i] + q[C + j] : (size_t)q[((j / 8) * C + i) * 8 + (j % 8)];
+                size_t l;
+                if (kind == 1) l = (size_t)q[i] + q[C + j];
+                else if (kind == 2) l = (size_t)q[i] + q[C + 8 * ((C + 15) / 16) + (int64_t)((const uint8_t *)(q + C))[i] * B * 8 + j];
+                else l = (size_t)q[((j / 8) * C + i) * 8 + (j % 8)];
                 out[cs + j * C + i] = l < lds.size() ? lds[l] : -2;
             }
     }
diff --git a/ultimate-spmv_amd/host/uspmv_internal.hpp b/ultimate-spmv_amd/host/uspmv_internal.hpp
--- a/ultimate-spmv_amd/host/uspmv_internal.hpp
+++ b/ultimate-spmv_amd/host/uspmv_internal.hpp
@@ -96,14 +96,16 @@
     int tile_rows = 256, max_elems = 0;
     int64_t n_tiles = 0, n_add_tiles = 0;
     int64_t n_chunks = 0, n_additive = 0;
+    int64_t n_classed = 0;
+    int64_t n_lines = 0;
     int64_t rec_bytes = 0;
-    std::vector<int32_t> line_ptr, lines;
+    std::vector<int32_t> line_ptr;
+    std::vector<uint32_t> lines;
     std::vector<int32_t> iv_ptr;
     std::vector<int32_t> iv;
     std::vector<uint32_t> rec_ptrs;
     std::vector<uint16_t> rec;
-    std::vector<int32_t> o2n;
-    std::vector<int32_t> cmap;
+    std::vector<int16_t> dmap;
 };
 int uspmv_build_additive_plan(const uspmv_scs *s, const uspmv_tlc_plan *lp, int budget, uspmv_additive_plan *plan,
                               const std::vector<int32_t> *new_to_old = nullptr, int tile_rows = 0);
```

Result: slower. 1181 GFLOP/s (-8.9%).
